# wamuumu/query-recommendation-system

Hardware: AMD Instinct MI355X
Metric: MinHash signatures/sec through the whole hot path (signatures -> LSH candidates -> pair scoring -> top-K) (higher is better)
Workload: dtype u16/int32 MinHash values, uint64 keys and pairs (integer); float64 cosine

## Files before the change

### include/qrlsh.h

```cpp
#ifndef QRLSH_H
#define QRLSH_H

#include <stddef.h>
#include <stdint.h>

#ifdef __cplusplus
extern "C" {
#endif

#define QRLSH_OK 0
#define QRLSH_EINVAL (-1)
#define QRLSH_EHIP (-2)
#define QRLSH_EUNSUPPORTED (-3)
#define QRLSH_EWORKSPACE (-4)

#define QRLSH_PERM_U16 0
#define QRLSH_PERM_I32 1

#define QRLSH_SIG_I32 0
#define QRLSH_SIG_U16 1

#define QRLSH_SORT_MIX 1u
#define QRLSH_SORT_IOTA 2u
#define QRLSH_SORT_FOLD 4u
#define QRLSH_SORT_OWNER 8u

#define QRLSH_SORT_HOST 16u

int qrlsh_version(void);
const char *qrlsh_last_error(void);

uint64_t qrlsh_mix64_host(uint64_t x);

int qrlsh_check_csr(const int64_t *offsets, const int32_t *rows, int64_t nq, int64_t nnz, int32_t D,
                    uint32_t *flags_out, void *stream);
int qrlsh_minhash(const int64_t *offsets, const int32_t *rows, int64_t nq, const void *perm_t,
                  int32_t perm_dtype, int32_t P, int32_t P_stride, int32_t D, int32_t *sig_out,
                  uint16_t *sig16_out, int64_t *norm2_out, uint64_t *keys_out, int32_t b, void *stream);

int qrlsh_band_keys(const int32_t *sig, int64_t nq, int32_t P, int32_t b, uint64_t *keys_out,
                    int64_t *norm2_out, void *stream);

size_t qrlsh_sort_workspace_bytes(int64_t n, int32_t nbatch);
int qrlsh_sort_u64(uint64_t *keys_a, uint64_t *keys_b, uint32_t *vals_a, uint32_t *vals_b, int64_t n,
                   int32_t nbatch, int32_t bit_lo, int32_t bit_hi, uint32_t flags, uint64_t aux,
                   void *workspace, size_t workspace_bytes, void *stream);

int qrlsh_owner_bounds(const uint64_t *words, int64_t n, int32_t bit_lo, uint64_t shard, int32_t world,
                       int64_t *bounds_out, void *stream);

size_t qrlsh_pairs_workspace_bytes(int64_t nq, int32_t b);
int qrlsh_pairs_count(const uint64_t *sorted_keys, int64_t nq, int32_t b, int32_t r, int32_t hash_bits,
                      void *workspace, size_t workspace_bytes, uint64_t *total_out, void *stream);
int qrlsh_pairs_fill(const uint64_t *sorted_keys, const uint32_t *sorted_ids, int64_t nq, int32_t b,
                     int32_t r, int32_t hash_bits, const void *workspace, uint64_t *pairs_out,
                     void *stream);

size_t qrlsh_bucket_workspace_bytes(int64_t nq, int32_t b, int32_t part_bits);
int qrlsh_bucket_pairs_count(const uint64_t *keys, uint64_t *part_keys, uint32_t *part_ids,
                             uint64_t *tmp_keys, uint32_t *tmp_ids, int64_t nq, int32_t b, int32_t r,
                             int32_t part_bits, void *workspace, size_t workspace_bytes,
                             uint64_t *total_overflow_out, void *stream);
int qrlsh_bucket_pairs_fill(const uint64_t *part_keys, const uint32_t *part_ids, int64_t nq, int32_t b,
                            int32_t r, int32_t part_bits, void *workspace, uint64_t *pairs_out,
                            void *stream);
size_t qrlsh_bucket_part_words(int64_t nq, int32_t b, int32_t part_bits);
int64_t qrlsh_set_big_part_limit(int64_t records);
size_t qrlsh_bucket_tmp_words(int64_t nq, int32_t b, int32_t part_bits);
int qrlsh_bucket_pairs_emit(const uint64_t *keys, uint64_t *part_keys, uint32_t *part_ids,
                            uint64_t *tmp_keys, uint32_t *tmp_ids, int64_t nq, int32_t b, int32_t r,
                            int32_t part_bits, void *workspace, size_t workspace_bytes,
                            uint64_t *pairs_out, uint64_t capacity, uint64_t *total_overflow_out,
                            void *stream);

int qrlsh_bucket_pairs_emit_chunked(const uint64_t *keys, int64_t key_chunk, int64_t key_chunk_stride,
                                    int64_t key_band_stride, uint64_t *part_keys, uint32_t *part_ids,
                                    uint64_t *tmp_keys, uint32_t *tmp_ids, int64_t nq, int32_t b, int32_t r,
                                    int32_t part_bits, void *workspace, size_t workspace_bytes,
                                    uint64_t *pairs_out, uint64_t capacity, uint64_t *total_overflow_out,
                                    void *stream);

size_t qrlsh_compact_workspace_bytes(int64_t n);
int qrlsh_unique_count(const uint64_t *sorted, int64_t n, void *workspace, size_t workspace_bytes,
                       uint64_t *total_out, void *stream);
int qrlsh_unique_fill(const uint64_t *sorted, int64_t n, const void *workspace, uint64_t *out,
                      void *stream);

size_t qrlsh_row_unique_workspace_bytes(int64_t n);
int qrlsh_row_unique_count(const uint64_t *grouped, int64_t n, int32_t group_bits, int32_t id_bits,
                           uint64_t *tmp, void *workspace, size_t workspace_bytes, uint64_t *total_overflow_out,
                           void *stream);
int qrlsh_row_unique_fill(const uint64_t *tmp, int64_t n, const void *workspace, uint64_t *out, void *stream);

size_t qrlsh_region_unique_workspace_bytes(int64_t nids, int32_t group_bits);
int qrlsh_region_unique_count(const uint64_t *grouped, int64_t n, int32_t group_bits, int32_t id_bits, int64_t nids,
                              uint64_t *tmp, void *workspace, size_t workspace_bytes, uint64_t *total_overflow_out,
                              void *stream);
int qrlsh_region_unique_fill(const uint64_t *tmp, int64_t n, int32_t group_bits, int64_t nids, const void *workspace,
                             uint64_t *out, void *stream);

size_t qrlsh_pair_regions_words(int64_t n, int64_t nids, int32_t group_bits, double words_per_query);
size_t qrlsh_pair_regions_tmp_words(int64_t n, int64_t nids, int32_t group_bits, double words_per_query);
int64_t qrlsh_pair_regions_cap(int64_t n, int64_t nids, int32_t group_bits, double words_per_query);
int64_t qrlsh_pair_regions_count(int64_t n, int64_t nids, int32_t group_bits, double words_per_query);
int qrlsh_pair_regions_scatter(const uint64_t *words, int64_t n, int32_t group_bits, int64_t nids, double words_per_query,
                               uint64_t *tmp_regions, uint64_t *regions, uint32_t *counts, uint32_t *overflow_out,
                               void *stream);
int qrlsh_region_unique_count_regions(const uint64_t *regions, const uint32_t *counts, int64_t cap, int64_t n,
                                      int32_t group_bits, int32_t id_bits, int64_t nids, uint64_t *tmp, void *workspace,
                                      size_t workspace_bytes, uint64_t *total_overflow_out, void *stream);

int qrlsh_row_norms(const int32_t *sig, int64_t nq, int32_t P, int64_t *norm2_out, void *stream);
int qrlsh_verify_pairs(const void *sig, int32_t sig_dtype, int32_t P, int32_t b, const uint64_t *pairs,
                       int64_t n, uint8_t *flags_out, void *stream);
int qrlsh_score_pairs(const void *sig, int32_t sig_dtype, const int64_t *norm2, int32_t P,
                      const uint64_t *pairs, int64_t n, int32_t *milli_out, double *cos_out,
                      uint64_t *edge_out, int32_t id_bits, uint32_t *edge_dst_out, void *stream);

int qrlsh_topk_count(const uint64_t *sorted_edges, int64_t n_edges, int32_t K, int32_t id_bits,
                     void *workspace, size_t workspace_bytes, uint64_t *total_out, void *stream);
int qrlsh_topk_fill(const uint64_t *sorted_edges, const uint32_t *sorted_dst, int64_t n_edges, int32_t K,
                    int32_t id_bits, const void *workspace, int32_t *src_out, int32_t *dst_out,
                    int32_t *milli_out, void *stream);
int qrlsh_topk_fill_based(const uint64_t *sorted_edges, const uint32_t *sorted_dst, int64_t n_edges, int32_t K,
                          int32_t id_bits, int64_t src_base, const void *workspace, int32_t *src_out,
                          int32_t *dst_out, int32_t *milli_out, void *stream);

int qrlsh_score_pairs_rev(const void *sig, int32_t sig_dtype, const int64_t *norm2, int32_t P,
                          const uint64_t *pairs, int64_t n, int32_t *milli_out, uint64_t *rev_out, int32_t id_bits,
                          uint32_t *rev_dst_out, void *stream);
int qrlsh_set_score_runs(int on);
size_t qrlsh_topk_select_workspace_bytes(int64_t nq);
int qrlsh_topk_select_count(const uint64_t *pairs, int64_t n, const uint64_t *rev_sorted, const uint32_t *rev_dst,
                            int64_t nq, int32_t K, int32_t id_bits, void *workspace, size_t workspace_bytes,
                            uint64_t *total_out, void *stream);
int qrlsh_topk_select_fill(const uint64_t *pairs, const int32_t *milli, int64_t n, const uint64_t *rev_sorted,
                           const uint32_t *rev_dst, int64_t nq, int32_t K, int32_t id_bits, const void *workspace,
                           int32_t *src_out, int32_t *dst_out, int32_t *milli_out, void *stream);

int qrlsh_remap_pairs(const uint64_t *pairs, int64_t n, int64_t q0, int64_t nql, const uint64_t *need,
                      int64_t n_need, uint64_t *out, void *stream);
int qrlsh_pair_edges(const uint64_t *pairs, const int32_t *milli, int64_t n, int32_t id_bits,
                     uint64_t *fwd_out, uint64_t *rev_out, uint32_t *fwd_dst_out, uint32_t *rev_dst_out,
                     void *stream);
size_t qrlsh_idset_workspace_bytes(int64_t nids);
int qrlsh_idset_build(const uint64_t *pairs, int64_t n, int64_t q0, int64_t nql, int64_t nids, int64_t shard,
                      int32_t world, void *workspace, size_t workspace_bytes, int64_t *bounds_out, void *stream);
int qrlsh_idset_list(const void *workspace, int64_t nids, uint64_t *ids_out, void *stream);
int qrlsh_idset_remap(const uint64_t *pairs, int64_t n, int64_t q0, int64_t nql, const void *workspace,
                      int64_t nids, uint64_t *out, void *stream);
int qrlsh_gather_rows(const void *sig, int64_t row_bytes, const int64_t *norm2, const uint64_t *ids, int64_t n,
                      int64_t q0, void *rows_out, int64_t *norms_out, void *stream);
int qrlsh_score_pairs_split(const void *sig, const int64_t *norm2, int64_t split_rows, const void *sig_b,
                            const int64_t *norm2_b, int32_t sig_dtype, int32_t P, const uint64_t *pairs,
                            int64_t n, int32_t *milli_out, void *stream);
int qrlsh_edges_localize(const uint64_t *edges, const uint32_t *edge_dst, int64_t n, int32_t id_bits, int64_t q0,
                         int64_t nql, uint64_t *out, void *stream);

int qrlsh_answer_sets_count(const uint32_t *bitmaps, int64_t words_per_row, int64_t D,
                            const int32_t *qrows, int64_t nq, int32_t nfeat, int32_t *sizes_out,
                            void *stream);
int qrlsh_answer_sets_fill(const uint32_t *bitmaps, int64_t words_per_row, int64_t D,
                           const int32_t *qrows, int64_t nq, int32_t nfeat, const int64_t *offsets,
                           int32_t *rows_out, void *stream);

int qrlsh_answer_sets_sweep(const uint32_t *bitmaps, int64_t words_per_row, int64_t D,
                            const int32_t *qrows, int64_t nq, int32_t nfeat, int32_t *sizes_out,
                            int32_t *slots_out, void *stream);
int qrlsh_answer_sets_compact(const int32_t *slots, const int64_t *offsets, int64_t nq,
                              int32_t *rows_out, void *stream);

#define QRLSH_SUM_PAIRWISE 0
#define QRLSH_SUM_SEQUENTIAL 1
size_t qrlsh_predict_workspace_bytes(int64_t nu, int64_t nq, int32_t kq);
int qrlsh_predict(const int32_t *ratings, int64_t nu, int64_t nq, const int64_t *q_off,
                  const int32_t *q_idx, const double *q_val, const int32_t *u_idx, const double *u_val,
                  int32_t ku, double query_weight, double user_weight, double default_mean,
                  int32_t sum_order, int32_t *out, uint32_t *too_long_out, int32_t kq, void *workspace,
                  size_t workspace_bytes, void *stream);

#define QRLSH_RECOMMEND_MAX_K 1024
size_t qrlsh_recommend_workspace_bytes(int64_t m, int64_t nq, int32_t k, int32_t slices);
int qrlsh_recommend_topk(const int32_t *ratings, const int32_t *pred, int64_t nu, int64_t nq, const int32_t *users,
                         int64_t m, int32_t k, int32_t lo, int32_t slices, int32_t *idx_out, int32_t *val_out,
                         int32_t *avail_out, void *workspace, size_t workspace_bytes, void *stream);

int qrlsh_center_rows(const int32_t *ratings, int64_t nu, int64_t nq, int64_t nq_stride, int32_t *out,
                      void *stream);

size_t qrlsh_user_gram_workspace_bytes(int64_t nu, int64_t nq);
int qrlsh_user_gram(const int32_t *ratings, int64_t nu, int64_t nq, double *mean_out, double *inv_scale_out,
                    double *gram_out, void *workspace, size_t workspace_bytes, void *stream);

size_t qrlsh_gather_sets_workspace_bytes(int64_t n);
int qrlsh_gather_sets_count(const uint64_t *ids, int64_t n, const void *offs, int32_t off_bytes, int64_t nql,
                            int64_t world, uint64_t *offsets_out, void *workspace, size_t workspace_bytes,
                            void *stream);
int qrlsh_gather_sets_fill(const uint64_t *ids, int64_t n, const void *offs, int32_t off_bytes, const void *rows,
                           int32_t row_bytes, int64_t nql, int64_t max_nnz, const uint64_t *offsets,
                           int32_t *rows_out, void *stream);

int qrlsh_synth_sizes(uint64_t seed, int64_t q0, int64_t nq_local, int64_t nq_total, int32_t cluster,
                      uint32_t D, const uint32_t *cdf, int32_t ncdf, uint32_t rep_thresh24,
                      int32_t *sizes_out, void *stream);
int qrlsh_synth_fill(uint64_t seed, int64_t q0, int64_t nq_local, int64_t nq_total, int32_t cluster,
                     uint32_t D, const uint32_t *cdf, int32_t ncdf, uint32_t rep_thresh24,
                     const int64_t *offsets, int32_t *rows_out, void *stream);

int qrlsh_prof_enable(int on);
int qrlsh_set_overlap(int on);
int qrlsh_prof_pause(int paused);
int qrlsh_prof_report(char *buf_host, size_t buflen);

#ifdef __cplusplus
}
#endif
#endif
```

### query-recommendation-system_amd/csrc/score.hip

```cpp
#include <stdlib.h>

#include "common.h"

typedef int i32x4 __attribute__((ext_vector_type(4)));
typedef unsigned short u16x8 __attribute__((ext_vector_type(8)));
typedef unsigned int u32x4 __attribute__((ext_vector_type(4)));

constexpr int SCORE_LPP = 16;

__device__ static inline int64_t c16(unsigned short v) { return v == 0xFFFFu ? -1 : (int64_t)v; }

template <typename SigT, bool VECLOAD>
__global__ __launch_bounds__(256) void score_pairs_kernel(const SigT *__restrict__ sig,
                                                          const int64_t *__restrict__ norm2, int P,
                                                          const uint64_t *__restrict__ pairs, int64_t n,
                                                          int32_t *__restrict__ milli, double *__restrict__ cosv,
                                                          uint64_t *__restrict__ edges, int id_bits,
                                                          uint32_t *__restrict__ edge_dst,
                                                          const SigT *__restrict__ sig_b,
                                                          const int64_t *__restrict__ norm2_b, uint32_t split,
                                                          int rev_only) {
  constexpr bool IS16 = sizeof(SigT) == 2;
  constexpr int VEC = IS16 ? 8 : 4;
  const int lane = threadIdx.x & (WAVE - 1);
  const int lig = lane & (SCORE_LPP - 1);
  const int64_t group = (((int64_t)blockIdx.x * blockDim.x + threadIdx.x) / SCORE_LPP);
  const int64_t ngroups = ((int64_t)gridDim.x * blockDim.x) / SCORE_LPP;
  const int64_t iters = (n + ngroups - 1) / ngroups;
  uint64_t pr_next = (group < n) ? pairs[group] : 0;
  for (int64_t it = 0; it < iters; ++it) {
    const int64_t t = it * ngroups + group;
    const bool live = t < n;
    const uint64_t pr = pr_next;
    const int64_t tn = t + ngroups;
    pr_next = (tn < n) ? pairs[tn] : 0;
    const uint32_t i = (uint32_t)(pr >> 32), j = (uint32_t)pr;
    const SigT *a = i < split ? sig + (size_t)i * P : sig_b + (size_t)(i - split) * P;
    const SigT *c = j < split ? sig + (size_t)j * P : sig_b + (size_t)(j - split) * P;
    const bool own_norms = norm2 == nullptr;
    int64_t na = 0, nb = 0;
    if (!own_norms && live && lig == 0) {
      na = i < split ? norm2[i] : norm2_b[i - split];
      nb = j < split ? norm2[j] : norm2_b[j - split];
    }
    int64_t dot = 0;
    if (live) {
      if (VECLOAD) {
        for (int col = lig * VEC; col < P; col += SCORE_LPP * VEC) {
          if (IS16) {
            const u16x8 x = *reinterpret_cast<const u16x8 *>(a + col);
            const u16x8 y = *reinterpret_cast<const u16x8 *>(c + col);
            const u32x4 xw = __builtin_bit_cast(u32x4, x), yw = __builtin_bit_cast(u32x4, y);
            const uint32_t hi = (xw[0] | xw[1] | xw[2] | xw[3] | yw[0] | yw[1] | yw[2] | yw[3]) & 0x80008000u;
            if (hi == 0) {
              uint32_t s0 = __builtin_amdgcn_udot2(__builtin_shufflevector(x, x, 0, 1),
                                                   __builtin_shufflevector(y, y, 0, 1), 0u, false);
              uint32_t s1 = __builtin_amdgcn_udot2(__builtin_shufflevector(x, x, 2, 3),
                                                   __builtin_shufflevector(y, y, 2, 3), 0u, false);
              s0 = __builtin_amdgcn_udot2(__builtin_shufflevector(x, x, 4, 5), __builtin_shufflevector(y, y, 4, 5),
                                          s0, false);
              s1 = __builtin_amdgcn_udot2(__builtin_shufflevector(x, x, 6, 7), __builtin_shufflevector(y, y, 6, 7),
                                          s1, false);
              dot += (int64_t)((uint64_t)s0 + (uint64_t)s1);
              if (own_norms) {
                uint32_t a0 = 0, a1 = 0, b0 = 0, b1 = 0;
                a0 = __builtin_amdgcn_udot2(__builtin_shufflevector(x, x, 0, 1), __builtin_shufflevector(x, x, 0, 1), a0, false);
                a1 = __builtin_amdgcn_udot2(__builtin_shufflevector(x, x, 2, 3), __builtin_shufflevector(x, x, 2, 3), a1, false);
                a0 = __builtin_amdgcn_udot2(__builtin_shufflevector(x, x, 4, 5), __builtin_shufflevector(x, x, 4, 5), a0, false);
                a1 = __builtin_amdgcn_udot2(__builtin_shufflevector(x, x, 6, 7), __builtin_shufflevector(x, x, 6, 7), a1, false);
                b0 = __builtin_amdgcn_udot2(__builtin_shufflevector(y, y, 0, 1), __builtin_shufflevector(y, y, 0, 1), b0, false);
                b1 = __builtin_amdgcn_udot2(__builtin_shufflevector(y, y, 2, 3), __builtin_shufflevector(y, y, 2, 3), b1, false);
                b0 = __builtin_amdgcn_udot2(__builtin_shufflevector(y, y, 4, 5), __builtin_shufflevector(y, y, 4, 5), b0, false);
                b1 = __builtin_amdgcn_udot2(__builtin_shufflevector(y, y, 6, 7), __builtin_shufflevector(y, y, 6, 7), b1, false);
                na += (int64_t)((uint64_t)a0 + (uint64_t)a1);
                nb += (int64_t)((uint64_t)b0 + (uint64_t)b1);
              }
            } else {
#pragma unroll
              for (int e = 0; e < 8; ++e) {
                const int64_t xe = c16(x[e]), ye = c16(y[e]);
                dot += xe * ye;
                if (own_norms) {
                  na += xe * xe;
                  nb += ye * ye;
                }
              }
            }
          } else {
            const i32x4 x = *reinterpret_cast<const i32x4 *>(a + col);
            const i32x4 y = *reinterpret_cast<const i32x4 *>(c + col);
            dot += (int64_t)x.x * y.x + (int64_t)x.y * y.y + (int64_t)x.z * y.z + (int64_t)x.w * y.w;
            if (own_norms) {
              na += (int64_t)x.x * x.x + (int64_t)x.y * x.y + (int64_t)x.z * x.z + (int64_t)x.w * x.w;
              nb += (int64_t)y.x * y.x + (int64_t)y.y * y.y + (int64_t)y.z * y.z + (int64_t)y.w * y.w;
            }
          }
        }
      } else {
        for (int col = lig; col < P; col += SCORE_LPP) {
          const int64_t xe = IS16 ? c16((unsigned short)a[col]) : (int64_t)a[col];
          const int64_t ye = IS16 ? c16((unsigned short)c[col]) : (int64_t)c[col];
          dot += xe * ye;
          if (own_norms) {
            na += xe * xe;
            nb += ye * ye;
          }
        }
      }
    }
#pragma unroll
    for (int m = 1; m < SCORE_LPP; m <<= 1) dot += __shfl_xor(dot, m, WAVE);
    if (own_norms) {
#pragma unroll
      for (int m = 1; m < SCORE_LPP; m <<= 1) {
        na += __shfl_xor(na, m, WAVE);
        nb += __shfl_xor(nb, m, WAVE);
      }
    }
    if (live && lig == 0) {
      double cs = 0.0;
      if (na != 0 && nb != 0) cs = (double)dot / (sqrt((double)na) * sqrt((double)nb));
      const int32_t mi = (int32_t)rint(cs * 1000.0);
      milli[t] = mi;
      if (cosv) cosv[t] = cs;
      if (edges) {
        const uint64_t inv = (uint64_t)(1000 - mi);
        if (rev_only) {
          if (edge_dst) {
            edges[t] = ((uint64_t)j << 11) | inv;
            edge_dst[t] = i;
          } else {
            edges[t] = ((uint64_t)j << (id_bits + 11)) | (inv << id_bits) | i;
          }
        } else if (edge_dst) {
          edges[2 * t] = ((uint64_t)i << 11) | inv;
          edges[2 * t + 1] = ((uint64_t)j << 11) | inv;
          edge_dst[2 * t] = j;
          edge_dst[2 * t + 1] = i;
        } else {
          edges[2 * t] = ((uint64_t)i << (id_bits + 11)) | (inv << id_bits) | j;
          edges[2 * t + 1] = ((uint64_t)j << (id_bits + 11)) | (inv << id_bits) | i;
        }
      }
    }
  }
}

template <int U> __device__ static inline uint32_t row_bcast_u32(uint32_t v) {
  return (uint32_t)__builtin_amdgcn_update_dpp((int)v, (int)v, 0x150 + U, 0xF, 0xF, false);
}
template <int CTRL> __device__ static inline uint64_t dpp_add_u64(uint64_t v) {
  const uint32_t lo = (uint32_t)__builtin_amdgcn_update_dpp(0, (int)(uint32_t)v, CTRL, 0xF, 0xF, false);
  const uint32_t hi = (uint32_t)__builtin_amdgcn_update_dpp(0, (int)(uint32_t)(v >> 32), CTRL, 0xF, 0xF, false);
  return v + (((uint64_t)hi << 32) | lo);
}
__device__ static inline uint64_t row_sum_u64(uint64_t v) {
  v = dpp_add_u64<0xB1>(v);
  v = dpp_add_u64<0x4E>(v);
  v = dpp_add_u64<0x141>(v);
  v = dpp_add_u64<0x140>(v);
  return v;
}

__device__ static __attribute__((noinline)) uint64_t chunk_dot_wide(u16x8 x, u16x8 y) {
  int64_t d = 0;
#pragma unroll
  for (int e = 0; e < 8; ++e) d += c16(x[e]) * c16(y[e]);
  return (uint64_t)d;
}

__device__ static inline uint64_t chunk_dot(u16x8 x, u16x8 y) {
  const u32x4 xw = __builtin_bit_cast(u32x4, x), yw = __builtin_bit_cast(u32x4, y);
  const uint32_t hi = (xw[0] | xw[1] | xw[2] | xw[3] | yw[0] | yw[1] | yw[2] | yw[3]) & 0x80008000u;
  if (hi == 0) {
    uint32_t s0 = __builtin_amdgcn_udot2(__builtin_shufflevector(x, x, 0, 1), __builtin_shufflevector(y, y, 0, 1), 0u, false);
    uint32_t s1 = __builtin_amdgcn_udot2(__builtin_shufflevector(x, x, 2, 3), __builtin_shufflevector(y, y, 2, 3), 0u, false);
    s0 = __builtin_amdgcn_udot2(__builtin_shufflevector(x, x, 4, 5), __builtin_shufflevector(y, y, 4, 5), s0, false);
    s1 = __builtin_amdgcn_udot2(__builtin_shufflevector(x, x, 6, 7), __builtin_shufflevector(y, y, 6, 7), s1, false);
    return (uint64_t)s0 + (uint64_t)s1;
  }
  return chunk_dot_wide(x, y);
}

#ifndef QR_SCORE_PF
#define QR_SCORE_PF 1
#endif
constexpr int SCORE_PF = QR_SCORE_PF;

#ifndef QR_SCORE_OCC
#define QR_SCORE_OCC 8
#endif
#ifndef QR_SCORE_OCC2
#define QR_SCORE_OCC2 5
#endif
template <int CH>
__global__ __launch_bounds__(256, CH == 1 ? QR_SCORE_OCC : QR_SCORE_OCC2) void score_runs_kernel(const uint16_t *__restrict__ sig, const int64_t *__restrict__ norm2,
                                                         const uint64_t *__restrict__ pairs, int64_t n,
                                                         int32_t *__restrict__ milli, double *__restrict__ cosv,
                                                         uint64_t *__restrict__ edges, int id_bits,
                                                         uint32_t *__restrict__ edge_dst,
                                                         const uint16_t *__restrict__ sig_b,
                                                         const int64_t *__restrict__ norm2_b, uint32_t split, int rev_only) {
  constexpr int P = CH * 128;
  constexpr int NB = SCORE_PF + 1;
  const int lig = threadIdx.x & (SCORE_LPP - 1);
  const int64_t group = ((int64_t)blockIdx.x * blockDim.x + threadIdx.x) / SCORE_LPP;
  const int64_t nchunks = (n + SCORE_LPP - 1) / SCORE_LPP;
  auto row_of = [&](uint32_t id) -> const uint16_t * {
    return (id < split ? sig + (size_t)id * P : sig_b + (size_t)(id - split) * P) + lig * 8;
  };
  auto load_row = [&](u16x8 (&dst)[CH], const uint16_t *p) {
#pragma unroll
    for (int k = 0; k < CH; ++k) dst[k] = *reinterpret_cast<const u16x8 *>(p + k * 128);
  };
  {
    const int64_t c = group;
    if (c >= nchunks) return;
    const int64_t t = c * SCORE_LPP + lig;
    const bool live = t < n;
    const uint64_t pw = live ? pairs[t] : 0ull;
    const uint32_t my_i = (uint32_t)(pw >> 32), my_j = (uint32_t)pw;
    int64_t na = 0, nb = 0;
    if (live) {
      na = my_i < split ? norm2[my_i] : norm2_b[my_i - split];
      nb = my_j < split ? norm2[my_j] : norm2_b[my_j - split];
    }
    uint64_t my_dot = 0;
    u16x8 ab[NB][CH], cb[NB][CH];
#define QR_ROW_I(U) row_bcast_u32<(U)>(my_i)
#define QR_ROW_J(U) row_bcast_u32<(U)>(my_j)
#ifndef QR_SCORE_AREUSE
#define QR_SCORE_AREUSE 0
#endif
#if QR_SCORE_AREUSE
#define QR_REQ(V)                                                                           \
    if ((V) < SCORE_LPP) {                                                                  \
      if ((V) == 0) {                                                                       \
        load_row(ab[0], row_of(QR_ROW_I(0)));                                               \
      } else {                                                                              \
        const uint32_t vi = QR_ROW_I((V) % SCORE_LPP), pi = QR_ROW_I(((V) + SCORE_LPP - 1) % SCORE_LPP); \
        _Pragma("unroll") for (int k = 0; k < CH; ++k) ab[(V) % NB][k] = ab[((V) + NB - 1) % NB][k]; \
        if (vi != pi) load_row(ab[(V) % NB], row_of(vi));                                   \
      }                                                                                     \
      load_row(cb[(V) % NB], row_of(QR_ROW_J((V) % SCORE_LPP)));                            \
    }
#else
#define QR_REQ(V)                                                                           \
    if ((V) < SCORE_LPP) {                                                                  \
      load_row(ab[(V) % NB], row_of(QR_ROW_I((V) % SCORE_LPP)));                            \
      load_row(cb[(V) % NB], row_of(QR_ROW_J((V) % SCORE_LPP)));                            \
    }
#endif
    static_assert(SCORE_PF >= 1 && SCORE_PF <= 4, "prefetch depth");
    QR_REQ(0)
    if (SCORE_PF > 1) { QR_REQ(1) }
    if (SCORE_PF > 2) { QR_REQ(2) }
    if (SCORE_PF > 3) { QR_REQ(3) }
#define QR_STEP(U)                                                                          \
    {                                                                                       \
      QR_REQ((U) + SCORE_PF)                                                                \
      uint64_t part = 0;                                                                    \
      _Pragma("unroll") for (int k = 0; k < CH; ++k) part += chunk_dot(ab[(U) % NB][k], cb[(U) % NB][k]); \
      const uint64_t tot = row_sum_u64(part);                                               \
      if (lig == (U)) my_dot = tot;                                                         \
      asm volatile("" : "+v"(my_dot));     \
      __builtin_amdgcn_sched_barrier(0);  \
    }
    QR_STEP(0) QR_STEP(1) QR_STEP(2) QR_STEP(3) QR_STEP(4) QR_STEP(5) QR_STEP(6) QR_STEP(7)
    QR_STEP(8) QR_STEP(9) QR_STEP(10) QR_STEP(11) QR_STEP(12) QR_STEP(13) QR_STEP(14) QR_STEP(15)
#undef QR_STEP
#undef QR_REQ
#undef QR_ROW_I
#undef QR_ROW_J
    if (live) {
      const int64_t dot = (int64_t)my_dot;
      double cs = 0.0;
      if (na != 0 && nb != 0) cs = (double)dot / (sqrt((double)na) * sqrt((double)nb));
      const int32_t mi = (int32_t)rint(cs * 1000.0);
      milli[t] = mi;
      if (cosv) cosv[t] = cs;
      if (edges) {
        const uint64_t inv = (uint64_t)(1000 - mi), i = my_i, j = my_j;
        if (rev_only) {
          if (edge_dst) {
            edges[t] = (j << 11) | inv;
            edge_dst[t] = (uint32_t)i;
          } else {
            edges[t] = (j << (id_bits + 11)) | (inv << id_bits) | i;
          }
        } else if (edge_dst) {
          edges[2 * t] = (i << 11) | inv;
          edges[2 * t + 1] = (j << 11) | inv;
          edge_dst[2 * t] = (uint32_t)j;
          edge_dst[2 * t + 1] = (uint32_t)i;
        } else {
          edges[2 * t] = (i << (id_bits + 11)) | (inv << id_bits) | j;
          edges[2 * t + 1] = (j << (id_bits + 11)) | (inv << id_bits) | i;
        }
      }
    }
  }
}

static int g_score_runs = -1;
QRLSH_EXPORT int qrlsh_set_score_runs(int on) {
  const int old = g_score_runs;
  g_score_runs = on != 0;
  return old;
}

static int score_launch(const void *sig, const void *sig_b, int64_t split, int32_t sig_dtype, const int64_t *norm2,
                        const int64_t *norm2_b, int32_t P, const uint64_t *pairs, int64_t n, int32_t *milli_out,
                        double *cos_out, uint64_t *edge_out, int32_t id_bits, uint32_t *edge_dst_out, void *stream,
                        int rev_only = 0) {
  const int64_t groups_per_block = 256 / SCORE_LPP;
  int64_t blocks = ceil_div64(n, groups_per_block);
  if (blocks > 256 * 32) blocks = 256 * 32;
  hipStream_t st = static_cast<hipStream_t>(stream);
  const dim3 grid((unsigned)blocks), block(256);
  const bool aligned = ((((uintptr_t)sig | (uintptr_t)sig_b) & 15) == 0);
  const uint32_t sp = split >= (1ll << 32) ? 0xFFFFFFFFu : (uint32_t)split;
  if (sig_dtype == QRLSH_SIG_U16) {
    const uint16_t *s16 = static_cast<const uint16_t *>(sig), *s16b = static_cast<const uint16_t *>(sig_b);
    if (g_score_runs < 0) {
      const char *e = getenv("QRLSH_SCORE_RUNS");
      g_score_runs = !(e && e[0] == '0');
    }
    if (g_score_runs && aligned && norm2 && (P == 128 || P == 256) && (sig_b == nullptr || norm2_b)) {
      const int64_t rb = ceil_div64(ceil_div64(n, SCORE_LPP), groups_per_block);
      QR_CHECK_ARG(rb <= 2147483647ll, "qrlsh_score_pairs: too many pairs for one launch");
      const dim3 rgrid((unsigned)rb);
      if (P == 128)
        QR_LAUNCH("score_pairs", (score_runs_kernel<1>), rgrid, block, 0, st, s16, norm2, pairs, n, milli_out, cos_out,
                  edge_out, id_bits, edge_dst_out, s16b, norm2_b, sp, rev_only);
      else
        QR_LAUNCH("score_pairs", (score_runs_kernel<2>), rgrid, block, 0, st, s16, norm2, pairs, n, milli_out, cos_out,
                  edge_out, id_bits, edge_dst_out, s16b, norm2_b, sp, rev_only);
      QR_LAUNCH_CHECK("qrlsh_score_pairs");
      return QRLSH_OK;
    }
    if (aligned && P % 8 == 0)
      QR_LAUNCH("score_pairs", (score_pairs_kernel<uint16_t, true>), grid, block, 0, st, s16, norm2, P, pairs, n, milli_out,
                cos_out, edge_out, id_bits, edge_dst_out, s16b, norm2_b, sp, rev_only);
    else
      QR_LAUNCH("score_pairs", (score_pairs_kernel<uint16_t, false>), grid, block, 0, st, s16, norm2, P, pairs, n, milli_out,
                cos_out, edge_out, id_bits, edge_dst_out, s16b, norm2_b, sp, rev_only);
  } else {
    const int32_t *s32 = static_cast<const int32_t *>(sig), *s32b = static_cast<const int32_t *>(sig_b);
    if (aligned && P % 4 == 0)
      QR_LAUNCH("score_pairs", (score_pairs_kernel<int32_t, true>), grid, block, 0, st, s32, norm2, P, pairs, n, milli_out,
                cos_out, edge_out, id_bits, edge_dst_out, s32b, norm2_b, sp, rev_only);
    else
      QR_LAUNCH("score_pairs", (score_pairs_kernel<int32_t, false>), grid, block, 0, st, s32, norm2, P, pairs, n, milli_out,
                cos_out, edge_out, id_bits, edge_dst_out, s32b, norm2_b, sp, rev_only);
  }
  QR_LAUNCH_CHECK("qrlsh_score_pairs");
  return QRLSH_OK;
}

QRLSH_EXPORT int qrlsh_score_pairs(const void *sig, int32_t sig_dtype, const int64_t *norm2, int32_t P,
                                   const uint64_t *pairs, int64_t n, int32_t *milli_out, double *cos_out,
                                   uint64_t *edge_out, int32_t id_bits, uint32_t *edge_dst_out, void *stream) {
  QR_CHECK_ARG(n >= 0 && P > 0, "qrlsh_score_pairs: bad sizes n=%lld P=%d", (long long)n, P);
  QR_CHECK_ARG(sig_dtype == QRLSH_SIG_I32 || sig_dtype == QRLSH_SIG_U16, "qrlsh_score_pairs: bad sig_dtype %d", sig_dtype);
  if (n == 0) return QRLSH_OK;
  QR_CHECK_ARG(sig && pairs && milli_out, "qrlsh_score_pairs: null pointer");
  if (edge_out && !edge_dst_out)
    QR_CHECK_ARG(id_bits > 0 && id_bits <= 26, "qrlsh_score_pairs: id_bits=%d must be in [1,26] without edge_dst_out", id_bits);
  QR_CHECK_ARG(!edge_dst_out || edge_out, "qrlsh_score_pairs: edge_dst_out needs edge_out");
  return score_launch(sig, nullptr, 1ll << 32, sig_dtype, norm2, nullptr, P, pairs, n, milli_out, cos_out, edge_out,
                      id_bits, edge_dst_out, stream);
}

QRLSH_EXPORT int qrlsh_score_pairs_rev(const void *sig, int32_t sig_dtype, const int64_t *norm2, int32_t P,
                                       const uint64_t *pairs, int64_t n, int32_t *milli_out, uint64_t *rev_out,
                                       int32_t id_bits, uint32_t *rev_dst_out, void *stream) {
  QR_CHECK_ARG(n >= 0 && P > 0, "qrlsh_score_pairs_rev: bad sizes n=%lld P=%d", (long long)n, P);
  QR_CHECK_ARG(sig_dtype == QRLSH_SIG_I32 || sig_dtype == QRLSH_SIG_U16, "qrlsh_score_pairs_rev: bad sig_dtype %d",
               sig_dtype);
  if (n == 0) return QRLSH_OK;
  QR_CHECK_ARG(sig && pairs && milli_out && rev_out, "qrlsh_score_pairs_rev: null pointer");
  QR_CHECK_ARG(rev_dst_out || (id_bits > 0 && id_bits <= 26),
               "qrlsh_score_pairs_rev: id_bits=%d must be in [1,26] without rev_dst_out", id_bits);
  return score_launch(sig, nullptr, 1ll << 32, sig_dtype, norm2, nullptr, P, pairs, n, milli_out, nullptr, rev_out, id_bits,
                      rev_dst_out, stream, 1);
}

QRLSH_EXPORT int qrlsh_score_pairs_split(const void *sig, const int64_t *norm2, int64_t split_rows, const void *sig_b,
                                         const int64_t *norm2_b, int32_t sig_dtype, int32_t P, const uint64_t *pairs,
                                         int64_t n, int32_t *milli_out, void *stream) {
  QR_CHECK_ARG(n >= 0 && P > 0 && split_rows >= 0 && split_rows < (1ll << 32), "qrlsh_score_pairs_split: bad sizes");
  QR_CHECK_ARG(sig_dtype == QRLSH_SIG_I32 || sig_dtype == QRLSH_SIG_U16, "qrlsh_score_pairs_split: bad sig_dtype %d",
               sig_dtype);
  if (n == 0) return QRLSH_OK;
  QR_CHECK_ARG(pairs && milli_out && (split_rows == 0 || sig) && ((norm2 == nullptr) == (norm2_b == nullptr) || !sig_b),
               "qrlsh_score_pairs_split: null pointer (norm2 and norm2_b: both or neither)");
  return score_launch(sig, sig_b, split_rows, sig_dtype, norm2, norm2_b, P, pairs, n, milli_out, nullptr, nullptr, 0,
                      nullptr, stream, 0);
}

template <typename SigT>
__global__ __launch_bounds__(256) void verify_pairs_kernel(const SigT *__restrict__ sig, int P, int b,
                                                           const uint64_t *__restrict__ pairs, int64_t n,
                                                           uint8_t *__restrict__ flags) {
  const int64_t t = (int64_t)blockIdx.x * blockDim.x + threadIdx.x;
  if (t >= n) return;
  const uint64_t pr = pairs[t];
  const SigT *a = sig + (size_t)(uint32_t)(pr >> 32) * P;
  const SigT *c = sig + (size_t)(uint32_t)pr * P;
  const int r = P / b;
  uint8_t hit = 0;
  for (int band = 0; band < b && !hit; ++band) {
    bool eq = true, empty = true;
    for (int k = 0; k < r; ++k) {
      const uint32_t x = (uint32_t)a[band * r + k] & 0xFFFFu, y = (uint32_t)c[band * r + k] & 0xFFFFu;
      eq &= x == y;
      empty &= x == 0xFFFFu;
    }
    hit = eq && !empty;
  }
  flags[t] = hit;
}

QRLSH_EXPORT int qrlsh_verify_pairs(const void *sig, int32_t sig_dtype, int32_t P, int32_t b, const uint64_t *pairs,
                                    int64_t n, uint8_t *flags_out, void *stream) {
  QR_CHECK_ARG(n >= 0 && P > 0 && b > 0 && P % b == 0, "qrlsh_verify_pairs: bad sizes n=%lld P=%d b=%d", (long long)n, P, b);
  QR_CHECK_ARG(sig_dtype == QRLSH_SIG_I32 || sig_dtype == QRLSH_SIG_U16, "qrlsh_verify_pairs: bad sig_dtype %d", sig_dtype);
  if (n == 0) return QRLSH_OK;
  QR_CHECK_ARG(sig && pairs && flags_out, "qrlsh_verify_pairs: null pointer");
  hipStream_t st = static_cast<hipStream_t>(stream);
  const dim3 grid((unsigned)ceil_div64(n, 256)), block(256);
  if (sig_dtype == QRLSH_SIG_U16)
    QR_LAUNCH("verify_pairs", (verify_pairs_kernel<uint16_t>), grid, block, 0, st, static_cast<const uint16_t *>(sig), P, b,
              pairs, n, flags_out);
  else
    QR_LAUNCH("verify_pairs", (verify_pairs_kernel<int32_t>), grid, block, 0, st, static_cast<const int32_t *>(sig), P, b,
              pairs, n, flags_out);
  QR_LAUNCH_CHECK("qrlsh_verify_pairs");
  return QRLSH_OK;
}

__global__ __launch_bounds__(256) void remap_pairs_kernel(const uint64_t *__restrict__ pairs, int64_t n, uint64_t q0,
                                                          uint64_t nql, const uint64_t *__restrict__ need,
                                                          int64_t n_need, uint64_t *__restrict__ out) {
  const int64_t t = (int64_t)blockIdx.x * blockDim.x + threadIdx.x;
  if (t >= n) return;
  const uint64_t pr = pairs[t], i = pr >> 32, j = pr & 0xFFFFFFFFull;
  uint64_t slot;
  if (j >= q0 && j < q0 + nql) {
    slot = j - q0;
  } else {
    int64_t lo = 0, hi = n_need;
    while (lo < hi) {
      const int64_t mid = (lo + hi) >> 1;
      if (need[mid] < j) lo = mid + 1;
      else hi = mid;
    }
    slot = nql + (uint64_t)lo;
  }
  out[t] = (i - q0) << 32 | slot;
}

__global__ __launch_bounds__(256) void pair_edges_kernel(const uint64_t *__restrict__ pairs,
                                                         const int32_t *__restrict__ milli, int64_t n, int id_bits,
                                                         uint64_t *__restrict__ fwd, uint64_t *__restrict__ rev,
                                                         uint32_t *__restrict__ fwd_dst,
                                                         uint32_t *__restrict__ rev_dst) {
  const int64_t t = (int64_t)blockIdx.x * blockDim.x + threadIdx.x;
  if (t >= n) return;
  const uint64_t pr = pairs[t], i = pr >> 32, j = pr & 0xFFFFFFFFull, inv = (uint64_t)(1000 - milli[t]);
  uint64_t *f = rev ? fwd + t : fwd + 2 * t, *r = rev ? rev + t : fwd + 2 * t + 1;
  if (id_bits > 0) {
    *f = i << (id_bits + 11) | inv << id_bits | j;
    *r = j << (id_bits + 11) | inv << id_bits | i;
  } else {
    *f = i << 11 | inv;
    *r = j << 11 | inv;
    if (rev) {
      fwd_dst[t] = (uint32_t)j;
      rev_dst[t] = (uint32_t)i;
    } else {
      fwd_dst[2 * t] = (uint32_t)j;
      fwd_dst[2 * t + 1] = (uint32_t)i;
    }
  }
}

QRLSH_EXPORT int qrlsh_remap_pairs(const uint64_t *pairs, int64_t n, int64_t q0, int64_t nql, const uint64_t *need,
                                   int64_t n_need, uint64_t *out, void *stream) {
  QR_CHECK_ARG(n >= 0 && q0 >= 0 && nql >= 0 && n_need >= 0, "qrlsh_remap_pairs: bad sizes");
  if (n == 0) return QRLSH_OK;
  QR_CHECK_ARG(pairs && out && (n_need == 0 || need), "qrlsh_remap_pairs: null pointer");
  QR_LAUNCH("remap_pairs", remap_pairs_kernel, dim3((unsigned)ceil_div64(n, 256)), dim3(256), 0,
            static_cast<hipStream_t>(stream), pairs, n, (uint64_t)q0, (uint64_t)nql, need, n_need, out);
  QR_LAUNCH_CHECK("qrlsh_remap_pairs");
  return QRLSH_OK;
}

QRLSH_EXPORT int qrlsh_pair_edges(const uint64_t *pairs, const int32_t *milli, int64_t n, int32_t id_bits,
                                  uint64_t *fwd_out, uint64_t *rev_out, uint32_t *fwd_dst_out, uint32_t *rev_dst_out,
                                  void *stream) {
  QR_CHECK_ARG(n >= 0 && id_bits >= 0 && id_bits <= 26, "qrlsh_pair_edges: bad arguments (id_bits=%d)", id_bits);
  if (n == 0) return QRLSH_OK;
  QR_CHECK_ARG(pairs && milli && fwd_out, "qrlsh_pair_edges: null pointer");
  QR_CHECK_ARG(id_bits > 0 || (fwd_dst_out && (rev_dst_out || !rev_out)), "qrlsh_pair_edges: id_bits == 0 needs the dst outputs");
  QR_LAUNCH("pair_edges", pair_edges_kernel, dim3((unsigned)ceil_div64(n, 256)), dim3(256), 0,
            static_cast<hipStream_t>(stream), pairs, milli, n, id_bits, fwd_out, rev_out, fwd_dst_out, rev_dst_out);
  QR_LAUNCH_CHECK("qrlsh_pair_edges");
  return QRLSH_OK;
}
```

### query-recommendation-system_amd/csrc/sort.hip

```cpp
#include "common.h"

constexpr int SORT_THREADS = 256;
constexpr int SORT_IPT = 16;
constexpr int SORT_TILE = SORT_THREADS * SORT_IPT;
constexpr int RADIX = 256;

__device__ static inline int xcd_tile(int bid, int ntiles) {
  const int q = ntiles >> 3, r = ntiles & 7, x = bid & 7, y = bid >> 3;
  return (x < r ? x * (q + 1) : r * (q + 1) + (x - r) * q) + y;
}

enum { SM_PLAIN = 0, SM_MIX = 1, SM_FOLD = 2, SM_OWNER = 3, SM_HOST = 4 };
template <int MODE> __device__ static inline uint32_t digit_of(uint64_t key, int shift, uint32_t fold = 0) {
  if (MODE == SM_OWNER || MODE == SM_HOST) {
    const uint64_t o = MODE == SM_HOST ? qr_pair_host(key, fold) : (key >> shift) / fold;
    return o < RADIX ? (uint32_t)o : RADIX - 1;
  }
  uint64_t x = key;
  if (MODE == SM_MIX) x = qr_mix64(key);
  if (MODE == SM_FOLD) x = ((key >> 32) << fold) | (key & ((1ull << fold) - 1ull));
  return (uint32_t)(x >> shift) & (RADIX - 1);
}

template <bool SPREAD>
// ... 307 lines not shown
    for (int i = 0; i < SORT_THREADS / WAVE; ++i) {
      const uint32_t c = cnt[i][d];
      cnt[i][d] = run;
      run += c;
    }
  }
  __syncthreads();
#pragma unroll
  for (int k = 0; k < SORT_IPT; ++k) {
    const int64_t idx = wbase + (int64_t)k * WAVE + lane;
    if (idx < n) skey[cnt[w][dr[k] >> 16] + (dr[k] & 0xFFFFu)] = key[k];
  }
  __syncthreads();
  const int ntile = (int)min((int64_t)SORT_TILE, n - tbase);
#pragma unroll
  for (int k = 0; k < SORT_IPT; ++k) {
    const int p = k * SORT_THREADS + threadIdx.x;
    if (p < ntile) {
      const uint64_t kk = skey[p];
      keys_out[boff + gdelta[digit_of<MODE>(kk, shift, fold)] + (uint32_t)p] = kk;
    }
  }
}

template <bool IOTA>
__global__ __launch_bounds__(SORT_THREADS, 3) void part_scatter_staged_kernel(
    const uint64_t *__restrict__ keys_in, const uint32_t *__restrict__ vals_in, uint64_t *__restrict__ keys_out,
    uint32_t *__restrict__ vals_out, int64_t n, int ntiles, int shift, const uint32_t *__restrict__ goff,
    const uint32_t *__restrict__ rtot, uint64_t ek, uint32_t dmask) {
  __shared__ uint32_t cnt[SORT_THREADS / WAVE][RADIX];
  __shared__ uint32_t dsum[SORT_THREADS / WAVE];
  __shared__ uint32_t lsum[SORT_THREADS / WAVE];
  __shared__ uint32_t gdelta[RADIX];
  __shared__ uint64_t skey[SORT_TILE];
  __shared__ uint32_t sval[SORT_TILE];
  const int tile = xcd_tile(blockIdx.x, ntiles), batch = blockIdx.y;
  const int lane = threadIdx.x & (WAVE - 1), w = threadIdx.x >> 6;
#pragma unroll
  for (int i = 0; i < SORT_THREADS / WAVE; ++i) cnt[i][threadIdx.x] = 0;
  __syncthreads();
  const size_t boff = (size_t)batch * n;
  const int64_t tbase = (int64_t)tile * SORT_TILE;
  const int64_t wbase = tbase + (int64_t)w * (WAVE * SORT_IPT);
  uint64_t key[SORT_IPT];
  uint32_t val[SORT_IPT];
  uint32_t dr[SORT_IPT];
  const uint64_t lt_mask = (1ull << lane) - 1ull;
#pragma unroll
  for (int k = 0; k < SORT_IPT; ++k) {
    const int64_t idx = wbase + (int64_t)k * WAVE + lane;
    const bool valid = idx < n;
    key[k] = valid ? keys_in[boff + idx] : 0;
    val[k] = IOTA ? (uint32_t)idx : (valid ? vals_in[boff + idx] : 0);
  }
#pragma unroll
  for (int k = 0; k < SORT_IPT; ++k) {
    const int64_t idx = wbase + (int64_t)k * WAVE + lane;
    const bool valid = idx < n;
    const uint32_t d = part_digit<true>(key[k], (int64_t)val[k], shift, ek, dmask);
    uint64_t m = __ballot(valid);
#pragma unroll
    for (int bit = 0; bit < 8; ++bit) {
      const bool one = (d >> bit) & 1u;
      const uint64_t bal = __ballot(one);
      m &= one ? bal : ~bal;
    }
    const uint32_t below = (uint32_t)__popcll(m & lt_mask);
    uint32_t prev = 0;
    if (valid) {
      prev = cnt[w][d];
      if (below == 0) cnt[w][d] = prev + (uint32_t)__popcll(m);
    }
    dr[k] = (d << 16) | (prev + below);
  }
  __syncthreads();
  {
    const int d = threadIdx.x;
    const uint32_t tot = rtot[(size_t)batch * RADIX + d];
    uint32_t tc = 0;
#pragma unroll
    for (int i = 0; i < SORT_THREADS / WAVE; ++i) tc += cnt[i][d];
    uint32_t inc = tot, linc = tc;
#pragma unroll
    for (int k = 1; k < WAVE; k <<= 1) {
      const uint32_t o = __shfl_up(inc, k, WAVE), lo = __shfl_up(linc, k, WAVE);
      if (lane >= k) {
        inc += o;
        linc += lo;
      }
    }
    if (lane == WAVE - 1) {
      dsum[w] = inc;
      lsum[w] = linc;
    }
    __syncthreads();
    uint32_t dbase = inc - tot, lstart = linc - tc;
#pragma unroll
    for (int k = 0; k < SORT_THREADS / WAVE; ++k)
      if (k < w) {
        dbase += dsum[k];
        lstart += lsum[k];
      }
    gdelta[d] = dbase + goff[((size_t)batch * RADIX + d) * ntiles + tile] - lstart;
    uint32_t run = lstart;
#pragma unroll
    for (int i = 0; i < SORT_THREADS / WAVE; ++i) {
      const uint32_t c = cnt[i][d];
      cnt[i][d] = run;
      run += c;
    }
  }
  __syncthreads();
#pragma unroll
  for (int k = 0; k < SORT_IPT; ++k) {
    const int64_t idx = wbase + (int64_t)k * WAVE + lane;
    if (idx < n) {
      const uint32_t d = dr[k] >> 16, lp = cnt[w][d] + (dr[k] & 0xFFFFu);
      skey[lp] = key[k];
      sval[lp] = val[k] | d << 24;
    }
  }
  __syncthreads();
  const int ntile = (int)min((int64_t)SORT_TILE, n - tbase);
#pragma unroll
  for (int k = 0; k < SORT_IPT; ++k) {
    const int p = k * SORT_THREADS + threadIdx.x;
    if (p < ntile) {
      const uint32_t vv = sval[p];
      const size_t dst = boff + gdelta[vv >> 24] + (uint32_t)p;
      keys_out[dst] = skey[p];
      vals_out[dst] = vv & 0xFFFFFFu;
    }
  }
}

struct PartPool {
  uint64_t *keys;
  uint32_t *vals;
  unsigned long long *cursor;
  uint32_t cap;
  uint4 *runs;
  unsigned long long *nruns;
  uint32_t runs_max;
  uint32_t *fill;
  uint32_t slot_base;
};

#ifndef QR_PS_IPT
#define QR_PS_IPT 16
#endif
constexpr int PS_IPT = QR_PS_IPT;
constexpr int PS_TILE = SORT_THREADS * PS_IPT;
constexpr int PS_WGS = PS_IPT <= 16 ? 3 : 2;
template <bool LEVEL2>
__global__ __launch_bounds__(SORT_THREADS, PS_WGS) void part_scatter_atomic_kernel(
    const uint64_t *__restrict__ keys_in, const uint32_t *__restrict__ vals_in, uint64_t *__restrict__ keys_out,
    uint32_t *__restrict__ vals_out, int64_t n_in, int ntiles, int shift, uint32_t dmask,
    uint32_t *__restrict__ cursors, uint32_t cap, uint32_t *__restrict__ overflow, uint64_t ek,
    const uint32_t *__restrict__ in_counts, uint32_t in_cap, int64_t chunk_len, int64_t chunk_stride,
    int64_t band_stride, PartPool pool) {
  __shared__ uint32_t cnt[RADIX];
  __shared__ uint32_t lsum[SORT_THREADS / WAVE];
  __shared__ uint32_t gdelta[RADIX];
  __shared__ uint8_t gok[RADIX];
  __shared__ uint64_t skey[PS_TILE];
  __shared__ uint32_t sval[PS_TILE];
  const int tile = LEVEL2 ? (int)blockIdx.x : xcd_tile(blockIdx.x, ntiles), batch = blockIdx.y;
  const int lane = threadIdx.x & (WAVE - 1), w = threadIdx.x >> 6;
  const int64_t n = LEVEL2 ? (int64_t)min(in_counts[batch], in_cap) : n_in;
  const int64_t tbase = (int64_t)tile * PS_TILE;
  if (tbase >= n) return;
  cnt[threadIdx.x] = 0;
  __syncthreads();
  const size_t boff = LEVEL2 ? (size_t)batch * in_cap : (size_t)batch * (size_t)(band_stride ? band_stride : n);
  const bool chunked = !LEVEL2 && chunk_len > 0 && chunk_len < n;
  const int64_t wbase = tbase + (int64_t)w * (WAVE * PS_IPT);
  const uint32_t nd = dmask + 1u;
  uint64_t key[PS_IPT];
  uint32_t val[PS_IPT];
  uint32_t dr[PS_IPT];
#pragma unroll
  for (int k = 0; k < PS_IPT; ++k) {
    const int64_t idx = wbase + (int64_t)k * WAVE + lane;
    const size_t at = chunked ? boff + (size_t)(idx / chunk_len) * chunk_stride + (size_t)(idx % chunk_len) : boff + idx;
    key[k] = idx < n ? keys_in[at] : ek;
    val[k] = LEVEL2 ? (idx < n ? vals_in[boff + idx] : 0u) : (uint32_t)idx;
  }
#pragma unroll
  for (int k = 0; k < PS_IPT; ++k) {
    const int64_t idx = wbase + (int64_t)k * WAVE + lane;
    const bool valid = idx < n && (LEVEL2 || key[k] != ek);
    if (!LEVEL2) key[k] = qr_mix64(key[k]);
    const uint32_t d = (uint32_t)(key[k] >> shift) & dmask;
    dr[k] = valid ? (d << 16) | atomicAdd(&cnt[d], 1u) : 0xFFFFFFFFu;
  }
  __syncthreads();
  const uint32_t tc = cnt[threadIdx.x];
  const uint32_t gb = tc ? atomicAdd(&cursors[(size_t)batch * nd + threadIdx.x], tc) : 0u;
  uint32_t lstart;
  {
    uint32_t linc = tc;
#pragma unroll
    for (int k = 1; k < WAVE; k <<= 1) {
      const uint32_t lo = __shfl_up(linc, k, WAVE);
      if (lane >= k) linc += lo;
    }
    if (lane == WAVE - 1) lsum[w] = linc;
    __syncthreads();
    lstart = linc - tc;
#pragma unroll
    for (int k = 0; k < SORT_THREADS / WAVE; ++k)
      if (k < w) lstart += lsum[k];
    cnt[threadIdx.x] = lstart;
  }
  __syncthreads();
#pragma unroll
  for (int k = 0; k < PS_IPT; ++k) {
    if (dr[k] != 0xFFFFFFFFu) {
      const uint32_t lp = cnt[dr[k] >> 16] + (dr[k] & 0xFFFFu);
      skey[lp] = key[k];
      sval[lp] = val[k];
    }
  }
  {
    const int d = threadIdx.x;
    uint32_t where = gb + tc <= cap ? 1u : 0u;
    uint32_t delta = (uint32_t)d * cap + gb - lstart;
    if (!where) {
      if (pool.keys) {
        const unsigned long long pb =
            __hip_atomic_fetch_add(pool.cursor, (unsigned long long)tc, __ATOMIC_RELAXED, __HIP_MEMORY_SCOPE_AGENT);
        if (pb + tc <= (unsigned long long)pool.cap) {
          const unsigned long long ri = __hip_atomic_fetch_add(pool.nruns, 1ull, __ATOMIC_RELAXED, __HIP_MEMORY_SCOPE_AGENT);
          if (ri < (unsigned long long)pool.runs_max) {
            const uint32_t slot = pool.slot_base + (uint32_t)batch * nd + (uint32_t)d;
            pool.runs[ri] = make_uint4(slot, tc, (uint32_t)pb, 0u);
            atomicMin(&pool.fill[slot], gb);
            where = 2u;
            delta = (uint32_t)pb - lstart;
          }
        }
      }
      if (!where) atomicOr(overflow, 1u);
    }
    gok[d] = (uint8_t)where;
    gdelta[d] = delta;
  }
  __syncthreads();
  uint32_t nstaged = 0;
#pragma unroll
  for (int k = 0; k < SORT_THREADS / WAVE; ++k) nstaged += lsum[k];
  const size_t obase = (size_t)batch * nd * cap;
#pragma unroll
  for (int k = 0; k < PS_IPT; ++k) {
    const uint32_t p = k * SORT_THREADS + threadIdx.x;
    if (p < nstaged) {
      const uint64_t x = skey[p];
      const uint32_t d = (uint32_t)(x >> shift) & dmask;
      const uint32_t where = gok[d];
      if (where == 1u) {
        const size_t dst = obase + (uint32_t)(gdelta[d] + p);
        keys_out[dst] = x;
        vals_out[dst] = sval[p];
      } else if (where == 2u) {
        const uint32_t dst = gdelta[d] + p;
        pool.keys[dst] = x;
        pool.vals[dst] = sval[p];
      }
    }
  }
}

#ifndef QR_PG_IPT
#define QR_PG_IPT 32
#endif
constexpr int PG_IPT = QR_PG_IPT;
constexpr int PG_TILE = SORT_THREADS * PG_IPT;
constexpr int PG_WGS = PG_IPT <= 16 ? 4 : PG_IPT <= 40 ? 2 : 1;
template <bool LEVEL2>
__global__ __launch_bounds__(SORT_THREADS, PG_WGS) void pair_group_scatter_kernel(
    const uint64_t *__restrict__ in, uint64_t *__restrict__ out, int64_t n_in, int ntiles, int shift, uint32_t dmask,
    uint32_t *__restrict__ cursors, uint32_t cap, uint32_t *__restrict__ overflow, const uint32_t *__restrict__ in_counts,
    uint32_t in_cap) {
  __shared__ uint32_t cnt[RADIX];
  __shared__ uint32_t lsum[SORT_THREADS / WAVE];
  __shared__ uint32_t gdelta[RADIX];
  __shared__ uint8_t gok[RADIX];
  __shared__ uint64_t skey[PG_TILE];
  const int tile = LEVEL2 ? (int)blockIdx.x : xcd_tile(blockIdx.x, ntiles), batch = blockIdx.y;
  const int lane = threadIdx.x & (WAVE - 1), w = threadIdx.x >> 6;
  const int64_t n = LEVEL2 ? (int64_t)min(in_counts[batch], in_cap) : n_in;
  const int64_t tbase = (int64_t)tile * PG_TILE;
  if (tbase >= n) return;
  cnt[threadIdx.x] = 0;
  __syncthreads();
  const size_t boff = LEVEL2 ? (size_t)batch * in_cap : 0;
  const int64_t wbase = tbase + (int64_t)w * (WAVE * PG_IPT);
  const uint32_t nd = dmask + 1u;
  uint64_t key[PG_IPT];
  uint32_t dr[PG_IPT];
#pragma unroll
  for (int k = 0; k < PG_IPT; ++k) {
    const int64_t idx = wbase + (int64_t)k * WAVE + lane;
    key[k] = idx < n ? in[boff + idx] : 0ull;
  }
#pragma unroll
  for (int k = 0; k < PG_IPT; ++k) {
    const int64_t idx = wbase + (int64_t)k * WAVE + lane;
    const uint32_t d = (uint32_t)(key[k] >> shift) & dmask;
    dr[k] = idx < n ? (d << 16) | atomicAdd(&cnt[d], 1u) : 0xFFFFFFFFu;
  }
  __syncthreads();
  const uint32_t tc = cnt[threadIdx.x];
  const uint32_t gb = tc ? atomicAdd(&cursors[(size_t)batch * nd + threadIdx.x], tc) : 0u;
  uint32_t lstart;
  {
    uint32_t linc = tc;
#pragma unroll
    for (int k = 1; k < WAVE; k <<= 1) {
      const uint32_t lo = __shfl_up(linc, k, WAVE);
      if (lane >= k) linc += lo;
    }
    if (lane == WAVE - 1) lsum[w] = linc;
    __syncthreads();
    lstart = linc - tc;
#pragma unroll
    for (int k = 0; k < SORT_THREADS / WAVE; ++k)
      if (k < w) lstart += lsum[k];
    cnt[threadIdx.x] = lstart;
  }
  __syncthreads();
#pragma unroll
  for (int k = 0; k < PG_IPT; ++k)
    if (dr[k] != 0xFFFFFFFFu) skey[cnt[dr[k] >> 16] + (dr[k] & 0xFFFFu)] = key[k];
  {
    const int d = threadIdx.x;
    const bool ok = (uint64_t)gb + tc <= cap;
    if (!ok) atomicOr(overflow, 1u);
    gok[d] = ok;
    gdelta[d] = (uint32_t)d * cap + gb - lstart;
  }
  __syncthreads();
  uint32_t nstaged = 0;
#pragma unroll
  for (int k = 0; k < SORT_THREADS / WAVE; ++k) nstaged += lsum[k];
  const size_t obase = (size_t)batch * nd * cap;
#pragma unroll
  for (int k = 0; k < PG_IPT; ++k) {
    const uint32_t p = k * SORT_THREADS + threadIdx.x;
    if (p < nstaged) {
      const uint64_t x = skey[p];
      const uint32_t d = (uint32_t)(x >> shift) & dmask;
      if (gok[d]) out[obase + (uint32_t)(gdelta[d] + p)] = x;
    }
  }
}

struct PairRegions {
  int rbits, ra, rb;
  int64_t nregions;
  int64_t na;
  uint32_t cap_a, cap_b;
};
static PairRegions pair_regions(int64_t n, int64_t nids, int group_bits, double words_per_query) {
  PairRegions r;
  const int64_t nr = (nids + (1ll << group_bits) - 1) >> group_bits;
  r.rbits = 1;
  while ((1ll << r.rbits) < nr) ++r.rbits;
  r.rb = r.rbits <= 8 ? r.rbits : (r.rbits + 1) / 2;
  r.ra = r.rbits - r.rb;
  r.na = (nr + (1ll << r.rb) - 1) >> r.rb;
  r.nregions = r.na << r.rb;
  double per = (double)n / (double)(nr > 0 ? nr : 1);
  const double hint = words_per_query * (double)(1ll << group_bits);
  if (hint > per) per = hint;
  const double cb = 3.0 * per + 4096.0;
  const double ca = r.ra ? 2.5 * per * (double)(1ll << r.rb) + 65536.0 : 0.0;
  r.cap_b = (uint32_t)(cb > 4.0e9 ? 4.0e9 : cb);
  r.cap_b = (r.cap_b + 63u) / 64u * 64u;
  r.cap_a = (uint32_t)(ca > 4.0e9 ? 4.0e9 : ca);
  r.cap_a = (r.cap_a + 63u) / 64u * 64u;
  return r;
}

static bool pair_regions_fit_u32(const PairRegions &r) {
  return (uint64_t)r.na * r.cap_a < (1ull << 32) && ((uint64_t)r.cap_b << r.rb) < (1ull << 32);
}

QRLSH_EXPORT size_t qrlsh_pair_regions_words(int64_t n, int64_t nids, int32_t group_bits, double words_per_query) {
  if (n <= 0 || nids <= 0 || group_bits < 0 || group_bits > 8) return 0;
  const PairRegions r = pair_regions(n, nids, group_bits, words_per_query);
  if (r.rbits > 16) return 0;
  if (!pair_regions_fit_u32(r)) return 0;
  return (size_t)r.nregions * r.cap_b;
}
QRLSH_EXPORT size_t qrlsh_pair_regions_tmp_words(int64_t n, int64_t nids, int32_t group_bits, double words_per_query) {
  if (n <= 0 || nids <= 0 || group_bits < 0 || group_bits > 8) return 0;
  const PairRegions r = pair_regions(n, nids, group_bits, words_per_query);
  return r.ra ? (size_t)r.na * r.cap_a : 0;
}
QRLSH_EXPORT int64_t qrlsh_pair_regions_cap(int64_t n, int64_t nids, int32_t group_bits, double words_per_query) {
  if (n <= 0 || nids <= 0 || group_bits < 0 || group_bits > 8) return 0;
  return (int64_t)pair_regions(n, nids, group_bits, words_per_query).cap_b;
}
QRLSH_EXPORT int64_t qrlsh_pair_regions_count(int64_t n, int64_t nids, int32_t group_bits, double words_per_query) {
  if (n <= 0 || nids <= 0 || group_bits < 0 || group_bits > 8) return 0;
  return pair_regions(n, nids, group_bits, words_per_query).nregions;
}

QRLSH_EXPORT int qrlsh_pair_regions_scatter(const uint64_t *words, int64_t n, int32_t group_bits, int64_t nids,
                                            double words_per_query, uint64_t *tmp_regions, uint64_t *regions,
                                            uint32_t *counts, uint32_t *overflow_out, void *stream) {
  QR_CHECK_ARG(n >= 0 && n < (1ll << 32) && nids > 0 && group_bits >= 0 && group_bits <= 8 && counts && overflow_out,
               "qrlsh_pair_regions_scatter: bad arguments");
  hipStream_t st = static_cast<hipStream_t>(stream);
  const PairRegions r = pair_regions(n > 0 ? n : 1, nids, group_bits, words_per_query);
  QR_CHECK_ARG(r.rbits <= 16 && r.na <= RADIX, "qrlsh_pair_regions_scatter: %d region bits", r.rbits);
  QR_CHECK_ARG(pair_regions_fit_u32(r),
               "qrlsh_pair_regions_scatter: regions reach 2^32 words (na * cap_a = %llu, 2^rb * cap_b = %llu; need both < 2^32)",
               (unsigned long long)r.na * r.cap_a, (unsigned long long)r.cap_b << r.rb);
// ... 213 lines not shown
  static_assert(CAP % THREADS == 0 && CAP <= 65535, "image = whole records per thread, slots fit 16 bits");
  __shared__ unsigned long long gbase;
  __shared__ __attribute__((aligned(16))) unsigned long long tab[CAP];
  __shared__ uint32_t cnt[CAP];
  __shared__ uint32_t wsum[THREADS / WAVE];
  const int part = blockIdx.x, band = blockIdx.y;
  const int tid = threadIdx.x, lane = tid & (WAVE - 1), w = tid >> 6;
  const size_t bslot = (size_t)band * nparts + part;
  const uint32_t start = counts ? 0u : starts[(size_t)band * (nparts + 1) + part];
  const uint32_t m = counts ? counts[bslot] : starts[(size_t)band * (nparts + 1) + part + 1] - start;
  const size_t first = counts ? bslot * cap : (size_t)band * nq + start;
  if (m > (uint32_t)CAP || (counts && m > cap)) {
    if (tid == 0) {
      bool listed = false;
      if (MODE == FIN_EMIT && biglist && counts) {
        const unsigned long long at =
            __hip_atomic_fetch_add(nbig, 1ull, __ATOMIC_RELAXED, __HIP_MEMORY_SCOPE_AGENT);
        if (at < (unsigned long long)big_max) {
          biglist[at] = (uint64_t)(big_base + bslot);
          listed = true;
        }
      }
      if (!listed) atomicOr(overflow, 1u);
      if (MODE == FIN_COUNT) blk[bslot] = 0;
    }
    return;
  }
  if (m == 0) {
    if (MODE == FIN_COUNT && tid == 0) blk[bslot] = 0;
    return;
  }
  const uint64_t *k = keys + first;
  const uint32_t *id = ids + first;
  uint64_t kreg[IPT];
  uint32_t ireg[IPT];
#pragma unroll
  for (int j = 0; j < IPT; ++j) {
    const uint32_t i = tid + j * THREADS;
    kreg[j] = i < m ? k[i] : ek;
    if (FILL) ireg[j] = i < m ? id[i] : 0u;
  }
#pragma unroll
  for (int j = 0; j < IPT; ++j) {
    const uint32_t i = tid + j * THREADS;
    tab[i] = ek;
    cnt[i] = 0;
  }
  __syncthreads();
  uint32_t so[IPT];
  uint32_t mine = 0;
  uint32_t slot[IPT];
  unsigned long long seen[IPT];
#pragma unroll
  for (int j = 0; j < IPT; ++j) {
    slot[j] = fin_home<CAP>(kreg[j]);
    seen[j] = kreg[j] != ek
                  ? atomicCAS(&tab[slot[j]], (unsigned long long)ek, (unsigned long long)kreg[j])
                  : (unsigned long long)ek;
  }
#pragma unroll
  for (int j = 0; j < IPT; ++j) {
    if (kreg[j] != ek) {
      unsigned long long old = seen[j];
      while (old != ek && old != kreg[j]) {
        slot[j] = slot[j] + 1 == (uint32_t)CAP ? 0u : slot[j] + 1;
        old = atomicCAS(&tab[slot[j]], (unsigned long long)ek, (unsigned long long)kreg[j]);
      }
    }
  }
#pragma unroll
  for (int j = 0; j < IPT; ++j) {
    so[j] = 0xFFFFFFFFu;
    if (kreg[j] != ek) {
      const uint32_t o = atomicAdd(&cnt[slot[j]], 1u);
      so[j] = o << 16 | slot[j];
      mine += o;
    }
  }
  uint32_t inc = mine;
#pragma unroll
  for (int d = 1; d < WAVE; d <<= 1) {
    const uint32_t o = __shfl_up(inc, d, WAVE);
    if (lane >= d) inc += o;
  }
  if (lane == WAVE - 1) wsum[w] = inc;
  __syncthreads();
  uint32_t base = 0, tot = 0;
#pragma unroll
  for (int i = 0; i < THREADS / WAVE; ++i) {
    const uint32_t x = wsum[i];
    if (i < w) base += x;
    tot += x;
  }
  if (MODE == FIN_COUNT) {
    if (tid == 0) blk[bslot] = (uint64_t)tot;
    return;
  }
  if (MODE == FIN_EMIT) {
    if (tot == 0) return;
    if (tid == 0)
      gbase = __hip_atomic_fetch_add(reinterpret_cast<unsigned long long *>(blk), (unsigned long long)tot,
                                     __ATOMIC_RELAXED, __HIP_MEMORY_SCOPE_AGENT);
  }
  const uint32_t pos0 = base + inc - mine;
  {
    const uint32_t b0 = tid * IPT;
    uint32_t v[IPT], sum = 0;
#pragma unroll
    for (int q = 0; q < IPT; ++q) {
      v[q] = cnt[b0 + q];
      sum += v[q];
    }
    uint32_t sinc = sum;
#pragma unroll
    for (int d = 1; d < WAVE; d <<= 1) {
      const uint32_t o = __shfl_up(sinc, d, WAVE);
      if (lane >= d) sinc += o;
    }
    __syncthreads();
    if (lane == WAVE - 1) wsum[w] = sinc;
    __syncthreads();
    uint32_t run = sinc - sum;
#pragma unroll
    for (int i = 0; i < THREADS / WAVE; ++i)
      if (i < w) run += wsum[i];
#pragma unroll
    for (int q = 0; q < IPT; ++q) {
      cnt[b0 + q] = run;
      run += v[q];
    }
  }
  __syncthreads();
  uint32_t *grp = reinterpret_cast<uint32_t *>(tab);
#pragma unroll
  for (int j = 0; j < IPT; ++j)
    if (so[j] != 0xFFFFFFFFu) grp[cnt[so[j] & 0xFFFFu] + (so[j] >> 16)] = ireg[j];
  __syncthreads();
  {
    const uint64_t obase = MODE == FIN_EMIT ? (uint64_t)gbase : blk[bslot];
    if (MODE == FIN_EMIT && obase + tot > capacity) return;
    uint64_t *dst = out + obase;
    uint32_t pos = pos0;
#pragma unroll
    for (int j = 0; j < IPT; ++j) {
      const bool rec = so[j] != 0xFFFFFFFFu;
      const uint32_t o = rec ? so[j] >> 16 : 0u;
      emit_run(dst, pos, ireg[j], grp, rec ? cnt[so[j] & 0xFFFFu] : 0u, o);
      pos += o;
    }
  }
}

constexpr int FIN_PK_THREADS = 512, FIN_PK_CAP = 4096, FIN_PK_MAX = 4095;
__global__ __launch_bounds__(FIN_PK_THREADS, 8) void bucket_finish_packed_kernel(
    const uint64_t *__restrict__ keys, const uint32_t *__restrict__ ids, int nparts, uint64_t *__restrict__ blk,
    uint32_t *__restrict__ overflow, uint64_t *__restrict__ out, uint64_t capacity, const uint32_t *__restrict__ counts,
    uint32_t cap, uint64_t *__restrict__ biglist, unsigned long long *__restrict__ nbig, uint32_t big_max,
    uint32_t big_base) {
  constexpr int THREADS = FIN_PK_THREADS, CAP = FIN_PK_CAP, IPT = CAP / THREADS;
  constexpr unsigned long long KMASK = (1ull << 52) - 1ull, ONE = 1ull << 52;
  __shared__ unsigned long long gbase;
  __shared__ __attribute__((aligned(16))) unsigned long long tab[CAP];
  __shared__ uint32_t wsum[THREADS / WAVE];
  const int part = blockIdx.x, band = blockIdx.y;
  const int tid = threadIdx.x, lane = tid & (WAVE - 1), w = tid >> 6;
  const size_t bslot = (size_t)band * nparts + part;
  const uint32_t m = counts[bslot];
  if (m > (uint32_t)FIN_PK_MAX) {
    if (tid == 0) {
      bool listed = false;
      const unsigned long long at = __hip_atomic_fetch_add(nbig, 1ull, __ATOMIC_RELAXED, __HIP_MEMORY_SCOPE_AGENT);
      if (at < (unsigned long long)big_max) {
        biglist[at] = (uint64_t)(big_base + bslot);
        listed = true;
      }
      if (!listed) atomicOr(overflow, 1u);
    }
    return;
  }
  if (m == 0) return;
  const size_t first = bslot * cap;
  const uint64_t *k = keys + first;
  const uint32_t *id = ids + first;
  uint64_t kreg[IPT];
  uint32_t ireg[IPT];
#pragma unroll
  for (int j = 0; j < IPT; ++j) {
    const uint32_t i = tid + j * THREADS;
    kreg[j] = i < m ? k[i] : 0ull;
    ireg[j] = i < m ? id[i] : 0u;
  }
#pragma unroll
  for (int j = 0; j < IPT; ++j) tab[tid + j * THREADS] = 0ull;
  __syncthreads();
  uint32_t so[IPT];
  uint32_t mine = 0;
#pragma unroll
  for (int j = 0; j < IPT; ++j) {
    so[j] = 0xFFFFFFFFu;
    if (tid + j * THREADS < (int)m) {
      const unsigned long long k52 = kreg[j] & KMASK;
      uint32_t slot = fin_home<CAP>(kreg[j]);
      uint32_t o;
      for (;;) {
        const unsigned long long old = atomicCAS(&tab[slot], 0ull, k52 | ONE);
        if (old == 0ull) {
          o = 0;
          break;
        }
        if ((old & KMASK) == k52) {
          o = (uint32_t)(atomicAdd(&tab[slot], ONE) >> 52);
          break;
        }
        slot = slot + 1 == (uint32_t)CAP ? 0u : slot + 1;
      }
      so[j] = o << 16 | slot;
      mine += o;
    }
  }
  uint32_t inc = mine;
#pragma unroll
  for (int d = 1; d < WAVE; d <<= 1) {
    const uint32_t o = __shfl_up(inc, d, WAVE);
    if (lane >= d) inc += o;
  }
  if (lane == WAVE - 1) wsum[w] = inc;
  __syncthreads();
  uint32_t base = 0, tot = 0;
#pragma unroll
  for (int i = 0; i < THREADS / WAVE; ++i) {
    const uint32_t x = wsum[i];
    if (i < w) base += x;
    tot += x;
  }
  if (tot == 0) return;
  if (tid == 0)
    gbase = __hip_atomic_fetch_add(reinterpret_cast<unsigned long long *>(blk), (unsigned long long)tot, __ATOMIC_RELAXED,
                                   __HIP_MEMORY_SCOPE_AGENT);
  const uint32_t pos0 = base + inc - mine;
  uint32_t *rs = reinterpret_cast<uint32_t *>(tab);
  uint32_t *grp = rs + CAP;
  {
    const uint32_t b0 = tid * IPT;
    uint32_t v[IPT], sum = 0;
#pragma unroll
    for (int q = 0; q < IPT; ++q) {
      v[q] = (uint32_t)(tab[b0 + q] >> 52);
      sum += v[q];
    }
    uint32_t sinc = sum;
#pragma unroll
    for (int d = 1; d < WAVE; d <<= 1) {
      const uint32_t o = __shfl_up(sinc, d, WAVE);
      if (lane >= d) sinc += o;
    }
    __syncthreads();
    if (lane == WAVE - 1) wsum[w] = sinc;
    __syncthreads();
    uint32_t run = sinc - sum;
#pragma unroll
    for (int i = 0; i < THREADS / WAVE; ++i)
      if (i < w) run += wsum[i];
#pragma unroll
    for (int q = 0; q < IPT; ++q) {
      rs[b0 + q] = run;
      run += v[q];
    }
  }
  __syncthreads();
#pragma unroll
  for (int j = 0; j < IPT; ++j)
    if (so[j] != 0xFFFFFFFFu) grp[rs[so[j] & 0xFFFFu] + (so[j] >> 16)] = ireg[j];
  __syncthreads();
  {
    const uint64_t obase = (uint64_t)gbase;
    if (obase + tot > capacity) return;
    uint64_t *dst = out + obase;
    uint32_t pos = pos0;
#pragma unroll
    for (int j = 0; j < IPT; ++j) {
      const bool rec = so[j] != 0xFFFFFFFFu;
      const uint32_t o = rec ? so[j] >> 16 : 0u;
      emit_run(dst, pos, ireg[j], grp, rec ? rs[so[j] & 0xFFFFu] : 0u, o);
      pos += o;
    }
  }
}

constexpr int FIN_BIG_GRID = 256;
constexpr int FIN_BIG_BLOCKS = 16;
constexpr uint32_t FIN_BIG_LIST = 4096;
constexpr int FIN_BIG_SLICES = 8;
constexpr uint32_t POOL_RUNS = 1u << 20;

struct BigDesc {
  uint64_t where;
  uint32_t m, pool;
};

__global__ __launch_bounds__(256) void bucket_big_gather_kernel(const uint64_t *__restrict__ biglist,
                                                                const unsigned long long *__restrict__ nbig, uint32_t big_max,
                                                                BigDesc *__restrict__ desc, const uint64_t *__restrict__ part_keys,
                                                                const uint32_t *__restrict__ part_ids,
                                                                const uint32_t *__restrict__ counts, uint32_t cap, PartPool pool,
                                                                uint32_t max_records, uint32_t *__restrict__ overflow) {
  __shared__ unsigned long long base_s;
  __shared__ uint32_t match[256];
  __shared__ uint32_t nmatch;
  const int tid = threadIdx.x;
  unsigned long long nb = *nbig;
  if (nb > big_max) nb = big_max;
  for (unsigned long long e = blockIdx.x; e < nb; e += gridDim.x) {
    const uint32_t slot = (uint32_t)biglist[e];
    const uint32_t m = counts[slot];
    const uint32_t f = pool.fill ? pool.fill[slot] : 0xFFFFFFFFu;
    if (m > max_records || (f == 0xFFFFFFFFu && m > cap)) {
      if (tid == 0) {
        atomicOr(overflow, 1u);
        desc[e] = BigDesc{0ull, 0u, 0u};
      }
      continue;
    }
    if (f == 0xFFFFFFFFu) {
      if (tid == 0) desc[e] = BigDesc{(uint64_t)slot * cap, m, 0u};
      continue;
    }
    __syncthreads();
    if (tid == 0)
      base_s = __hip_atomic_fetch_add(pool.cursor, (unsigned long long)m, __ATOMIC_RELAXED, __HIP_MEMORY_SCOPE_AGENT);
    __syncthreads();
    const unsigned long long base = base_s;
    if (base + m > (unsigned long long)pool.cap) {
      if (tid == 0) {
        atomicOr(overflow, 1u);
        desc[e] = BigDesc{0ull, 0u, 0u};
      }
      continue;
    }
    for (uint32_t i = tid; i < f; i += blockDim.x) {
      pool.keys[base + i] = part_keys[(size_t)slot * cap + i];
      pool.vals[base + i] = part_ids[(size_t)slot * cap + i];
    }
    uint32_t at = f;
    unsigned long long nr = *pool.nruns;
    if (nr > pool.runs_max) nr = pool.runs_max;
    for (unsigned long long r0 = 0; r0 < nr; r0 += blockDim.x) {
      __syncthreads();
      if (tid == 0) nmatch = 0;
      __syncthreads();
      const unsigned long long r = r0 + tid;
      if (r < nr && pool.runs[r].x == slot) match[atomicAdd(&nmatch, 1u)] = (uint32_t)r;
      __syncthreads();
      const uint32_t nm = nmatch;
      for (uint32_t q = 0; q < nm; ++q) {
        const uint4 run = pool.runs[match[q]];
        if (at + run.y <= m)
          for (uint32_t i = tid; i < run.y; i += blockDim.x) {
            pool.keys[base + at + i] = pool.keys[(size_t)run.z + i];
            pool.vals[base + at + i] = pool.vals[(size_t)run.z + i];
          }
        at += run.y;
      }
    }
    if (tid == 0) {
      if (at != m) atomicOr(overflow, 1u);
      desc[e] = BigDesc{(uint64_t)base, at == m ? m : 0u, 1u};
    }
  }
}

__global__ __launch_bounds__(FIN_THREADS) void bucket_finish_big_kernel(
    const uint64_t *__restrict__ keys, const uint32_t *__restrict__ ids, const uint64_t *pool_keys, const uint32_t *pool_ids,
    uint64_t ek, const BigDesc *__restrict__ desc, const unsigned long long *__restrict__ nbig, uint32_t big_max,
    uint64_t *__restrict__ blk, uint64_t *__restrict__ out, uint64_t capacity) {
  __shared__ unsigned long long gbase;
  __shared__ __attribute__((aligned(16))) unsigned long long tab[FIN_CAP];
  __shared__ uint32_t cnt[FIN_CAP + 1];
  __shared__ uint32_t grp[FIN_CAP];
  __shared__ uint32_t srt[FIN_CAP];
  __shared__ uint32_t wsum[FIN_THREADS / WAVE];
  const int tid = threadIdx.x, lane = tid & (WAVE - 1), w = tid >> 6;
  unsigned long long nb = *nbig;
  if (nb > big_max) nb = big_max;
  auto scan = [&](uint32_t v, uint32_t &total) -> uint32_t {
    uint32_t inc = v;
#pragma unroll
    for (int d = 1; d < WAVE; d <<= 1) {
      const uint32_t o = __shfl_up(inc, d, WAVE);
      if (lane >= d) inc += o;
    }
    __syncthreads();
    if (lane == WAVE - 1) wsum[w] = inc;
    __syncthreads();
    uint32_t base = 0, tot = 0;
#pragma unroll
    for (int i = 0; i < FIN_THREADS / WAVE; ++i) {
      const uint32_t x = wsum[i];
      if (i < w) base += x;
      tot += x;
    }
    total = tot;
    return base + inc - v;
  };
  constexpr int COMBOS = FIN_BIG_BLOCKS * (FIN_BIG_BLOCKS + 1) / 2;
  static_assert(FIN_THREADS % FIN_BIG_SLICES == 0, "a thread's records share their position mod the slice count");
  for (unsigned long long item = blockIdx.x; item < nb * COMBOS * FIN_BIG_SLICES; item += gridDim.x) {
    const uint32_t sl = (uint32_t)(item % FIN_BIG_SLICES);
    const unsigned long long e = item / ((unsigned long long)COMBOS * FIN_BIG_SLICES);
    int combo = (int)((item / FIN_BIG_SLICES) % COMBOS);
    uint32_t bi = 0;
    while (combo > (int)bi) {
      combo -= (int)bi + 1;
      ++bi;
    }
    const uint32_t bj_only = (uint32_t)combo;
    const BigDesc de = desc[e];
    const uint32_t m = de.m;
    const uint64_t *k = (de.pool ? pool_keys : keys) + de.where;
    const uint32_t *id = (de.pool ? pool_ids : ids) + de.where;
    const uint32_t nblk = (m + FIN_CAP - 1) / FIN_CAP;
    if (bi >= nblk) continue;
    {
      const uint32_t lo = bi * FIN_CAP, mb = min((uint32_t)FIN_CAP, m - lo);
      uint64_t kreg[FIN_IPT];
      uint32_t ireg[FIN_IPT], so[FIN_IPT];
      __syncthreads();
#pragma unroll
      for (int j = 0; j < FIN_IPT; ++j) {
        const uint32_t i = tid + j * FIN_THREADS;
        kreg[j] = i < mb ? k[lo + i] : ek;
        ireg[j] = i < mb ? id[lo + i] : 0u;
        tab[i] = ek;
        cnt[i] = 0;
      }
      __syncthreads();
#pragma unroll
      for (int j = 0; j < FIN_IPT; ++j) {
        so[j] = 0xFFFFFFFFu;
        if (kreg[j] != ek) {
          uint32_t slot = fin_home(kreg[j]);
          for (;;) {
            const unsigned long long old = atomicCAS(&tab[slot], (unsigned long long)ek, (unsigned long long)kreg[j]);
            if (old == ek || old == kreg[j]) break;
            slot = slot + 1 == (uint32_t)FIN_CAP ? 0u : slot + 1;
          }
          const uint32_t o = atomicAdd(&cnt[slot], 1u);
          so[j] = o << 16 | slot;
        }
      }
      __syncthreads();
      {
        const uint32_t b0 = tid * FIN_IPT;
        uint32_t v[FIN_IPT], sum = 0;
#pragma unroll
        for (int q = 0; q < FIN_IPT; ++q) {
          v[q] = cnt[b0 + q];
          sum += v[q];
        }
        uint32_t all;
        uint32_t run = scan(sum, all);
#pragma unroll
        for (int q = 0; q < FIN_IPT; ++q) {
          cnt[b0 + q] = run;
          run += v[q];
        }
        if (tid == 0) cnt[FIN_CAP] = all;
      }
      __syncthreads();
#pragma unroll
      for (int j = 0; j < FIN_IPT; ++j)
        if (so[j] != 0xFFFFFFFFu) grp[cnt[so[j] & 0xFFFFu] + (so[j] >> 16)] = ireg[j];
      __syncthreads();
      if (bj_only == bi) {
        uint32_t rk[FIN_IPT];
#pragma unroll
        for (int j = 0; j < FIN_IPT; ++j) {
          rk[j] = 0;
          if (so[j] != 0xFFFFFFFFu) {
            const uint32_t sl0 = so[j] & 0xFFFFu, s0 = cnt[sl0], c = cnt[sl0 + 1] - s0, me = ireg[j];
            uint32_t r = 0;
            for (uint32_t u = 0; u < c; ++u) r += grp[s0 + u] < me;
            rk[j] = r;
          }
        }
        __syncthreads();
#pragma unroll
        for (int j = 0; j < FIN_IPT; ++j)
          if (so[j] != 0xFFFFFFFFu) srt[cnt[so[j] & 0xFFFFu] + rk[j]] = ireg[j];
        uint32_t mine = 0;
#pragma unroll
        for (int j = 0; j < FIN_IPT; ++j) {
          if (so[j] == 0xFFFFFFFFu || (rk[j] & (FIN_BIG_SLICES - 1)) != sl) rk[j] = 0;
          mine += rk[j];
        }
        uint32_t tot;
        const uint32_t pos0 = scan(mine, tot);
        if (tid == 0 && tot)
          gbase = __hip_atomic_fetch_add(reinterpret_cast<unsigned long long *>(blk), (unsigned long long)tot,
                                         __ATOMIC_RELAXED, __HIP_MEMORY_SCOPE_AGENT);
        __syncthreads();
        if (tot && gbase + tot <= capacity) {
          uint64_t *dst = out + gbase;
          uint32_t pos = pos0;
#pragma unroll
          for (int j = 0; j < FIN_IPT; ++j) {
            emit_run(dst, pos, ireg[j], srt, so[j] != 0xFFFFFFFFu ? cnt[so[j] & 0xFFFFu] : 0u, rk[j]);
            pos += rk[j];
          }
        }
      }
      if (bj_only < bi) {
        const uint32_t bj = bj_only;
        const uint32_t lo2 = bj * FIN_CAP;
        uint32_t hit[FIN_IPT];
        uint32_t mine2 = 0;
#pragma unroll
        for (int j = 0; j < FIN_IPT; ++j) {
          const uint32_t i = tid + j * FIN_THREADS;
          const uint64_t x = k[lo2 + i];
          ireg[j] = id[lo2 + i];
          uint32_t slot = fin_home(x), found = 0xFFFFFFFFu;
          const bool my_slice = (uint32_t)(tid & (FIN_BIG_SLICES - 1)) == sl;
          for (int step = 0; my_slice && step < FIN_CAP; ++step) {
            const unsigned long long tv = tab[slot];
            if (tv == x) {
              found = slot;
              break;
            }
            if (tv == ek) break;
            slot = slot + 1 == (uint32_t)FIN_CAP ? 0u : slot + 1;
          }
          if ((uint32_t)(tid & (FIN_BIG_SLICES - 1)) != sl) found = 0xFFFFFFFFu;
          hit[j] = found;
          if (found != 0xFFFFFFFFu) mine2 += cnt[found + 1] - cnt[found];
        }
        uint32_t tot2;
        const uint32_t p0 = scan(mine2, tot2);
        if (tid == 0 && tot2)
          gbase = __hip_atomic_fetch_add(reinterpret_cast<unsigned long long *>(blk), (unsigned long long)tot2,
                                         __ATOMIC_RELAXED, __HIP_MEMORY_SCOPE_AGENT);
        __syncthreads();
        if (tot2 && gbase + tot2 <= capacity) {
          uint64_t *dst = out + gbase;
          uint32_t pos = p0;
#pragma unroll
          for (int j = 0; j < FIN_IPT; ++j) {
            const bool h = hit[j] != 0xFFFFFFFFu;
            const uint32_t s0 = h ? cnt[hit[j]] : 0u, c = h ? cnt[hit[j] + 1] - s0 : 0u;
            emit_run(dst, pos, ireg[j], grp, s0, c);
            pos += c;
          }
        }
        __syncthreads();
      }
    }
  }
}

static int g_fin_packed = [] {
  const char *e = getenv("QRLSH_FIN_PACKED");
  return !(e && e[0] == '0') ? 1 : 0;
}();

static uint32_t g_big_limit = (uint32_t)FIN_BIG_BLOCKS * FIN_CAP;
QRLSH_EXPORT int64_t qrlsh_set_big_part_limit(int64_t records) {
  const int64_t max = (int64_t)FIN_BIG_BLOCKS * FIN_CAP, old = g_big_limit;
  g_big_limit = (uint32_t)(records <= 0 || records > max ? max : records);
  return old;
}

static size_t align16(size_t x) { return (x + 15) & ~(size_t)15; }
constexpr int EMIT_MAX_GROUPS = 16;
struct BucketWs {
  uint32_t *ghist, *rtot, *starts;
  uint64_t *blk;
  uint32_t *tail;
  uint32_t *fill;
  unsigned long long *poolctl;
  uint4 *runs;
  BigDesc *desc;
  size_t bytes;
};
static BucketWs bucket_ws(void *workspace, int64_t nq, int32_t b, int32_t T) {
  BucketWs w;
  const size_t nparts = (size_t)1 << T;
  const int64_t ntiles = ceil_div64(nq, SORT_TILE);
  char *p = static_cast<char *>(workspace);
  size_t off = 0;
  w.ghist = reinterpret_cast<uint32_t *>(p + off);
  w.rtot = w.ghist + (size_t)b * RADIX * ntiles;
  off += align16(qrlsh_sort_workspace_bytes(nq, b));
  w.starts = reinterpret_cast<uint32_t *>(p + off);
  off += align16((size_t)b * (nparts + 1) * sizeof(uint32_t));
  w.blk = reinterpret_cast<uint64_t *>(p + off);
  off += (size_t)b * nparts * sizeof(uint64_t);
  w.tail = reinterpret_cast<uint32_t *>(p + off);
  off += 16;
  w.fill = reinterpret_cast<uint32_t *>(p + off);
  off += align16((size_t)b * nparts * sizeof(uint32_t));
  w.poolctl = reinterpret_cast<unsigned long long *>(p + off);
  off += 16;
  w.runs = reinterpret_cast<uint4 *>(p + off);
  off += (size_t)POOL_RUNS * sizeof(uint4);
  w.desc = reinterpret_cast<BigDesc *>(p + off);
  off += (size_t)EMIT_MAX_GROUPS * FIN_BIG_LIST * sizeof(BigDesc);
  w.bytes = off;
  return w;
}

QRLSH_EXPORT size_t qrlsh_bucket_workspace_bytes(int64_t nq, int32_t b, int32_t part_bits) {
  if (nq <= 0 || b <= 0 || part_bits < 8 || part_bits > 16) return 64;
  return bucket_ws(nullptr, nq, b, part_bits).bytes;
}

static void bucket_partition(const uint64_t *keys, uint64_t *part_keys, uint32_t *part_ids, uint64_t *tmp_keys,
                             uint32_t *tmp_ids, int64_t nq, int32_t b, int32_t r, int32_t part_bits, const BucketWs &w,
                             hipStream_t st) {
  const int T = part_bits, nparts = 1 << T;
  const int ntiles = (int)ceil_div64(nq, SORT_TILE);
  const dim3 grid(ntiles, b), block(SORT_THREADS);
  const uint64_t ek = qr_empty_key(r);
  const uint32_t *no_vals = nullptr;
  const bool staged = nq <= (1ll << 24);
  if (T == 8) {
    QR_LAUNCH("sort_hist", (sort_hist_kernel<SM_MIX, true>), grid, block, 0, st, keys, nq, ntiles, 56, w.ghist, ek, 0,
              (uint32_t)RADIX - 1u, no_vals);
    launch_rowscan(w.ghist, ntiles, w.rtot, b, st);
    if (staged)
      QR_LAUNCH("sort_scatter_kv", (part_scatter_staged_kernel<true>), grid, block, 0, st, keys, no_vals, part_keys,
                part_ids, nq, ntiles, 56, w.ghist, w.rtot, ek, (uint32_t)RADIX - 1u);
    else
      QR_LAUNCH("sort_scatter_kv", (sort_scatter_kernel<SM_MIX, true, true, true>), grid, block, 0, st, keys, no_vals,
                part_keys, part_ids, nq, ntiles, 56, w.ghist, w.rtot, ek, 0, (uint32_t)RADIX - 1u);
  } else {
    const uint32_t lowmask = (1u << (T - 8)) - 1u;
    QR_LAUNCH("sort_hist", (sort_hist_kernel<SM_MIX, true>), grid, block, 0, st, keys, nq, ntiles, 64 - T, w.ghist, ek, 0,
              lowmask, no_vals);
    launch_rowscan(w.ghist, ntiles, w.rtot, b, st);
    if (staged)
      QR_LAUNCH("sort_scatter_kv", (part_scatter_staged_kernel<true>), grid, block, 0, st, keys, no_vals, tmp_keys,
                tmp_ids, nq, ntiles, 64 - T, w.ghist, w.rtot, ek, lowmask);
    else
      QR_LAUNCH("sort_scatter_kv", (sort_scatter_kernel<SM_MIX, true, true, true>), grid, block, 0, st, keys, no_vals,
                tmp_keys, tmp_ids, nq, ntiles, 64 - T, w.ghist, w.rtot, ek, 0, lowmask);
    QR_LAUNCH("sort_hist", (sort_hist_kernel<SM_MIX, true>), grid, block, 0, st, (const uint64_t *)tmp_keys, nq, ntiles,
              56, w.ghist, ek, 0, (uint32_t)RADIX - 1u, (const uint32_t *)tmp_ids);
    launch_rowscan(w.ghist, ntiles, w.rtot, b, st);
    if (staged)
      QR_LAUNCH("sort_scatter_kv", (part_scatter_staged_kernel<false>), grid, block, 0, st, (const uint64_t *)tmp_keys,
                (const uint32_t *)tmp_ids, part_keys, part_ids, nq, ntiles, 56, w.ghist, w.rtot, ek,
                (uint32_t)RADIX - 1u);
    else
      QR_LAUNCH("sort_scatter_kv", (sort_scatter_kernel<SM_MIX, true, false, true>), grid, block, 0, st,
                (const uint64_t *)tmp_keys, (const uint32_t *)tmp_ids, part_keys, part_ids, nq, ntiles, 56, w.ghist,
                w.rtot, ek, 0, (uint32_t)RADIX - 1u);
  }
  QR_LAUNCH("bucket_bounds", bucket_bounds_kernel, dim3((nparts + 1 + 255) / 256, b), dim3(256), 0, st,
            (const uint64_t *)part_keys, (const uint32_t *)part_ids, nq, T, ek, w.starts);
}

static int bucket_check(const char *name, const uint64_t *keys, uint64_t *part_keys, uint32_t *part_ids,
                        uint64_t *tmp_keys, uint32_t *tmp_ids, int64_t nq, int32_t b, int32_t r, int32_t part_bits,
                        void *workspace, size_t workspace_bytes, uint64_t *total_overflow_out, hipStream_t st) {
  QR_CHECK_ARG(nq >= 0 && b > 0 && b <= 65535 && r > 0, "%s: bad sizes nq=%lld b=%d r=%d", name, (long long)nq, b, r);
  QR_CHECK_ARG(part_bits >= 8 && part_bits <= 16, "%s: part_bits=%d not in [8,16]", name, part_bits);
  QR_CHECK_ARG(nq < (1ll << 32), "%s: nq too large", name);
  QR_CHECK_ARG(total_overflow_out && workspace, "%s: null pointer", name);
  if (hipMemsetAsync(total_overflow_out, 0, 2 * sizeof(uint64_t), st) != hipSuccess) {
    qrlsh_set_error("%s: hipMemsetAsync failed", name);
    return QRLSH_EHIP;
  }
  if (nq == 0) return QRLSH_OK;
  QR_CHECK_ARG(keys && part_keys && part_ids, "%s: null pointer", name);
  QR_CHECK_ARG(part_bits == 8 || (tmp_keys && tmp_ids), "%s: part_bits > 8 needs tmp buffers", name);
  if (workspace_bytes < qrlsh_bucket_workspace_bytes(nq, b, part_bits)) {
    qrlsh_set_error("%s: workspace %zu < %zu bytes", name, workspace_bytes,
                    qrlsh_bucket_workspace_bytes(nq, b, part_bits));
    return QRLSH_EWORKSPACE;
  }
  return QRLSH_OK;
}

QRLSH_EXPORT int qrlsh_bucket_pairs_count(const uint64_t *keys, uint64_t *part_keys, uint32_t *part_ids,
                                          uint64_t *tmp_keys, uint32_t *tmp_ids, int64_t nq, int32_t b, int32_t r,
                                          int32_t part_bits, void *workspace, size_t workspace_bytes,
                                          uint64_t *total_overflow_out, void *stream) {
  hipStream_t st = static_cast<hipStream_t>(stream);
  const int rc = bucket_check("qrlsh_bucket_pairs_count", keys, part_keys, part_ids, tmp_keys, tmp_ids, nq, b, r,
                              part_bits, workspace, workspace_bytes, total_overflow_out, st);
  if (rc != QRLSH_OK || nq == 0) return rc;
  const int nparts = 1 << part_bits;
  const uint64_t ek = qr_empty_key(r);
  const BucketWs w = bucket_ws(workspace, nq, b, part_bits);
  bucket_partition(keys, part_keys, part_ids, tmp_keys, tmp_ids, nq, b, r, part_bits, w, st);
  QR_LAUNCH("bucket_count", (bucket_finish_kernel<FIN_COUNT>), dim3(nparts, b), dim3(FIN_THREADS), 0, st,
            (const uint64_t *)part_keys, (const uint32_t *)part_ids, nq, (const uint32_t *)w.starts, nparts, ek, w.blk,
            reinterpret_cast<uint32_t *>(total_overflow_out + 1), (uint64_t *)nullptr, (uint64_t)0);
  QR_LAUNCH("scan_blocks", scan_u64_kernel, dim3(1), dim3(1024), 0, st, w.blk, (int64_t)b * nparts, total_overflow_out);
  QR_LAUNCH_CHECK("qrlsh_bucket_pairs_count");
  return QRLSH_OK;
}

static uint32_t part_region(int64_t nq) {
  const int64_t c = ((nq / RADIX) * 3 / 2 + 512 + 63) / 64 * 64;
  return (uint32_t)(c < FIN_CAP ? c : FIN_CAP);
}

static int coarse_bits(int T) { return (T + 1) / 2; }
static uint32_t coarse_region(int64_t nq, int c1) {
  const double a = (double)nq / (double)(1 << c1);
  const double slack = a >= 4096.0 ? 0.25 * a + 8192.0 : 6.0 * sqrt(a) + 2.0 * a + 64.0;
  return (uint32_t)(((int64_t)(a + slack) + 63) / 64 * 64);
}
static bool small_form(int64_t nq, int T) { return (nq >> T) >= 1024 && (nq >> T) <= FIN_SMALL_MEAN; }
static uint32_t fine_region(int64_t nq, int T) {
  if ((nq >> T) >= 1024) return small_form(nq, T) ? FIN_SMALL_CAP : FIN_CAP;
  const int64_t c = ((nq >> T) * 2 + 128 + 63) / 64 * 64;
  return (uint32_t)(c < FIN_CAP ? c : FIN_CAP);
}
static bool one_kernel_partition(int64_t nq, int part_bits) { return nq < (1ll << 32) && part_bits >= 8; }
static size_t pool_records(int64_t nq, int32_t b) {
  size_t n = (size_t)b * (size_t)nq / 16;
  if (n < ((size_t)1 << 20)) n = (size_t)1 << 20;
  if (n > 0xFFFFFF00ull) n = 0xFFFFFF00ull;
  return n;
}
static size_t region_words(int64_t nq, int32_t b, int32_t part_bits) {
  return part_bits == 8 ? (size_t)b * RADIX * part_region(nq) : ((size_t)b << part_bits) * fine_region(nq, part_bits);
}

QRLSH_EXPORT size_t qrlsh_bucket_part_words(int64_t nq, int32_t b, int32_t part_bits) {
  if (nq <= 0 || b <= 0) return 0;
  const size_t plain = (size_t)b * nq;
  if (!one_kernel_partition(nq, part_bits)) return plain;
  const size_t regions = region_words(nq, b, part_bits) + pool_records(nq, b);
  return regions > plain ? regions : plain;
}
QRLSH_EXPORT size_t qrlsh_bucket_tmp_words(int64_t nq, int32_t b, int32_t part_bits) {
  if (nq <= 0 || b <= 0 || part_bits <= 8) return 0;
  const size_t plain = (size_t)b * nq;
  if (!one_kernel_partition(nq, part_bits)) return plain;
  const int c1 = coarse_bits(part_bits);
  const size_t regions = ((size_t)b << c1) * coarse_region(nq, c1);
  return regions > plain ? regions : plain;
}

QRLSH_EXPORT int qrlsh_bucket_pairs_emit(const uint64_t *keys, uint64_t *part_keys, uint32_t *part_ids,
                                         uint64_t *tmp_keys, uint32_t *tmp_ids, int64_t nq, int32_t b, int32_t r,
                                         int32_t part_bits, void *workspace, size_t workspace_bytes,
                                         uint64_t *pairs_out, uint64_t capacity, uint64_t *total_overflow_out,
                                         void *stream) {
  return qrlsh_bucket_pairs_emit_chunked(keys, 0, 0, 0, part_keys, part_ids, tmp_keys, tmp_ids, nq, b, r, part_bits,
                                         workspace, workspace_bytes, pairs_out, capacity, total_overflow_out, stream);
}

QRLSH_EXPORT int qrlsh_bucket_pairs_emit_chunked(const uint64_t *keys, int64_t key_chunk, int64_t key_chunk_stride,
                                                 int64_t key_band_stride, uint64_t *part_keys, uint32_t *part_ids,
                                                 uint64_t *tmp_keys, uint32_t *tmp_ids, int64_t nq, int32_t b,
                                                 int32_t r, int32_t part_bits, void *workspace,
                                                 size_t workspace_bytes, uint64_t *pairs_out, uint64_t capacity,
                                                 uint64_t *total_overflow_out, void *stream) {
  QR_CHECK_ARG(key_chunk >= 0 && key_chunk_stride >= 0 && key_band_stride >= 0,
               "qrlsh_bucket_pairs_emit_chunked: bad key layout");
  hipStream_t st = static_cast<hipStream_t>(stream);
  const int rc = bucket_check("qrlsh_bucket_pairs_emit", keys, part_keys, part_ids, tmp_keys, tmp_ids, nq, b, r,
                              part_bits, workspace, workspace_bytes, total_overflow_out, st);
  if (rc != QRLSH_OK || nq == 0) return rc;
  QR_CHECK_ARG(pairs_out || capacity == 0, "qrlsh_bucket_pairs_emit: null output with capacity %llu",
               (unsigned long long)capacity);
  const int nparts = 1 << part_bits;
  const BucketWs w = bucket_ws(workspace, nq, b, part_bits);
  const uint64_t ekx = qr_mix64(qr_empty_key(r));
#define QR_PART_SCATTER(LEVEL2_, ...) QR_LAUNCH("part_scatter", (part_scatter_atomic_kernel<LEVEL2_>), __VA_ARGS__)
  if (one_kernel_partition(nq, part_bits)) {
    const int T = part_bits;
    const bool two = T > 8;
    const int c1 = two ? coarse_bits(T) : 8;
    const uint32_t cap1 = two ? coarse_region(nq, c1) : part_region(nq), cap2 = two ? fine_region(nq, T) : cap1;
    const uint32_t lowmask = (1u << (T - c1)) - 1u;
    uint32_t *cur1 = two ? w.ghist : w.starts, *cur2 = w.starts;
    if (hipMemsetAsync(cur1, 0, ((size_t)b << c1) * sizeof(uint32_t), st) != hipSuccess ||
        (two && hipMemsetAsync(cur2, 0, ((size_t)b << T) * sizeof(uint32_t), st) != hipSuccess)) {
      qrlsh_set_error("qrlsh_bucket_pairs_emit: hipMemsetAsync failed");
      return QRLSH_EHIP;
    }
    uint32_t *ovf = reinterpret_cast<uint32_t *>(total_overflow_out + 1);
    const size_t reg_words = region_words(nq, b, T);
    PartPool pool;
    pool.keys = part_keys + reg_words;
    pool.vals = part_ids + reg_words;
    pool.cursor = w.poolctl;
    pool.nruns = w.poolctl + 1;
    pool.cap = (uint32_t)pool_records(nq, b);
    pool.runs = w.runs;
    pool.runs_max = POOL_RUNS;
    pool.fill = w.fill;
    pool.slot_base = 0;
    PartPool no_pool = pool;
    no_pool.keys = nullptr;
    no_pool.vals = nullptr;
    if (hipMemsetAsync(w.fill, 0xFF, ((size_t)b << T) * sizeof(uint32_t), st) != hipSuccess ||
        hipMemsetAsync(w.poolctl, 0, 16, st) != hipSuccess) {
      qrlsh_set_error("qrlsh_bucket_pairs_emit: hipMemsetAsync failed");
      return QRLSH_EHIP;
    }
    constexpr int MAX_GROUPS = EMIT_MAX_GROUPS;
    unsigned long long *nbig0 = reinterpret_cast<unsigned long long *>(w.blk);
    uint64_t *biglist0 = w.blk + MAX_GROUPS;
    const uint64_t slots = (uint64_t)b << T;
    if (hipMemsetAsync(nbig0, 0, MAX_GROUPS * sizeof(unsigned long long), st) != hipSuccess) {
      qrlsh_set_error("qrlsh_bucket_pairs_emit: hipMemsetAsync failed");
      return QRLSH_EHIP;
    }
    const bool small_parts = two && small_form(nq, T);
    const int ntiles = (int)ceil_div64(nq, PS_TILE);
    const int64_t band_words = key_band_stride ? key_band_stride : nq;
    static int groups_env = -1;
    if (groups_env < 0) {
      const char *e = getenv("QRLSH_EMIT_GROUPS");
      groups_env = e ? atoi(e) : 2;
      if (groups_env < 1) groups_env = 1;
    }
    int GROUPS = (int64_t)b * nq >= (64ll << 20) ? groups_env : 1;
    if (GROUPS > MAX_GROUPS) GROUPS = MAX_GROUPS;
    const int per = (b + GROUPS - 1) / GROUPS;
    const int ngroups = (b + per - 1) / per;
    const uint64_t list_room = (slots - MAX_GROUPS) / (uint64_t)ngroups;
    const uint32_t big_max = (uint32_t)(list_room < FIN_BIG_LIST ? list_room : FIN_BIG_LIST);
    if (ngroups > 1 && hipMemsetAsync(w.runs, 0, (size_t)POOL_RUNS * sizeof(uint4), st) != hipSuccess) {
      qrlsh_set_error("qrlsh_bucket_pairs_emit: hipMemsetAsync failed");
      return QRLSH_EHIP;
    }
    hipStream_t aux = nullptr;
    int gi = 0;
    for (int g0 = 0; g0 < b; g0 += per, ++gi) {
      const int nb = (b - g0 < per) ? b - g0 : per;
      hipStream_t s = (aux && (gi & 1)) ? aux : st;
      uint64_t *biglist = biglist0 + (size_t)gi * big_max;
      unsigned long long *nbig = nbig0 + gi;
      uint64_t *k1 = two ? tmp_keys : part_keys;
      uint32_t *v1 = two ? tmp_ids : part_ids;
      pool.slot_base = (uint32_t)((size_t)g0 << T);
      BigDesc *desc = w.desc + (size_t)gi * FIN_BIG_LIST;
      QR_PART_SCATTER(false, dim3(ntiles, nb), dim3(SORT_THREADS), 0, s, keys + (size_t)g0 * band_words,
                      (const uint32_t *)nullptr, k1 + ((size_t)g0 << c1) * cap1, v1 + ((size_t)g0 << c1) * cap1, nq,
                      ntiles, 64 - c1, (1u << c1) - 1u, cur1 + ((size_t)g0 << c1), cap1, ovf, qr_empty_key(r),
                      (const uint32_t *)nullptr, 0u, key_chunk, key_chunk_stride, key_band_stride, two ? no_pool : pool);
      if (two)
        QR_PART_SCATTER(true, dim3((unsigned)ceil_div64(cap1, PS_TILE), nb << c1), dim3(SORT_THREADS), 0, s,
                        (const uint64_t *)tmp_keys + ((size_t)g0 << c1) * cap1,
                        (const uint32_t *)tmp_ids + ((size_t)g0 << c1) * cap1, part_keys + ((size_t)g0 << T) * cap2,
                        part_ids + ((size_t)g0 << T) * cap2, (int64_t)0, 0, 64 - T, lowmask, cur2 + ((size_t)g0 << T),
                        cap2, ovf, qr_empty_key(r), (const uint32_t *)cur1 + ((size_t)g0 << c1), cap1, (int64_t)0,
                        (int64_t)0, (int64_t)0, pool);
      if (gi == 0 && b > per) aux = qr_aux_fork(st);
      if (small_parts && T >= 12 && g_fin_packed)
        QR_LAUNCH("bucket_emit", bucket_finish_packed_kernel, dim3(nparts, nb), dim3(FIN_PK_THREADS), 0, s,
                  (const uint64_t *)part_keys + ((size_t)g0 << T) * cap2, (const uint32_t *)part_ids + ((size_t)g0 << T) * cap2,
                  nparts, total_overflow_out, ovf, pairs_out, capacity, (const uint32_t *)cur2 + ((size_t)g0 << T), cap2, biglist,
                  nbig, big_max, (uint32_t)((size_t)g0 << T));
      else if (small_parts)
        QR_LAUNCH("bucket_emit", (bucket_finish_kernel<FIN_EMIT, FIN_SMALL_THREADS, FIN_SMALL_CAP>), dim3(nparts, nb),
                  dim3(FIN_SMALL_THREADS), 0, s, (const uint64_t *)part_keys + ((size_t)g0 << T) * cap2,
                  (const uint32_t *)part_ids + ((size_t)g0 << T) * cap2, nq, (const uint32_t *)nullptr, nparts, ekx,
                  total_overflow_out, ovf, pairs_out, capacity, (const uint32_t *)cur2 + ((size_t)g0 << T), cap2, biglist, nbig,
                  big_max, (uint32_t)((size_t)g0 << T));
      else
        QR_LAUNCH("bucket_emit", (bucket_finish_kernel<FIN_EMIT>), dim3(nparts, nb), dim3(FIN_THREADS), 0, s,
                  (const uint64_t *)part_keys + ((size_t)g0 << T) * cap2, (const uint32_t *)part_ids + ((size_t)g0 << T) * cap2,
                  nq, (const uint32_t *)nullptr, nparts, ekx, total_overflow_out, ovf, pairs_out, capacity,
                  (const uint32_t *)cur2 + ((size_t)g0 << T), cap2, biglist, nbig, big_max, (uint32_t)((size_t)g0 << T));
      QR_LAUNCH("bucket_emit_big", bucket_big_gather_kernel, dim3(64), dim3(256), 0, s, (const uint64_t *)biglist,
                (const unsigned long long *)nbig, big_max, desc, (const uint64_t *)part_keys, (const uint32_t *)part_ids,
                (const uint32_t *)cur2, cap2, pool, g_big_limit, ovf);
      QR_LAUNCH("bucket_emit_big", bucket_finish_big_kernel, dim3(FIN_BIG_GRID), dim3(FIN_THREADS), 0, s,
                (const uint64_t *)part_keys, (const uint32_t *)part_ids, (const uint64_t *)pool.keys,
                (const uint32_t *)pool.vals, ekx, (const BigDesc *)desc, (const unsigned long long *)nbig, big_max,
                total_overflow_out, pairs_out, capacity);
    }
    if (aux && qr_aux_join(st) != QRLSH_OK) return QRLSH_EHIP;
    QR_LAUNCH_CHECK("qrlsh_bucket_pairs_emit");
    return QRLSH_OK;
  }
#undef QR_PART_SCATTER
  QR_CHECK_ARG(key_chunk == 0, "qrlsh_bucket_pairs_emit_chunked: chunked keys need nq < 2^32");
  bucket_partition(keys, part_keys, part_ids, tmp_keys, tmp_ids, nq, b, r, part_bits, w, st);
  QR_LAUNCH("bucket_emit", (bucket_finish_kernel<FIN_EMIT>), dim3(nparts, b), dim3(FIN_THREADS), 0, st,
            (const uint64_t *)part_keys, (const uint32_t *)part_ids, nq, (const uint32_t *)w.starts, nparts,
            qr_empty_key(r), total_overflow_out, reinterpret_cast<uint32_t *>(total_overflow_out + 1), pairs_out,
            capacity);
  QR_LAUNCH_CHECK("qrlsh_bucket_pairs_emit");
  return QRLSH_OK;
}

QRLSH_EXPORT int qrlsh_bucket_pairs_fill(const uint64_t *part_keys, const uint32_t *part_ids, int64_t nq, int32_t b,
                                         int32_t r, int32_t part_bits, void *workspace, uint64_t *pairs_out,
                                         void *stream) {
  QR_CHECK_ARG(nq >= 0 && b > 0 && r > 0 && part_bits >= 8 && part_bits <= 16,
               "qrlsh_bucket_pairs_fill: bad sizes");
  if (nq == 0) return QRLSH_OK;
  QR_CHECK_ARG(part_keys && part_ids && workspace && pairs_out, "qrlsh_bucket_pairs_fill: null pointer");
  const int nparts = 1 << part_bits;
  const BucketWs w = bucket_ws(workspace, nq, b, part_bits);
  QR_LAUNCH("bucket_fill", (bucket_finish_kernel<FIN_FILL>), dim3(nparts, b), dim3(FIN_THREADS), 0,
            static_cast<hipStream_t>(stream), part_keys, part_ids, nq, (const uint32_t *)w.starts, nparts,
            qr_empty_key(r), w.blk, w.tail, pairs_out, (uint64_t)0);
  QR_LAUNCH_CHECK("qrlsh_bucket_pairs_fill");
  return QRLSH_OK;
}
```

### query-recommendation-system_amd/qrlsh/_lib.py

```python
import ctypes
import os

_HERE = os.path.dirname(os.path.abspath(__file__))
LIB_PATH = os.environ.get("QRLSH_LIB", os.path.join(_HERE, "libqrlsh.so"))

QRLSH_OK = 0
QRLSH_EINVAL = -1
QRLSH_EHIP = -2
QRLSH_EUNSUPPORTED = -3
QRLSH_EWORKSPACE = -4

PERM_U16 = 0
PERM_I32 = 1
SIG_I32 = 0
SIG_U16 = 1
SORT_MIX = 1
SORT_IOTA = 2
SORT_FOLD = 4
SORT_OWNER = 8
SORT_HOST = 16
SUM_PAIRWISE = 0
SUM_SEQUENTIAL = 1
RECOMMEND_MAX_K = 1024

_vp = ctypes.c_void_p
_i32 = ctypes.c_int32
_i64 = ctypes.c_int64
_u32 = ctypes.c_uint32
_u64 = ctypes.c_uint64
_sz = ctypes.c_size_t

SIGNATURES = {
    "qrlsh_version": (ctypes.c_int, []),
    "qrlsh_last_error": (ctypes.c_char_p, []),
    "qrlsh_mix64_host": (_u64, [_u64]),
    "qrlsh_minhash": (ctypes.c_int, [_vp, _vp, _i64, _vp, _i32, _i32, _i32, _i32, _vp, _vp, _vp, _vp, _i32, _vp]),
    "qrlsh_check_csr": (ctypes.c_int, [_vp, _vp, _i64, _i64, _i32, _vp, _vp]),
    "qrlsh_band_keys": (ctypes.c_int, [_vp, _i64, _i32, _i32, _vp, _vp, _vp]),
    "qrlsh_sort_workspace_bytes": (_sz, [_i64, _i32]),
    "qrlsh_sort_u64": (ctypes.c_int, [_vp, _vp, _vp, _vp, _i64, _i32, _i32, _i32, _u32, _u64, _vp, _sz, _vp]),
    "qrlsh_owner_bounds": (ctypes.c_int, [_vp, _i64, _i32, _u64, _i32, _vp, _vp]),
    "qrlsh_pairs_workspace_bytes": (_sz, [_i64, _i32]),
    "qrlsh_pairs_count": (ctypes.c_int, [_vp, _i64, _i32, _i32, _i32, _vp, _sz, _vp, _vp]),
    "qrlsh_pairs_fill": (ctypes.c_int, [_vp, _vp, _i64, _i32, _i32, _i32, _vp, _vp, _vp]),
    "qrlsh_bucket_workspace_bytes": (_sz, [_i64, _i32, _i32]),
    "qrlsh_bucket_pairs_count": (ctypes.c_int, [_vp, _vp, _vp, _vp, _vp, _i64, _i32, _i32, _i32, _vp, _sz, _vp, _vp]),
    "qrlsh_bucket_pairs_fill": (ctypes.c_int, [_vp, _vp, _i64, _i32, _i32, _i32, _vp, _vp, _vp]),
    "qrlsh_bucket_pairs_emit_chunked": (ctypes.c_int, [_vp, _i64, _i64, _i64, _vp, _vp, _vp, _vp, _i64, _i32, _i32, _i32, _vp, _sz, _vp, _u64, _vp, _vp]),
    "qrlsh_bucket_part_words": (_sz, [_i64, _i32, _i32]),
    "qrlsh_set_big_part_limit": (_i64, [_i64]),
    "qrlsh_set_score_runs": (_i32, [_i32]),
    "qrlsh_bucket_tmp_words": (_sz, [_i64, _i32, _i32]),
    "qrlsh_bucket_pairs_emit": (ctypes.c_int, [_vp, _vp, _vp, _vp, _vp, _i64, _i32, _i32, _i32, _vp, _sz, _vp, _u64, _vp, _vp]),
    "qrlsh_compact_workspace_bytes": (_sz, [_i64]),
    "qrlsh_row_unique_workspace_bytes": (_sz, [_i64]),
    "qrlsh_row_unique_count": (ctypes.c_int, [_vp, _i64, _i32, _i32, _vp, _vp, _sz, _vp, _vp]),
    "qrlsh_row_unique_fill": (ctypes.c_int, [_vp, _i64, _vp, _vp, _vp]),
    "qrlsh_region_unique_workspace_bytes": (_sz, [_i64, _i32]),
    "qrlsh_region_unique_count": (ctypes.c_int, [_vp, _i64, _i32, _i32, _i64, _vp, _vp, _sz, _vp, _vp]),
    "qrlsh_region_unique_fill": (ctypes.c_int, [_vp, _i64, _i32, _i64, _vp, _vp, _vp]),
    "qrlsh_region_unique_count_regions": (ctypes.c_int, [_vp, _vp, _i64, _i64, _i32, _i32, _i64, _vp, _vp, _sz, _vp, _vp]),
    "qrlsh_pair_regions_words": (_sz, [_i64, _i64, _i32, ctypes.c_double]),
    "qrlsh_pair_regions_tmp_words": (_sz, [_i64, _i64, _i32, ctypes.c_double]),
    "qrlsh_pair_regions_cap": (_i64, [_i64, _i64, _i32, ctypes.c_double]),
    "qrlsh_pair_regions_count": (_i64, [_i64, _i64, _i32, ctypes.c_double]),
    "qrlsh_pair_regions_scatter": (ctypes.c_int, [_vp, _i64, _i32, _i64, ctypes.c_double, _vp, _vp, _vp, _vp, _vp]),
    "qrlsh_unique_count": (ctypes.c_int, [_vp, _i64, _vp, _sz, _vp, _vp]),
    "qrlsh_unique_fill": (ctypes.c_int, [_vp, _i64, _vp, _vp, _vp]),
    "qrlsh_row_norms": (ctypes.c_int, [_vp, _i64, _i32, _vp, _vp]),
    "qrlsh_verify_pairs": (ctypes.c_int, [_vp, _i32, _i32, _i32, _vp, _i64, _vp, _vp]),
    "qrlsh_score_pairs": (ctypes.c_int, [_vp, _i32, _vp, _i32, _vp, _i64, _vp, _vp, _vp, _i32, _vp, _vp]),
    "qrlsh_remap_pairs": (ctypes.c_int, [_vp, _i64, _i64, _i64, _vp, _i64, _vp, _vp]),
    "qrlsh_pair_edges": (ctypes.c_int, [_vp, _vp, _i64, _i32, _vp, _vp, _vp, _vp, _vp]),
    "qrlsh_topk_count": (ctypes.c_int, [_vp, _i64, _i32, _i32, _vp, _sz, _vp, _vp]),
    "qrlsh_topk_fill": (ctypes.c_int, [_vp, _vp, _i64, _i32, _i32, _vp, _vp, _vp, _vp, _vp]),
    "qrlsh_topk_fill_based": (ctypes.c_int, [_vp, _vp, _i64, _i32, _i32, _i64, _vp, _vp, _vp, _vp, _vp]),
    "qrlsh_score_pairs_rev": (ctypes.c_int, [_vp, _i32, _vp, _i32, _vp, _i64, _vp, _vp, _i32, _vp, _vp]),
    "qrlsh_topk_select_workspace_bytes": (_sz, [_i64]),
    "qrlsh_topk_select_count": (ctypes.c_int, [_vp, _i64, _vp, _vp, _i64, _i32, _i32, _vp, _sz, _vp, _vp]),
    "qrlsh_topk_select_fill": (ctypes.c_int, [_vp, _vp, _i64, _vp, _vp, _i64, _i32, _i32, _vp, _vp, _vp, _vp, _vp]),
    "qrlsh_idset_workspace_bytes": (_sz, [_i64]),
    "qrlsh_idset_build": (ctypes.c_int, [_vp, _i64, _i64, _i64, _i64, _i64, _i32, _vp, _sz, _vp, _vp]),
    "qrlsh_idset_list": (ctypes.c_int, [_vp, _i64, _vp, _vp]),
    "qrlsh_idset_remap": (ctypes.c_int, [_vp, _i64, _i64, _i64, _vp, _i64, _vp, _vp]),
    "qrlsh_gather_rows": (ctypes.c_int, [_vp, _i64, _vp, _vp, _i64, _i64, _vp, _vp, _vp]),
    "qrlsh_score_pairs_split": (ctypes.c_int, [_vp, _vp, _i64, _vp, _vp, _i32, _i32, _vp, _i64, _vp, _vp]),
    "qrlsh_edges_localize": (ctypes.c_int, [_vp, _vp, _i64, _i32, _i64, _i64, _vp, _vp]),
    "qrlsh_answer_sets_count": (ctypes.c_int, [_vp, _i64, _i64, _vp, _i64, _i32, _vp, _vp]),
    "qrlsh_answer_sets_fill": (ctypes.c_int, [_vp, _i64, _i64, _vp, _i64, _i32, _vp, _vp, _vp]),
    "qrlsh_answer_sets_sweep": (ctypes.c_int, [_vp, _i64, _i64, _vp, _i64, _i32, _vp, _vp, _vp]),
    "qrlsh_answer_sets_compact": (ctypes.c_int, [_vp, _vp, _i64, _vp, _vp]),
    "qrlsh_predict_workspace_bytes": (_sz, [_i64, _i64, _i32]),
    "qrlsh_predict": (ctypes.c_int, [_vp, _i64, _i64, _vp, _vp, _vp, _vp, _vp, _i32, ctypes.c_double, ctypes.c_double,
                                     ctypes.c_double, _i32, _vp, _vp, _i32, _vp, _sz, _vp]),
    "qrlsh_recommend_workspace_bytes": (_sz, [_i64, _i64, _i32, _i32]),
    "qrlsh_recommend_topk": (ctypes.c_int, [_vp, _vp, _i64, _i64, _vp, _i64, _i32, _i32, _i32, _vp, _vp, _vp, _vp, _sz,
                                            _vp]),
    "qrlsh_center_rows": (ctypes.c_int, [_vp, _i64, _i64, _i64, _vp, _vp]),
    "qrlsh_user_gram_workspace_bytes": (_sz, [_i64, _i64]),
    "qrlsh_user_gram": (ctypes.c_int, [_vp, _i64, _i64, _vp, _vp, _vp, _vp, _sz, _vp]),
    "qrlsh_gather_sets_workspace_bytes": (_sz, [_i64]),
    "qrlsh_gather_sets_count": (ctypes.c_int, [_vp, _i64, _vp, _i32, _i64, _i64, _vp, _vp, _sz, _vp]),
    "qrlsh_gather_sets_fill": (ctypes.c_int, [_vp, _i64, _vp, _i32, _vp, _i32, _i64, _i64, _vp, _vp, _vp]),
    "qrlsh_prof_enable": (ctypes.c_int, [ctypes.c_int]),
    "qrlsh_set_overlap": (ctypes.c_int, [ctypes.c_int]),
    "qrlsh_prof_pause": (ctypes.c_int, [ctypes.c_int]),
    "qrlsh_prof_report": (ctypes.c_int, [ctypes.c_char_p, _sz]),
    "qrlsh_synth_sizes": (ctypes.c_int, [_u64, _i64, _i64, _i64, _i32, _u32, _vp, _i32, _u32, _vp, _vp]),
    "qrlsh_synth_fill": (ctypes.c_int, [_u64, _i64, _i64, _i64, _i32, _u32, _vp, _i32, _u32, _vp, _vp, _vp]),
}


class QrlshError(RuntimeError):
    def __init__(self, code, msg):
        super().__init__("libqrlsh error %d: %s" % (code, msg))
        self.code = code


_lib = None


def load():
    global _lib
    if _lib is not None:
        return _lib
    if not os.path.exists(LIB_PATH):
        raise ImportError(
            "libqrlsh.so not found at %s -- the HIP extension is required (there is no CPU fallback). "
            "Build it with: make -C query-recommendation-system_amd/csrc" % LIB_PATH)
    lib = ctypes.CDLL(LIB_PATH)
    for name, (res, args) in SIGNATURES.items():
        fn = getattr(lib, name)
        fn.restype = res
        fn.argtypes = args
    _lib = lib
    return lib


def check(rc):
    if rc < 0:
        msg = load().qrlsh_last_error().decode("utf-8", "replace")
        if rc == QRLSH_EUNSUPPORTED:
            raise NotImplementedError("libqrlsh: " + msg)
        raise QrlshError(rc, msg)
    return rc


def prof_enable(on=True):
    check(load().qrlsh_prof_enable(1 if on else 0))


def prof_pause(paused=True):
    check(load().qrlsh_prof_pause(1 if paused else 0))


def prof_report():
    buf = ctypes.create_string_buffer(1 << 16)
    check(load().qrlsh_prof_report(buf, len(buf)))
    out = {}
    for line in buf.value.decode().splitlines():
        name, cnt, ms = line.split()
        out[name] = (int(cnt), float(ms))
    return out
```

### query-recommendation-system_amd/qrlsh/ops.py

```python
import ctypes

import numpy as np
import torch

from . import _lib

_vp = ctypes.c_void_p


def _stream():
    return _vp(torch.cuda.current_stream().cuda_stream)


def _ptr(t):
    if t is None:
        return None
    return _vp(t.data_ptr())


def _need(t, dtype, name, ndim=None):
    if not isinstance(t, torch.Tensor) or not t.is_cuda:
        raise TypeError("%s must be a CUDA/HIP tensor" % name)
    if t.dtype != dtype:
        raise TypeError("%s must have dtype %s, got %s" % (name, dtype, t.dtype))
# ... 239 lines not shown
    ib = id_bits_for(nq)
    p, _ = sort_u64(pairs, None, 0, 2 * ib, fold=ib)
    return p


def row_group_bits(id_bits, words_per_row=0.0):
    g = id_bits % 8
    if not (id_bits > 8 and 0 < g <= 4):
        return 0
    return g if words_per_row * (1 << g) <= 1024 else 0


def group_pairs_by_i(pairs, nq, group_bits=0):
    p, _ = sort_u64(pairs, None, 32 + group_bits, 32 + id_bits_for(nq))
    return p


def row_unique(grouped, group_bits=0, id_bits=32):
    lib = _lib.load()
    _need(grouped, torch.int64, "grouped", 1)
    n = grouped.numel()
    if n == 0:
        return grouped
    dev = grouped.device
    tmp = torch.empty_like(grouped)
    ws = _ws(lib.qrlsh_row_unique_workspace_bytes(n), dev)
    tot = torch.empty(2, dtype=torch.int64, device=dev)
    _lib.check(lib.qrlsh_row_unique_count(_ptr(grouped), n, int(group_bits), int(id_bits), _ptr(tmp), _ptr(ws),
                                          ws.numel(), _ptr(tot), _stream()))
    total, overflow = tot.tolist()
    if overflow:
        return None
    out = torch.empty((total,), dtype=torch.int64, device=dev)
    _lib.check(lib.qrlsh_row_unique_fill(_ptr(tmp), n, _ptr(ws), _ptr(out), _stream()))
    return out


def region_group_bits(id_bits, nids, words_per_query=0.0):
    g = min(8, 32 - id_bits, id_bits)
    if g + id_bits == 32 and nids >= (1 << id_bits):
        g -= 1
    while g > 0 and words_per_query * (1 << g) > 16384:
        g -= 1
    return g if g >= 3 else None


def region_unique(grouped, group_bits, id_bits, nids):
    lib = _lib.load()
    _need(grouped, torch.int64, "grouped", 1)
    n = grouped.numel()
    if n == 0:
        return grouped
    dev = grouped.device
    tmp = torch.empty_like(grouped)
    ws = _ws(lib.qrlsh_region_unique_workspace_bytes(nids, group_bits), dev)
    tot = torch.empty(2, dtype=torch.int64, device=dev)
    _lib.check(lib.qrlsh_region_unique_count(_ptr(grouped), n, int(group_bits), int(id_bits), int(nids), _ptr(tmp), _ptr(ws),
                                             ws.numel(), _ptr(tot), _stream()))
    total, overflow = tot.tolist()
    if overflow:
        return None
    out = torch.empty((total,), dtype=torch.int64, device=dev)
    _lib.check(lib.qrlsh_region_unique_fill(_ptr(tmp), n, int(group_bits), int(nids), _ptr(ws), _ptr(out), _stream()))
    return out


REGION_MIN_GROUP_BITS = 6
REGION_SCATTER_MAX_BYTES = 48 << 30


def region_unique_scattered(emitted, group_bits, id_bits, nids, words_per_query=0.0):
    lib = _lib.load()
    _need(emitted, torch.int64, "emitted", 1)
    n = emitted.numel()
    if n == 0:
        return emitted, ""
    dev = emitted.device
    wpq = float(words_per_query)
    words = lib.qrlsh_pair_regions_words(n, nids, group_bits, wpq)
    twords = lib.qrlsh_pair_regions_tmp_words(n, nids, group_bits, wpq)
    if words == 0 or n >= (1 << 32) or (2 * words + twords) * 8 > REGION_SCATTER_MAX_BYTES:
        return None, "cap"
    cap = lib.qrlsh_pair_regions_cap(n, nids, group_bits, wpq)
    nreg = lib.qrlsh_pair_regions_count(n, nids, group_bits, wpq)
    try:
        regions = torch.empty((words,), dtype=torch.int64, device=dev)
        tmpr = torch.empty((twords,), dtype=torch.int64, device=dev) if twords else None
        tmp = torch.empty_like(regions)
    except torch.cuda.OutOfMemoryError:
        regions = tmpr = tmp = None
        torch.cuda.empty_cache()
        return None, "cap"
    counts = torch.empty((nreg + 256,), dtype=torch.int32, device=dev)
    ovf = torch.empty((1,), dtype=torch.int32, device=dev)
    _lib.check(lib.qrlsh_pair_regions_scatter(_ptr(emitted), n, int(group_bits), int(nids), wpq, _ptr(tmpr), _ptr(regions),
                                              _ptr(counts), _ptr(ovf), _stream()))
    del tmpr
    ws = _ws(lib.qrlsh_region_unique_workspace_bytes(nids, group_bits), dev)
    tot = torch.empty(2, dtype=torch.int64, device=dev)
    _lib.check(lib.qrlsh_region_unique_count_regions(_ptr(regions), _ptr(counts), cap, n, int(group_bits), int(id_bits),
                                                     int(nids), _ptr(tmp), _ptr(ws), ws.numel(), _ptr(tot), _stream()))
    total, overflow = tot.tolist()
    if int(ovf.item()):
        return None, "cap"
    if overflow:
        return None, "distinct"
    del regions
    out = torch.empty((total,), dtype=torch.int64, device=dev)
    _lib.check(lib.qrlsh_region_unique_fill(_ptr(tmp), n, int(group_bits), int(nids), _ptr(ws), _ptr(out), _stream()))
    return out, ""


def unique_pairs(emitted, nq, stats=None, words_per_query=None, scatter=True):
    ib = id_bits_for(nq)
    wpq = emitted.numel() / max(nq, 1) if words_per_query is None else words_per_query
    g = region_group_bits(ib, nq, wpq)
    pairs = None
    if g is not None and g < REGION_MIN_GROUP_BITS:
        grouped, g = emitted, 0
    elif g is not None:
        path, why = "regions-in-lds", "cap"
        if scatter:
            pairs, why = region_unique_scattered(emitted, g, ib, nq, wpq)
            path = "regions-in-lds (scattered)"
        if pairs is None and why == "distinct":
            grouped = emitted
        elif pairs is None:
            grouped = group_pairs_by_i(emitted, nq, g)
            pairs = region_unique(grouped, g, ib, nq)
            path = "regions-in-lds"
    else:
        g = row_group_bits(ib, wpq)
        grouped = group_pairs_by_i(emitted, nq, g)
        pairs = row_unique(grouped, g, ib)
        path = "rows-in-lds"
    if stats is not None:
        stats["dedup_path"] = path if pairs is not None else "full-sort"
        stats["group_bits"] = g
    if pairs is None:
        pairs = unique_sorted(sort_pairs(grouped, nq))
    return pairs


def part_bits_for(n):
    t = 8
    while t < 16 and n > 4400 * (1 << t):
        t += 1
    return t


_EMIT_HINT = {}


def emit_pairs_fast(keys, r, part_bits=None, one_pass=True, capacity=None, chunks=None):
    lib = _lib.load()
    if chunks is not None:
        world, b, nql = chunks[:3]
        stride = chunks[3] if len(chunks) > 3 else b * nql
        nq = world * nql
        _need(keys, torch.int64, "keys")
        if stride < b * nql or keys.numel() < (world - 1) * stride + b * nql or not one_pass:
            raise ValueError("chunked keys: need (world - 1) * stride + nb * nql words and the one-pass form")
        layout = (nql, stride, nql)
    else:
        _need(keys, torch.int64, "keys", 2)
        b, nq = keys.shape
        layout = (0, 0, 0)
    dev = keys.device
    T = part_bits if part_bits is not None else part_bits_for(nq)
    if nq > 6144 * (1 << T):
        return None
    words = lib.qrlsh_bucket_part_words(nq, b, T) if one_pass else b * nq
    pk = torch.empty((words,), dtype=torch.int64, device=dev)
    pid = torch.empty((words,), dtype=torch.int32, device=dev)
    twords = (lib.qrlsh_bucket_tmp_words(nq, b, T) if one_pass else b * nq) if T > 8 else 0
    tk = torch.empty((twords,), dtype=torch.int64, device=dev) if T > 8 else None
    tid = torch.empty((twords,), dtype=torch.int32, device=dev) if T > 8 else None
    ws = _ws(lib.qrlsh_bucket_workspace_bytes(nq, b, T), dev)
    tot = torch.zeros(2, dtype=torch.int64, device=dev)
    if one_pass:
        shape = (nq, b, r)
        if capacity is None:
            capacity = _EMIT_HINT[shape] * 5 // 4 + 1024 if shape in _EMIT_HINT else 24 * nq + 1024
        while True:
            pairs = torch.empty((capacity,), dtype=torch.int64, device=dev)
            _lib.check(lib.qrlsh_bucket_pairs_emit_chunked(_ptr(keys), layout[0], layout[1], layout[2], _ptr(pk),
                                                           _ptr(pid), _ptr(tk), _ptr(tid), nq, b, r, T, _ptr(ws),
                                                           ws.numel(), _ptr(pairs), capacity, _ptr(tot), _stream()))
            n, overflow = tot.tolist()
            if overflow:
                return None
            _EMIT_HINT[shape] = n
            if n <= capacity:
                return pairs[:n]
            del pairs
            capacity = n
    _lib.check(lib.qrlsh_bucket_pairs_count(_ptr(keys), _ptr(pk), _ptr(pid), _ptr(tk), _ptr(tid), nq, b, r, T,
                                            _ptr(ws), ws.numel(), _ptr(tot), _stream()))
    n, overflow = tot.tolist()
    if overflow:
        return None
    del tk, tid
    pairs = torch.empty((n,), dtype=torch.int64, device=dev)
    if n:
        _lib.check(lib.qrlsh_bucket_pairs_fill(_ptr(pk), _ptr(pid), nq, b, r, T, _ptr(ws), _ptr(pairs), _stream()))
    return pairs


def emit_pairs_any(keys, r, stats=None):
    emitted = emit_pairs_fast(keys, r)
    if stats is not None:
        stats["bucket_path"] = "partition+lds" if emitted is not None else "general-sort"
        stats["part_bits"] = part_bits_for(keys.shape[1])
    if emitted is None:
        sk, sid = bucket_sort(keys)
        emitted = emit_pairs(sk, sid, r)
    return emitted


def verify_pairs(sig, b, pairs):
    lib = _lib.load()
    if not isinstance(sig, torch.Tensor) or sig.dtype not in (torch.int32, torch.int16):
        raise TypeError("sig must be an int32 or int16 (compact) tensor")
    _need(sig, sig.dtype, "sig", 2)
    _need(pairs, torch.int64, "pairs", 1)
    n = pairs.numel()
    flags = torch.empty((n,), dtype=torch.uint8, device=sig.device)
    code = _lib.SIG_U16 if sig.dtype == torch.int16 else _lib.SIG_I32
    _lib.check(lib.qrlsh_verify_pairs(_ptr(sig), code, sig.shape[1], b, _ptr(pairs), n, _ptr(flags), _stream()))
    return flags


def drop_unverified(sig, b, pairs, stats=None):
    if pairs.numel() == 0:
        return pairs
    flags = verify_pairs(sig, b, pairs)
    bad = int((flags == 0).sum().item())
    if stats is not None:
        stats["hash_collision_pairs_dropped"] = bad
    return pairs if bad == 0 else pairs[flags.bool()]


def candidate_pairs(keys, r, stats=None, sig=None):
    b, nq = keys.shape
    if r > 4 and sig is None:
        raise ValueError("band width r=%d > 4 needs the signatures for exact verification" % r)
    emitted = emit_pairs_any(keys, r, stats)
    if stats is not None:
        stats["emitted_pairs"] = int(emitted.numel())
    if emitted.numel() == 0:
        return emitted
    pairs = unique_pairs(emitted, nq, stats)
    if r > 4:
        pairs = drop_unverified(sig, b, pairs, stats)
    return pairs


def wide_ids(id_bits):
    return 2 * id_bits + 11 > 64


def score_pairs(sig, norm2, pairs, want_cos=False, edge_id_bits=None, wide=None):
    lib = _lib.load()
    if not isinstance(sig, torch.Tensor) or sig.dtype not in (torch.int32, torch.int16):
        raise TypeError("sig must be an int32 or int16 (compact) tensor")
    _need(sig, sig.dtype, "sig", 2)
    if norm2 is not None:
        _need(norm2, torch.int64, "norm2", 1)
    _need(pairs, torch.int64, "pairs", 1)
    n = pairs.numel()
    dev = sig.device
    milli = torch.empty((n,), dtype=torch.int32, device=dev)
    cosv = torch.empty((n,), dtype=torch.float64, device=dev) if want_cos else None
    edges = torch.empty((2 * n,), dtype=torch.int64, device=dev) if edge_id_bits is not None else None
    if wide is None:
        wide = edge_id_bits is not None and wide_ids(edge_id_bits)
    edst = torch.empty((2 * n,), dtype=torch.int32, device=dev) if (wide and edges is not None) else None
    code = _lib.SIG_U16 if sig.dtype == torch.int16 else _lib.SIG_I32
    _lib.check(lib.qrlsh_score_pairs(_ptr(sig), code, _ptr(norm2), sig.shape[1], _ptr(pairs), n, _ptr(milli),
                                     _ptr(cosv), _ptr(edges), edge_id_bits if edge_id_bits is not None else 0,
                                     _ptr(edst), _stream()))
    return milli, cosv, ((edges, edst) if edst is not None else edges)


class RemoteIds:

    def __init__(self, ws, nids, q0, nql, bounds):
        self.ws, self.nids, self.q0, self.nql, self.bounds = ws, nids, q0, nql, bounds


def remote_ids(pairs, q0, nql, nids, world):
    lib = _lib.load()
    _need(pairs, torch.int64, "pairs", 1)
    dev = pairs.device
    ws = _ws(lib.qrlsh_idset_workspace_bytes(nids), dev)
    bounds = torch.empty((world + 1,), dtype=torch.int64, device=dev)
    _lib.check(lib.qrlsh_idset_build(_ptr(pairs), pairs.numel(), int(q0), int(nql), int(nids), int(nql), world,
                                     _ptr(ws), ws.numel(), _ptr(bounds), _stream()))
    return RemoteIds(ws, nids, q0, nql, bounds)


def remote_id_list(rid, total):
    lib = _lib.load()
    out = torch.empty((total,), dtype=torch.int64, device=rid.ws.device)
    if total:
        _lib.check(lib.qrlsh_idset_list(_ptr(rid.ws), rid.nids, _ptr(out), _stream()))
    return out


def remap_pairs_ids(pairs, rid):
    lib = _lib.load()
    _need(pairs, torch.int64, "pairs", 1)
    out = torch.empty_like(pairs)
    _lib.check(lib.qrlsh_idset_remap(_ptr(pairs), pairs.numel(), int(rid.q0), int(rid.nql), _ptr(rid.ws), rid.nids,
                                     _ptr(out), _stream()))
    return out


def gather_rows(sig, norm2, ids, q0):
    lib = _lib.load()
    _need(ids, torch.int64, "ids", 1)
    n = ids.numel()
    rows = torch.empty((n, sig.shape[1]), dtype=sig.dtype, device=sig.device)
    norms = torch.empty((n,), dtype=torch.int64, device=sig.device)
    _lib.check(lib.qrlsh_gather_rows(_ptr(sig), sig.shape[1] * sig.element_size(), _ptr(norm2), _ptr(ids), n, int(q0),
                                     _ptr(rows), _ptr(norms), _stream()))
    return rows, norms


def gather_sets(ids, offs_all, rows_all, nql):
    lib = _lib.load()
    _need(ids, torch.int64, "ids", 1)
    if offs_all.dtype not in (torch.int32, torch.int64) or rows_all.dtype not in (torch.int16, torch.int32):
        raise TypeError("offs_all must be int32 / int64, rows_all int16 / int32")
    _need(offs_all, offs_all.dtype, "offs_all", 2)
    _need(rows_all, rows_all.dtype, "rows_all", 2)
    world, max_nnz = rows_all.shape
    if tuple(offs_all.shape) != (world, nql + 1):
        raise ValueError("offs_all must be [world, nql + 1]")
    n, dev = ids.numel(), ids.device
    off = torch.empty((n + 1,), dtype=torch.int64, device=dev)
    ws = _ws(lib.qrlsh_gather_sets_workspace_bytes(n), dev)
    _lib.check(lib.qrlsh_gather_sets_count(_ptr(ids), n, _ptr(offs_all), offs_all.element_size(), int(nql), world, _ptr(off),
                                           _ptr(ws), ws.numel(), _stream()))
    total = int(off[-1].item())
    rows = torch.empty((total,), dtype=torch.int32, device=dev)
    if total:
        _lib.check(lib.qrlsh_gather_sets_fill(_ptr(ids), n, _ptr(offs_all), offs_all.element_size(), _ptr(rows_all),
                                              rows_all.element_size(), int(nql), max_nnz, _ptr(off), _ptr(rows), _stream()))
    return off, rows


def score_pairs_split(sig, norm2, sig_b, norm2_b, pairs):
    lib = _lib.load()
    _need(pairs, torch.int64, "pairs", 1)
    n = pairs.numel()
    milli = torch.empty((n,), dtype=torch.int32, device=pairs.device)
    code = _lib.SIG_U16 if sig.dtype == torch.int16 else _lib.SIG_I32
    _lib.check(lib.qrlsh_score_pairs_split(_ptr(sig), _ptr(norm2), sig.shape[0], _ptr(sig_b), _ptr(norm2_b), code,
                                           sig.shape[1], _ptr(pairs), n, _ptr(milli), _stream()))
    return milli


def pair_edges_interleaved(pairs, milli, id_bits, wide=False):
    lib = _lib.load()
    n, dev = pairs.numel(), pairs.device
    e = torch.empty((2 * n,), dtype=torch.int64, device=dev)
    d = torch.empty((2 * n,), dtype=torch.int32, device=dev) if wide else None
    _lib.check(lib.qrlsh_pair_edges(_ptr(pairs), _ptr(milli), n, 0 if wide else int(id_bits), _ptr(e), None, _ptr(d),
                                    None, _stream()))
    return (e, d) if wide else e


def local_bits_for(nql):
    return max(1, int(nql - 1).bit_length()) if nql > 1 else 1


def topk_edges_local(edges, edst, K, id_bits, q0, nql, select=True):
    lib = _lib.load()
    dev = edges.device
    n = edges.numel()
    if n == 0:
        z = torch.empty((0,), dtype=torch.int32, device=dev)
        return z, z.clone(), z.clone()
    lb = local_bits_for(nql)
    if lb + 11 + id_bits > 64:
        raise NotImplementedError("%d local + %d global id bits do not fit the 64-bit top-K key" % (lb, id_bits))
    loc = torch.empty_like(edges)
    _lib.check(lib.qrlsh_edges_localize(_ptr(edges), _ptr(edst), n, id_bits, int(q0), int(nql), _ptr(loc), _stream()))
    if select and K <= SELECT_MAX_K and n < (1 << 31):
        src, dst, val = topk_select(None, None, loc, K, id_bits, int(nql))
        src += int(q0)
        return src, dst, val
    se, _ = sort_u64(loc, None, 0, lb + 11 + id_bits)
    ws = _ws(lib.qrlsh_compact_workspace_bytes(n), dev)
    total = torch.zeros(1, dtype=torch.int64, device=dev)
    _lib.check(lib.qrlsh_topk_count(_ptr(se), n, K, id_bits, _ptr(ws), ws.numel(), _ptr(total), _stream()))
    m = int(total.item())
    src = torch.empty((m,), dtype=torch.int32, device=dev)
    dst = torch.empty((m,), dtype=torch.int32, device=dev)
    val = torch.empty((m,), dtype=torch.int32, device=dev)
    _lib.check(lib.qrlsh_topk_fill_based(_ptr(se), None, n, K, id_bits, int(q0), _ptr(ws), _ptr(src), _ptr(dst),
                                         _ptr(val), _stream()))
    return src, dst, val


def score_pairs_rev(sig, norm2, pairs, id_bits, wide=None):
    lib = _lib.load()
    _need(sig, sig.dtype, "sig", 2)
    if norm2 is not None:
        _need(norm2, torch.int64, "norm2", 1)
    _need(pairs, torch.int64, "pairs", 1)
    n, dev = pairs.numel(), sig.device
    if wide is None:
        wide = wide_ids(id_bits)
    milli = torch.empty((n,), dtype=torch.int32, device=dev)
    rev = torch.empty((n,), dtype=torch.int64, device=dev)
    rdst = torch.empty((n,), dtype=torch.int32, device=dev) if wide else None
    code = _lib.SIG_U16 if sig.dtype == torch.int16 else _lib.SIG_I32
    _lib.check(lib.qrlsh_score_pairs_rev(_ptr(sig), code, _ptr(norm2), sig.shape[1], _ptr(pairs), n, _ptr(milli), _ptr(rev),
                                         0 if wide else int(id_bits), _ptr(rdst), _stream()))
    return milli, ((rev, rdst) if wide else rev)


SELECT_MAX_K = 256


def topk_select(pairs, milli, rev, K, id_bits, nq):
    lib = _lib.load()
    rdst = None
    if isinstance(rev, tuple):
        rev, rdst = rev
    dev = rev.device
    n = rev.numel()
    if n == 0:
        z = torch.empty((0,), dtype=torch.int32, device=dev)
        return z, z.clone(), z.clone()
    if K > SELECT_MAX_K:
        raise ValueError("topk_select handles K <= %d; use topk_edges (the sort form) beyond" % SELECT_MAX_K)
    if rdst is None:
        src_bits = id_bits if pairs is not None else local_bits_for(nq)
        rs, rd = sort_u64(rev, None, id_bits + 11, id_bits + 11 + src_bits)
    else:
        rs, rd = sort_u64(rev, rdst, 11, 11 + id_bits)
    ws = _ws(lib.qrlsh_topk_select_workspace_bytes(nq), dev)
    total = torch.zeros(1, dtype=torch.int64, device=dev)
    _lib.check(lib.qrlsh_topk_select_count(_ptr(pairs), n, _ptr(rs), _ptr(rd), int(nq), K, int(id_bits), _ptr(ws), ws.numel(),
                                           _ptr(total), _stream()))
    m = int(total.item())
    src = torch.empty((m,), dtype=torch.int32, device=dev)
    dst = torch.empty((m,), dtype=torch.int32, device=dev)
    val = torch.empty((m,), dtype=torch.int32, device=dev)
    _lib.check(lib.qrlsh_topk_select_fill(_ptr(pairs), _ptr(milli), n, _ptr(rs), _ptr(rd), int(nq), K, int(id_bits), _ptr(ws),
                                          _ptr(src), _ptr(dst), _ptr(val), _stream()))
    return src, dst, val


def remap_pairs(pairs, q0, nql, need):
    lib = _lib.load()
    _need(pairs, torch.int64, "pairs", 1)
    _need(need, torch.int64, "need", 1)
    out = torch.empty_like(pairs)
    _lib.check(lib.qrlsh_remap_pairs(_ptr(pairs), pairs.numel(), int(q0), int(nql), _ptr(need), need.numel(),
                                     _ptr(out), _stream()))
    return out


def pair_edges(pairs, milli, id_bits, wide=False):
    lib = _lib.load()
    _need(pairs, torch.int64, "pairs", 1)
    _need(milli, torch.int32, "milli", 1)
    n, dev = pairs.numel(), pairs.device
    fwd = torch.empty((n,), dtype=torch.int64, device=dev)
    rev = torch.empty((n,), dtype=torch.int64, device=dev)
    fd = torch.empty((n,), dtype=torch.int32, device=dev) if wide else None
    rd = torch.empty((n,), dtype=torch.int32, device=dev) if wide else None
    _lib.check(lib.qrlsh_pair_edges(_ptr(pairs), _ptr(milli), n, 0 if wide else int(id_bits), _ptr(fwd), _ptr(rev),
                                    _ptr(fd), _ptr(rd), _stream()))
    return ((fwd, fd), (rev, rd)) if wide else (fwd, rev)


def topk_edges(edges, K, id_bits):
    lib = _lib.load()
    edst = None
    if isinstance(edges, tuple):
        edges, edst = edges
    _need(edges, torch.int64, "edges", 1)
    dev = edges.device
    n = edges.numel()
    if n == 0:
        z = torch.empty((0,), dtype=torch.int32, device=dev)
        return z, z.clone(), z.clone()
    if edst is None:
        se, sd = sort_u64(edges, None, id_bits, 2 * id_bits + 11)
        kb = id_bits
    else:
        se, sd = sort_u64(edges, edst, 0, id_bits + 11)
        kb = 0
    ws = _ws(lib.qrlsh_compact_workspace_bytes(n), dev)
    total = torch.zeros(1, dtype=torch.int64, device=dev)
    _lib.check(lib.qrlsh_topk_count(_ptr(se), n, K, kb, _ptr(ws), ws.numel(), _ptr(total), _stream()))
    m = int(total.item())
    src = torch.empty((m,), dtype=torch.int32, device=dev)
    dst = torch.empty((m,), dtype=torch.int32, device=dev)
    val = torch.empty((m,), dtype=torch.int32, device=dev)
    _lib.check(lib.qrlsh_topk_fill(_ptr(se), _ptr(sd), n, K, kb, _ptr(ws), _ptr(src), _ptr(dst), _ptr(val), _stream()))
    return src, dst, val
```

### query-recommendation-system_amd/qrlsh/pipeline.py

```python
import math
import time
from dataclasses import dataclass, field

import numpy as np
import torch

from . import ops


def max_candidates(nq):
    return round(math.log(nq, 1.5))


def select_bands(P, thresh=0.2):
    for b in range(P, 0, -1):
        if P % b == 0 and b % 10 == 0:
            r = P / b
            if round((1 / b) ** (1 / r), 2) >= thresh:
                return b
    raise ValueError("no band count satisfies the reference rule for PERM=%d; pass b explicitly" % P)


@dataclass
class HotPathResult:
    sig: torch.Tensor
    norm2: torch.Tensor
    pairs: torch.Tensor
    milli: torch.Tensor
    src: torch.Tensor
    dst: torch.Tensor
    val: torch.Tensor
    K: int = 0
    b: int = 0
    stats: dict = field(default_factory=dict)

    def sig_int32(self):
        return ops.sig_to_int32(self.sig)


def query_similarities(offsets, rows, table, b, K, timings=None, compact=None, wide_ids=None, topk="select",
                       validate=True):
    nq = offsets.numel() - 1
    P = table.P
    if P % b != 0:
        raise AssertionError("signature length %d not divisible by b=%d" % (P, b))
    r = P // b
    stats = {}

    def tick(name, t0):
        if timings is not None:
            torch.cuda.synchronize()
            timings[name] = timings.get(name, 0.0) + (time.perf_counter() - t0)
            return time.perf_counter()
        return t0

    t0 = time.perf_counter() if timings is not None else 0.0
    if compact is None:
        compact = ops.can_compact(table)
    sig, norm2, keys = ops.minhash(offsets, rows, table, b=b, want_norm=True, compact=compact, validate=validate)
    t0 = tick("signatures", t0)
    pairs = ops.candidate_pairs(keys, r, stats, sig=sig)
    del keys
    t0 = tick("candidates", t0)
    ib = ops.id_bits_for(nq)
    if topk == "select" and (K > ops.SELECT_MAX_K or pairs.numel() >= (1 << 31)):
        topk = "sort"
    if topk == "select":
        milli, rev = ops.score_pairs_rev(sig, norm2, pairs, ib, wide=wide_ids)
        t0 = tick("scoring", t0)
        src, dst, val = ops.topk_select(pairs, milli, rev, K, ib, nq)
    else:
        milli, _, edges = ops.score_pairs(sig, norm2, pairs, edge_id_bits=ib, wide=wide_ids)
        t0 = tick("scoring", t0)
        src, dst, val = ops.topk_edges(edges, K, ib)
    tick("topk", t0)
    stats["topk"] = topk
    stats["unique_pairs"] = int(pairs.numel())
    stats["kept_edges"] = int(src.numel())
    return HotPathResult(sig, norm2, pairs, milli, src, dst, val, K, b, stats)


def sims_to_dict(src, dst, val):
    src, dst, val = ops.to_host(src), ops.to_host(dst), ops.to_host(val)
    out = {}
    if len(src) == 0:
        return out
    cut = np.flatnonzero(np.diff(src)) + 1
    starts = np.concatenate(([0], cut))
    ends = np.concatenate((cut, [len(src)]))
    for s, e in zip(starts, ends):
        out[int(src[s])] = {"indexes": dst[s:e].astype(np.int64), "values": val[s:e].astype(np.float64) / 1000.0}
    return out
```

Baseline: 603.6 million.

## Pack bucket partition records into 8 bytes and verify candidate bands during scoring

Adds a packed bucket-partition path that folds the record id into the low bits of the hashed key, so partition records take 8 bytes instead of 12. This removes the separate value array and its traffic. Because the truncated hash can yield false candidate pairs, the scoring kernel now checks that at least one band matches exactly. It marks pairs that fail, counts them atomically, and a three-kernel compaction then drops them before top-K. This trades cheaper partitioning for extra scoring-time checks, three compaction launches, and atomic contention.

```diff
diff --git a/include/qrlsh.h b/include/qrlsh.h
--- a/include/qrlsh.h
+++ b/include/qrlsh.h
@@ -79,6 +79,13 @@
                                     int32_t part_bits, void *workspace, size_t workspace_bytes,
                                     uint64_t *pairs_out, uint64_t capacity, uint64_t *total_overflow_out,
                                     void *stream);
+
+int qrlsh_bucket_pairs_emit_packed(const uint64_t *keys, uint64_t *part_words, uint64_t *tmp_words, int64_t nq,
+                                   int32_t b, int32_t r, int32_t part_bits, int32_t id_bits, void *workspace,
+                                   size_t workspace_bytes, uint64_t *pairs_out, uint64_t capacity,
+                                   uint64_t *total_overflow_out, void *stream);
+int qrlsh_set_packed_records(int on);
+int qrlsh_set_packed_hash_bits(int bits);
 
 size_t qrlsh_compact_workspace_bytes(int64_t n);
 int qrlsh_unique_count(const uint64_t *sorted, int64_t n, void *workspace, size_t workspace_bytes,
@@ -129,6 +136,12 @@
 int qrlsh_score_pairs_rev(const void *sig, int32_t sig_dtype, const int64_t *norm2, int32_t P,
                           const uint64_t *pairs, int64_t n, int32_t *milli_out, uint64_t *rev_out, int32_t id_bits,
                           uint32_t *rev_dst_out, void *stream);
+int qrlsh_score_pairs_rev_checked(const void *sig, const int64_t *norm2, int32_t P, int32_t b, const uint64_t *pairs,
+                                  int64_t n, int32_t *milli_out, uint64_t *rev_out, int32_t id_bits,
+                                  unsigned long long *false_count, void *stream);
+size_t qrlsh_drop_marked_workspace_bytes(int64_t n);
+int qrlsh_drop_marked_pairs(uint64_t *pairs, int32_t *milli, int64_t n, const unsigned long long *false_count,
+                            void *workspace, size_t workspace_bytes, void *stream);
 int qrlsh_set_score_runs(int on);
 size_t qrlsh_topk_select_workspace_bytes(int64_t nq);
 int qrlsh_topk_select_count(const uint64_t *pairs, int64_t n, const uint64_t *rev_sorted, const uint32_t *rev_dst,
diff --git a/query-recommendation-system_amd/csrc/score.hip b/query-recommendation-system_amd/csrc/score.hip
--- a/query-recommendation-system_amd/csrc/score.hip
+++ b/query-recommendation-system_amd/csrc/score.hip
@@ -154,6 +154,13 @@
   const uint32_t hi = (uint32_t)__builtin_amdgcn_update_dpp(0, (int)(uint32_t)(v >> 32), CTRL, 0xF, 0xF, false);
   return v + (((uint64_t)hi << 32) | lo);
 }
+__device__ static inline uint32_t row_or_u32(uint32_t v) {
+  v |= (uint32_t)__builtin_amdgcn_update_dpp(0, (int)v, 0xB1, 0xF, 0xF, false);
+  v |= (uint32_t)__builtin_amdgcn_update_dpp(0, (int)v, 0x4E, 0xF, 0xF, false);
+  v |= (uint32_t)__builtin_amdgcn_update_dpp(0, (int)v, 0x141, 0xF, 0xF, false);
+  v |= (uint32_t)__builtin_amdgcn_update_dpp(0, (int)v, 0x140, 0xF, 0xF, false);
+  return v;
+}
 __device__ static inline uint64_t row_sum_u64(uint64_t v) {
   v = dpp_add_u64<0xB1>(v);
   v = dpp_add_u64<0x4E>(v);
@@ -193,14 +200,16 @@
 #ifndef QR_SCORE_OCC2
 #define QR_SCORE_OCC2 5
 #endif
-template <int CH>
+template <int CH, bool CHECK = false>
 __global__ __launch_bounds__(256, CH == 1 ? QR_SCORE_OCC : QR_SCORE_OCC2) void score_runs_kernel(const uint16_t *__restrict__ sig, const int64_t *__restrict__ norm2,
                                                          const uint64_t *__restrict__ pairs, int64_t n,
                                                          int32_t *__restrict__ milli, double *__restrict__ cosv,
                                                          uint64_t *__restrict__ edges, int id_bits,
                                                          uint32_t *__restrict__ edge_dst,
                                                          const uint16_t *__restrict__ sig_b,
-                                                         const int64_t *__restrict__ norm2_b, uint32_t split, int rev_only) {
+                                                         const int64_t *__restrict__ norm2_b, uint32_t split, int rev_only,
+                                                         unsigned long long *__restrict__ false_count = nullptr) {
+  static_assert(!CHECK || CH == 1, "the band test is written for rows of 128 values");
   constexpr int P = CH * 128;
   constexpr int NB = SCORE_PF + 1;
   const int lig = threadIdx.x & (SCORE_LPP - 1);
@@ -226,6 +235,7 @@
       nb = my_j < split ? norm2[my_j] : norm2_b[my_j - split];
     }
     uint64_t my_dot = 0;
+    uint32_t hits = 0;
     u16x8 ab[NB][CH], cb[NB][CH];
 #define QR_ROW_I(U) row_bcast_u32<(U)>(my_i)
 #define QR_ROW_J(U) row_bcast_u32<(U)>(my_j)
@@ -263,6 +273,13 @@
       _Pragma("unroll") for (int k = 0; k < CH; ++k) part += chunk_dot(ab[(U) % NB][k], cb[(U) % NB][k]); \
       const uint64_t tot = row_sum_u64(part);                                               \
       if (lig == (U)) my_dot = tot;                                                         \
+      if (CHECK) {                                                                          \
+        const u32x4 aw = __builtin_bit_cast(u32x4, ab[(U) % NB][0]), cw = __builtin_bit_cast(u32x4, cb[(U) % NB][0]); \
+        const bool b0 = aw[0] == cw[0] && aw[1] == cw[1] && (aw[0] & aw[1]) != 0xFFFFFFFFu;  \
+        const bool b1 = aw[2] == cw[2] && aw[3] == cw[3] && (aw[2] & aw[3]) != 0xFFFFFFFFu;  \
+        hits |= (uint32_t)(b0 || b1) << (U);                                                \
+        asm volatile("" : "+v"(hits));   \
+      }                                                                                     \
       asm volatile("" : "+v"(my_dot));     \
       __builtin_amdgcn_sched_barrier(0);  \
     }
@@ -272,7 +289,13 @@
 #undef QR_REQ
 #undef QR_ROW_I
 #undef QR_ROW_J
-    if (live) {
+    bool shares = true;
+    if (CHECK) shares = (row_or_u32(hits) >> lig) & 1u;
+    if (CHECK && live && !shares) {
+      milli[t] = -1;
+      edges[t] = ((((uint64_t)1 << id_bits) - 1u) << (id_bits + 11)) | my_i;
+      atomicAdd(false_count, 1ull);
+    } else if (live) {
       const int64_t dot = (int64_t)my_dot;
       double cs = 0.0;
       if (na != 0 && nb != 0) cs = (double)dot / (sqrt((double)na) * sqrt((double)nb));
@@ -386,6 +409,143 @@
                       rev_dst_out, stream, 1);
 }
 
+QRLSH_EXPORT int qrlsh_score_pairs_rev_checked(const void *sig, const int64_t *norm2, int32_t P, int32_t b,
+                                               const uint64_t *pairs, int64_t n, int32_t *milli_out, uint64_t *rev_out,
+                                               int32_t id_bits, unsigned long long *false_count, void *stream) {
+  QR_CHECK_ARG(n >= 0 && P == 128 && b == 32 && id_bits > 0 && id_bits <= 26,
+               "qrlsh_score_pairs_rev_checked: serves P = 128, b = 32, id_bits in [1,26] (n=%lld P=%d b=%d id_bits=%d)",
+               (long long)n, P, b, id_bits);
+  if (n == 0) return QRLSH_OK;
+  QR_CHECK_ARG(sig && norm2 && pairs && milli_out && rev_out && false_count, "qrlsh_score_pairs_rev_checked: null pointer");
+  QR_CHECK_ARG(((uintptr_t)sig & 15) == 0, "qrlsh_score_pairs_rev_checked: rows must be 16-byte aligned");
+  const int64_t rb = ceil_div64(ceil_div64(n, SCORE_LPP), 256 / SCORE_LPP);
+  QR_CHECK_ARG(rb <= 2147483647ll, "qrlsh_score_pairs_rev_checked: too many pairs for one launch");
+  QR_LAUNCH("score_pairs", (score_runs_kernel<1, true>), dim3((unsigned)rb), dim3(256), 0, static_cast<hipStream_t>(stream),
+            static_cast<const uint16_t *>(sig), norm2, pairs, n, milli_out, (double *)nullptr, rev_out, id_bits,
+            (uint32_t *)nullptr, (const uint16_t *)nullptr, (const int64_t *)nullptr, 0xFFFFFFFFu, 1, false_count);
+  QR_LAUNCH_CHECK("qrlsh_score_pairs_rev_checked");
+  return QRLSH_OK;
+}
+
+constexpr int DROP_IPT = 16, DROP_TILE = 256 * DROP_IPT, DROP_GRID = 2048;
+__device__ static inline void drop_range(int64_t n, int64_t &t0, int64_t &t1) {
+  const int64_t ntiles = (n + DROP_TILE - 1) / DROP_TILE, per = (ntiles + gridDim.x - 1) / gridDim.x;
+  t0 = min((int64_t)blockIdx.x * per, ntiles);
+  t1 = min(t0 + per, ntiles);
+}
+__global__ __launch_bounds__(256) void drop_count_kernel(const int32_t *__restrict__ milli, int64_t n,
+                                                         const unsigned long long *__restrict__ false_count,
+                                                         uint32_t *__restrict__ bcnt) {
+  __shared__ uint32_t wsum[4];
+  if (*false_count == 0) return;
+  int64_t t0, t1;
+  drop_range(n, t0, t1);
+  uint32_t c = 0;
+  for (int64_t tile = t0; tile < t1; ++tile)
+#pragma unroll
+    for (int k = 0; k < DROP_IPT; ++k) {
+      const int64_t i = tile * DROP_TILE + k * 256 + threadIdx.x;
+      c += i < n && milli[i] < 0;
+    }
+  for (int d = 32; d > 0; d >>= 1) c += __shfl_xor(c, d, WAVE);
+  if ((threadIdx.x & (WAVE - 1)) == 0) wsum[threadIdx.x >> 6] = c;
+  __syncthreads();
+  if (threadIdx.x == 0) bcnt[blockIdx.x] = wsum[0] + wsum[1] + wsum[2] + wsum[3];
+}
+__global__ __launch_bounds__(256) void drop_scatter_kernel(const uint64_t *__restrict__ pairs,
+                                                           const int32_t *__restrict__ milli, int64_t n,
+                                                           const unsigned long long *__restrict__ false_count,
+                                                           const uint32_t *__restrict__ bcnt, uint64_t *__restrict__ tpairs,
+                                                           int32_t *__restrict__ tmilli) {
+  __shared__ uint32_t part[DROP_IPT * 4];
+  __shared__ uint32_t wsum[4];
+  if (*false_count == 0) return;
+  const int tid = threadIdx.x, lane = tid & (WAVE - 1), w = tid >> 6;
+  int64_t t0, t1;
+  drop_range(n, t0, t1);
+  uint32_t before = 0;
+  for (uint32_t g = tid; g < blockIdx.x; g += 256) before += bcnt[g];
+  for (int d = 32; d > 0; d >>= 1) before += __shfl_xor(before, d, WAVE);
+  if (lane == 0) wsum[w] = before;
+  __syncthreads();
+  int64_t out = t0 * DROP_TILE - (int64_t)(wsum[0] + wsum[1] + wsum[2] + wsum[3]);
+  for (int64_t tile = t0; tile < t1; ++tile) {
+    bool keep[DROP_IPT];
+    uint32_t below[DROP_IPT];
+#pragma unroll
+    for (int k = 0; k < DROP_IPT; ++k) {
+      const int64_t i = tile * DROP_TILE + k * 256 + tid;
+      keep[k] = i < n && milli[i] >= 0;
+      const uint64_t m = __ballot(keep[k]);
+      below[k] = __popcll(m & ((1ull << lane) - 1ull));
+      if (lane == 0) part[k * 4 + w] = (uint32_t)__popcll(m);
+    }
+    __syncthreads();
+    if (w == 0) {
+      const uint32_t v = part[lane];
+      uint32_t inc = v;
+      for (int d = 1; d < WAVE; d <<= 1) {
+        const uint32_t o = __shfl_up(inc, d, WAVE);
+        if (lane >= d) inc += o;
+      }
+      part[lane] = inc - v;
+      if (lane == WAVE - 1) wsum[0] = inc;
+    }
+    __syncthreads();
+#pragma unroll
+    for (int k = 0; k < DROP_IPT; ++k)
+      if (keep[k]) {
+        const int64_t i = tile * DROP_TILE + k * 256 + tid, o = out + part[k * 4 + w] + below[k];
+        tpairs[o] = pairs[i];
+        tmilli[o] = milli[i];
+      }
+    out += wsum[0];
+    __syncthreads();
+  }
+}
+__global__ __launch_bounds__(256) void drop_copy_kernel(uint64_t *__restrict__ pairs, int32_t *__restrict__ milli, int64_t n,
+                                                        const unsigned long long *__restrict__ false_count,
+                                                        const uint64_t *__restrict__ tpairs,
+                                                        const int32_t *__restrict__ tmilli) {
+  const unsigned long long f = *false_count;
+  if (f == 0) return;
+  const int64_t kept = n - (int64_t)f;
+  for (int64_t i = (int64_t)blockIdx.x * 256 + threadIdx.x; i < n; i += (int64_t)gridDim.x * 256) {
+    pairs[i] = i < kept ? tpairs[i] : ~0ull;
+    milli[i] = i < kept ? tmilli[i] : -1;
+  }
+}
+
+QRLSH_EXPORT size_t qrlsh_drop_marked_workspace_bytes(int64_t n) {
+  if (n <= 0) return 64;
+  return ((size_t)n * 12 + 15) / 16 * 16 + (size_t)DROP_GRID * sizeof(uint32_t);
+}
+QRLSH_EXPORT int qrlsh_drop_marked_pairs(uint64_t *pairs, int32_t *milli, int64_t n,
+                                         const unsigned long long *false_count, void *workspace, size_t workspace_bytes,
+                                         void *stream) {
+  QR_CHECK_ARG(n >= 0 && n < (1ll << 40), "qrlsh_drop_marked_pairs: bad size n=%lld", (long long)n);
+  if (n == 0) return QRLSH_OK;
+  QR_CHECK_ARG(pairs && milli && false_count && workspace, "qrlsh_drop_marked_pairs: null pointer");
+  if (workspace_bytes < qrlsh_drop_marked_workspace_bytes(n)) {
+    qrlsh_set_error("qrlsh_drop_marked_pairs: workspace %zu < %zu bytes", workspace_bytes,
+                    qrlsh_drop_marked_workspace_bytes(n));
+    return QRLSH_EWORKSPACE;
+  }
+  hipStream_t st = static_cast<hipStream_t>(stream);
+  uint64_t *tp = static_cast<uint64_t *>(workspace);
+  int32_t *tm = reinterpret_cast<int32_t *>(tp + n);
+  uint32_t *bcnt = reinterpret_cast<uint32_t *>(static_cast<char *>(workspace) + ((size_t)n * 12 + 15) / 16 * 16);
+  const int64_t ntiles = ceil_div64(n, DROP_TILE);
+  const dim3 grid((unsigned)(ntiles < DROP_GRID ? ntiles : DROP_GRID)), blk(256);
+  QR_LAUNCH("drop_marked", drop_count_kernel, grid, blk, 0, st, (const int32_t *)milli, n, false_count, bcnt);
+  QR_LAUNCH("drop_marked", drop_scatter_kernel, grid, blk, 0, st, (const uint64_t *)pairs, (const int32_t *)milli, n,
+            false_count, (const uint32_t *)bcnt, tp, tm);
+  QR_LAUNCH("drop_marked", drop_copy_kernel, dim3(DROP_GRID), blk, 0, st, pairs, milli, n, false_count,
+            (const uint64_t *)tp, (const int32_t *)tm);
+  QR_LAUNCH_CHECK("qrlsh_drop_marked_pairs");
+  return QRLSH_OK;
+}
+
 QRLSH_EXPORT int qrlsh_score_pairs_split(const void *sig, const int64_t *norm2, int64_t split_rows, const void *sig_b,
                                          const int64_t *norm2_b, int32_t sig_dtype, int32_t P, const uint64_t *pairs,
                                          int64_t n, int32_t *milli_out, void *stream) {
diff --git a/query-recommendation-system_amd/csrc/sort.hip b/query-recommendation-system_amd/csrc/sort.hip
--- a/query-recommendation-system_amd/csrc/sort.hip
+++ b/query-recommendation-system_amd/csrc/sort.hip
@@ -483,19 +483,22 @@
 constexpr int PS_IPT = QR_PS_IPT;
 constexpr int PS_TILE = SORT_THREADS * PS_IPT;
 constexpr int PS_WGS = PS_IPT <= 16 ? 3 : 2;
-template <bool LEVEL2>
-__global__ __launch_bounds__(SORT_THREADS, PS_WGS) void part_scatter_atomic_kernel(
+constexpr int PS_WGS_PACKED = PS_IPT <= 16 ? 4 : 2;
+template <bool LEVEL2, bool PACKED = false>
+__global__ __launch_bounds__(SORT_THREADS, PACKED ? PS_WGS_PACKED : PS_WGS) void part_scatter_atomic_kernel(
     const uint64_t *__restrict__ keys_in, const uint32_t *__restrict__ vals_in, uint64_t *__restrict__ keys_out,
     uint32_t *__restrict__ vals_out, int64_t n_in, int ntiles, int shift, uint32_t dmask,
     uint32_t *__restrict__ cursors, uint32_t cap, uint32_t *__restrict__ overflow, uint64_t ek,
     const uint32_t *__restrict__ in_counts, uint32_t in_cap, int64_t chunk_len, int64_t chunk_stride,
-    int64_t band_stride, PartPool pool) {
+    int64_t band_stride, PartPool pool, uint64_t hmask = 0) {
   __shared__ uint32_t cnt[RADIX];
   __shared__ uint32_t lsum[SORT_THREADS / WAVE];
   __shared__ uint32_t gdelta[RADIX];
   __shared__ uint8_t gok[RADIX];
+  constexpr bool DIG = PACKED && !LEVEL2;
   __shared__ uint64_t skey[PS_TILE];
-  __shared__ uint32_t sval[PS_TILE];
+  __shared__ uint32_t sval[PACKED ? 1 : PS_TILE];
+  __shared__ uint8_t sdig[DIG ? PS_TILE : 1];
   const int tile = LEVEL2 ? (int)blockIdx.x : xcd_tile(blockIdx.x, ntiles), batch = blockIdx.y;
   const int lane = threadIdx.x & (WAVE - 1), w = threadIdx.x >> 6;
   const int64_t n = LEVEL2 ? (int64_t)min(in_counts[batch], in_cap) : n_in;
@@ -515,7 +518,7 @@
     const int64_t idx = wbase + (int64_t)k * WAVE + lane;
     const size_t at = chunked ? boff + (size_t)(idx / chunk_len) * chunk_stride + (size_t)(idx % chunk_len) : boff + idx;
     key[k] = idx < n ? keys_in[at] : ek;
-    val[k] = LEVEL2 ? (idx < n ? vals_in[boff + idx] : 0u) : (uint32_t)idx;
+    val[k] = LEVEL2 ? (PACKED || idx >= n ? 0u : vals_in[boff + idx]) : (uint32_t)idx;
   }
 #pragma unroll
   for (int k = 0; k < PS_IPT; ++k) {
@@ -549,8 +552,13 @@
   for (int k = 0; k < PS_IPT; ++k) {
     if (dr[k] != 0xFFFFFFFFu) {
       const uint32_t lp = cnt[dr[k] >> 16] + (dr[k] & 0xFFFFu);
-      skey[lp] = key[k];
-      sval[lp] = val[k];
+      if (DIG) {
+        skey[lp] = (key[k] << (64 - shift) & hmask) | val[k];
+        sdig[lp] = (uint8_t)(dr[k] >> 16);
+      } else {
+        skey[lp] = key[k];
+        if (!PACKED) sval[lp] = val[k];
+      }
     }
   }
   {
@@ -587,16 +595,16 @@
     const uint32_t p = k * SORT_THREADS + threadIdx.x;
     if (p < nstaged) {
       const uint64_t x = skey[p];
-      const uint32_t d = (uint32_t)(x >> shift) & dmask;
+      const uint32_t d = DIG ? (uint32_t)sdig[p] : (uint32_t)(x >> shift) & dmask;
       const uint32_t where = gok[d];
       if (where == 1u) {
         const size_t dst = obase + (uint32_t)(gdelta[d] + p);
         keys_out[dst] = x;
-        vals_out[dst] = sval[p];
+        if (!PACKED) vals_out[dst] = sval[p];
       } else if (where == 2u) {
         const uint32_t dst = gdelta[d] + p;
         pool.keys[dst] = x;
-        pool.vals[dst] = sval[p];
+        if (!PACKED) pool.vals[dst] = sval[p];
       }
     }
   }
@@ -1116,11 +1124,24 @@
 }
 
 constexpr int FIN_PK_THREADS = 512, FIN_PK_CAP = 4096, FIN_PK_MAX = 4095;
+template <bool PACKED>
+__device__ static inline void load_record(const uint64_t *k, const uint32_t *id, size_t i, int ib, uint64_t &key,
+                                          uint32_t &rid) {
+  if (PACKED) {
+    const uint64_t w = k[i];
+    key = w >> ib;
+    rid = (uint32_t)w & ((1u << ib) - 1u);
+  } else {
+    key = k[i];
+    rid = id[i];
+  }
+}
+template <bool PACKED = false>
 __global__ __launch_bounds__(FIN_PK_THREADS, 8) void bucket_finish_packed_kernel(
     const uint64_t *__restrict__ keys, const uint32_t *__restrict__ ids, int nparts, uint64_t *__restrict__ blk,
     uint32_t *__restrict__ overflow, uint64_t *__restrict__ out, uint64_t capacity, const uint32_t *__restrict__ counts,
     uint32_t cap, uint64_t *__restrict__ biglist, unsigned long long *__restrict__ nbig, uint32_t big_max,
-    uint32_t big_base) {
+    uint32_t big_base, int ib = 0) {
   constexpr int THREADS = FIN_PK_THREADS, CAP = FIN_PK_CAP, IPT = CAP / THREADS;
   constexpr unsigned long long KMASK = (1ull << 52) - 1ull, ONE = 1ull << 52;
   __shared__ unsigned long long gbase;
@@ -1145,14 +1166,15 @@
   if (m == 0) return;
   const size_t first = bslot * cap;
   const uint64_t *k = keys + first;
-  const uint32_t *id = ids + first;
+  const uint32_t *id = PACKED ? nullptr : ids + first;
   uint64_t kreg[IPT];
   uint32_t ireg[IPT];
 #pragma unroll
   for (int j = 0; j < IPT; ++j) {
     const uint32_t i = tid + j * THREADS;
-    kreg[j] = i < m ? k[i] : 0ull;
-    ireg[j] = i < m ? id[i] : 0u;
+    kreg[j] = 0ull;
+    ireg[j] = 0u;
+    if (i < m) load_record<PACKED>(k, id, i, ib, kreg[j], ireg[j]);
   }
 #pragma unroll
   for (int j = 0; j < IPT; ++j) tab[tid + j * THREADS] = 0ull;
@@ -1262,6 +1284,7 @@
   uint32_t m, pool;
 };
 
+template <bool PACKED = false>
 __global__ __launch_bounds__(256) void bucket_big_gather_kernel(const uint64_t *__restrict__ biglist,
                                                                 const unsigned long long *__restrict__ nbig, uint32_t big_max,
                                                                 BigDesc *__restrict__ desc, const uint64_t *__restrict__ part_keys,
@@ -1303,7 +1326,7 @@
     }
     for (uint32_t i = tid; i < f; i += blockDim.x) {
       pool.keys[base + i] = part_keys[(size_t)slot * cap + i];
-      pool.vals[base + i] = part_ids[(size_t)slot * cap + i];
+      if (!PACKED) pool.vals[base + i] = part_ids[(size_t)slot * cap + i];
     }
     uint32_t at = f;
     unsigned long long nr = *pool.nruns;
@@ -1321,7 +1344,7 @@
         if (at + run.y <= m)
           for (uint32_t i = tid; i < run.y; i += blockDim.x) {
             pool.keys[base + at + i] = pool.keys[(size_t)run.z + i];
-            pool.vals[base + at + i] = pool.vals[(size_t)run.z + i];
+            if (!PACKED) pool.vals[base + at + i] = pool.vals[(size_t)run.z + i];
           }
         at += run.y;
       }
@@ -1333,10 +1356,11 @@
   }
 }
 
+template <bool PACKED = false>
 __global__ __launch_bounds__(FIN_THREADS) void bucket_finish_big_kernel(
     const uint64_t *__restrict__ keys, const uint32_t *__restrict__ ids, const uint64_t *pool_keys, const uint32_t *pool_ids,
     uint64_t ek, const BigDesc *__restrict__ desc, const unsigned long long *__restrict__ nbig, uint32_t big_max,
-    uint64_t *__restrict__ blk, uint64_t *__restrict__ out, uint64_t capacity) {
+    uint64_t *__restrict__ blk, uint64_t *__restrict__ out, uint64_t capacity, int ib = 0) {
   __shared__ unsigned long long gbase;
   __shared__ __attribute__((aligned(16))) unsigned long long tab[FIN_CAP];
   __shared__ uint32_t cnt[FIN_CAP + 1];
@@ -1381,7 +1405,7 @@
     const BigDesc de = desc[e];
     const uint32_t m = de.m;
     const uint64_t *k = (de.pool ? pool_keys : keys) + de.where;
-    const uint32_t *id = (de.pool ? pool_ids : ids) + de.where;
+    const uint32_t *id = PACKED ? nullptr : (de.pool ? pool_ids : ids) + de.where;
     const uint32_t nblk = (m + FIN_CAP - 1) / FIN_CAP;
     if (bi >= nblk) continue;
     {
@@ -1392,8 +1416,9 @@
 #pragma unroll
       for (int j = 0; j < FIN_IPT; ++j) {
         const uint32_t i = tid + j * FIN_THREADS;
-        kreg[j] = i < mb ? k[lo + i] : ek;
-        ireg[j] = i < mb ? id[lo + i] : 0u;
+        kreg[j] = ek;
+        ireg[j] = 0u;
+        if (i < mb) load_record<PACKED>(k, id, lo + i, ib, kreg[j], ireg[j]);
         tab[i] = ek;
         cnt[i] = 0;
       }
@@ -1481,8 +1506,8 @@
 #pragma unroll
         for (int j = 0; j < FIN_IPT; ++j) {
           const uint32_t i = tid + j * FIN_THREADS;
-          const uint64_t x = k[lo2 + i];
-          ireg[j] = id[lo2 + i];
+          uint64_t x;
+          load_record<PACKED>(k, id, lo2 + i, ib, x, ireg[j]);
           uint32_t slot = fin_home(x), found = 0xFFFFFFFFu;
           const bool my_slice = (uint32_t)(tid & (FIN_BIG_SLICES - 1)) == sl;
           for (int step = 0; my_slice && step < FIN_CAP; ++step) {
@@ -1525,6 +1550,22 @@
   const char *e = getenv("QRLSH_FIN_PACKED");
   return !(e && e[0] == '0') ? 1 : 0;
 }();
+
+static int g_packed_records = [] {
+  const char *e = getenv("QRLSH_PACKED_RECORDS");
+  return !(e && e[0] == '0') ? 1 : 0;
+}();
+static int g_packed_hash_bits = 0;
+QRLSH_EXPORT int qrlsh_set_packed_records(int on) {
+  const int old = g_packed_records;
+  if (on >= 0) g_packed_records = on != 0;
+  return old;
+}
+QRLSH_EXPORT int qrlsh_set_packed_hash_bits(int bits) {
+  const int old = g_packed_hash_bits;
+  g_packed_hash_bits = bits > 0 ? bits : 0;
+  return old;
+}
 
 static uint32_t g_big_limit = (uint32_t)FIN_BIG_BLOCKS * FIN_CAP;
 QRLSH_EXPORT int64_t qrlsh_set_big_part_limit(int64_t records) {
@@ -1709,6 +1750,138 @@
   return regions > plain ? regions : plain;
 }
 
+template <bool PACKED>
+static int bucket_emit_regions(const uint64_t *keys, int64_t key_chunk, int64_t key_chunk_stride, int64_t key_band_stride,
+                               uint64_t *part_keys, uint32_t *part_ids, uint64_t *tmp_keys, uint32_t *tmp_ids, int64_t nq,
+                               int32_t b, int32_t r, int32_t part_bits, const BucketWs &w, int ib, uint64_t *pairs_out,
+                               uint64_t capacity, uint64_t *total_overflow_out, hipStream_t st) {
+  const int nparts = 1 << part_bits;
+  const uint64_t ekx = PACKED ? ~0ull : qr_mix64(qr_empty_key(r));
+#define QR_PART_SCATTER(LEVEL2_, ...) QR_LAUNCH("part_scatter", (part_scatter_atomic_kernel<LEVEL2_, PACKED>), __VA_ARGS__)
+  const int T = part_bits;
+  const bool two = T > 8;
+  const int c1 = two ? coarse_bits(T) : 8;
+  const uint32_t cap1 = two ? coarse_region(nq, c1) : part_region(nq), cap2 = two ? fine_region(nq, T) : cap1;
+  const uint32_t lowmask = (1u << (T - c1)) - 1u;
+  uint32_t *cur1 = two ? w.ghist : w.starts, *cur2 = w.starts;
+  if (hipMemsetAsync(cur1, 0, ((size_t)b << c1) * sizeof(uint32_t), st) != hipSuccess ||
+      (two && hipMemsetAsync(cur2, 0, ((size_t)b << T) * sizeof(uint32_t), st) != hipSuccess)) {
+    qrlsh_set_error("qrlsh_bucket_pairs_emit: hipMemsetAsync failed");
+    return QRLSH_EHIP;
+  }
+  uint32_t *ovf = reinterpret_cast<uint32_t *>(total_overflow_out + 1);
+  const size_t reg_words = region_words(nq, b, T);
+  PartPool pool;
+  pool.keys = part_keys + reg_words;
+  pool.vals = PACKED ? nullptr : part_ids + reg_words;
+  pool.cursor = w.poolctl;
+  pool.nruns = w.poolctl + 1;
+  pool.cap = (uint32_t)pool_records(nq, b);
+  pool.runs = w.runs;
+  pool.runs_max = POOL_RUNS;
+  pool.fill = w.fill;
+  pool.slot_base = 0;
+  PartPool no_pool = pool;
+  no_pool.keys = nullptr;
+  no_pool.vals = nullptr;
+  if (hipMemsetAsync(w.fill, 0xFF, ((size_t)b << T) * sizeof(uint32_t), st) != hipSuccess ||
+      hipMemsetAsync(w.poolctl, 0, 16, st) != hipSuccess) {
+    qrlsh_set_error("qrlsh_bucket_pairs_emit: hipMemsetAsync failed");
+    return QRLSH_EHIP;
+  }
+  constexpr int MAX_GROUPS = EMIT_MAX_GROUPS;
+  unsigned long long *nbig0 = reinterpret_cast<unsigned long long *>(w.blk);
+  uint64_t *biglist0 = w.blk + MAX_GROUPS;
+  const uint64_t slots = (uint64_t)b << T;
+  if (hipMemsetAsync(nbig0, 0, MAX_GROUPS * sizeof(unsigned long long), st) != hipSuccess) {
+    qrlsh_set_error("qrlsh_bucket_pairs_emit: hipMemsetAsync failed");
+    return QRLSH_EHIP;
+  }
+  const bool small_parts = two && small_form(nq, T);
+  uint64_t hmask = 0;
+  if (PACKED) {
+    int kb = g_packed_hash_bits > 0 && g_packed_hash_bits < 64 - ib ? g_packed_hash_bits : 64 - ib;
+    if (kb < T - c1) kb = T - c1;
+    hmask = ~0ull << (64 - kb);
+  }
+  const int ntiles = (int)ceil_div64(nq, PS_TILE);
+  const int64_t band_words = key_band_stride ? key_band_stride : nq;
+  static int groups_env = -1;
+  if (groups_env < 0) {
+    const char *e = getenv("QRLSH_EMIT_GROUPS");
+    groups_env = e ? atoi(e) : 2;
+    if (groups_env < 1) groups_env = 1;
+  }
+  int GROUPS = (int64_t)b * nq >= (64ll << 20) ? groups_env : 1;
+  if (GROUPS > MAX_GROUPS) GROUPS = MAX_GROUPS;
+  const int per = (b + GROUPS - 1) / GROUPS;
+  const int ngroups = (b + per - 1) / per;
+  const uint64_t list_room = (slots - MAX_GROUPS) / (uint64_t)ngroups;
+  const uint32_t big_max = (uint32_t)(list_room < FIN_BIG_LIST ? list_room : FIN_BIG_LIST);
+  if (ngroups > 1 && hipMemsetAsync(w.runs, 0, (size_t)POOL_RUNS * sizeof(uint4), st) != hipSuccess) {
+    qrlsh_set_error("qrlsh_bucket_pairs_emit: hipMemsetAsync failed");
+    return QRLSH_EHIP;
+  }
+  hipStream_t aux = nullptr;
+  int gi = 0;
+  for (int g0 = 0; g0 < b; g0 += per, ++gi) {
+    const int nb = (b - g0 < per) ? b - g0 : per;
+    hipStream_t s = (aux && (gi & 1)) ? aux : st;
+    uint64_t *biglist = biglist0 + (size_t)gi * big_max;
+    unsigned long long *nbig = nbig0 + gi;
+    uint64_t *k1 = two ? tmp_keys : part_keys;
+    uint32_t *v1 = two ? tmp_ids : part_ids;
+    pool.slot_base = (uint32_t)((size_t)g0 << T);
+    BigDesc *desc = w.desc + (size_t)gi * FIN_BIG_LIST;
+    QR_PART_SCATTER(false, dim3(ntiles, nb), dim3(SORT_THREADS), 0, s, keys + (size_t)g0 * band_words,
+                    (const uint32_t *)nullptr, k1 + ((size_t)g0 << c1) * cap1, v1 + ((size_t)g0 << c1) * cap1, nq,
+                    ntiles, 64 - c1, (1u << c1) - 1u, cur1 + ((size_t)g0 << c1), cap1, ovf, qr_empty_key(r),
+                    (const uint32_t *)nullptr, 0u, key_chunk, key_chunk_stride, key_band_stride, two ? no_pool : pool,
+                    hmask);
+    if (two)
+      QR_PART_SCATTER(true, dim3((unsigned)ceil_div64(cap1, PS_TILE), nb << c1), dim3(SORT_THREADS), 0, s,
+                      (const uint64_t *)tmp_keys + ((size_t)g0 << c1) * cap1,
+                      (const uint32_t *)tmp_ids + ((size_t)g0 << c1) * cap1, part_keys + ((size_t)g0 << T) * cap2,
+                      part_ids + ((size_t)g0 << T) * cap2, (int64_t)0, 0, PACKED ? 64 - (T - c1) : 64 - T, lowmask,
+                      cur2 + ((size_t)g0 << T),
+                      cap2, ovf, qr_empty_key(r), (const uint32_t *)cur1 + ((size_t)g0 << c1), cap1, (int64_t)0,
+                      (int64_t)0, (int64_t)0, pool);
+    if (gi == 0 && b > per) aux = qr_aux_fork(st);
+    if (PACKED)
+      QR_LAUNCH("bucket_emit", bucket_finish_packed_kernel<true>, dim3(nparts, nb), dim3(FIN_PK_THREADS), 0, s,
+                (const uint64_t *)part_keys + ((size_t)g0 << T) * cap2, (const uint32_t *)nullptr, nparts,
+                total_overflow_out, ovf, pairs_out, capacity, (const uint32_t *)cur2 + ((size_t)g0 << T), cap2, biglist,
+                nbig, big_max, (uint32_t)((size_t)g0 << T), ib);
+    else if (small_parts && T >= 12 && g_fin_packed)
+      QR_LAUNCH("bucket_emit", bucket_finish_packed_kernel<false>, dim3(nparts, nb), dim3(FIN_PK_THREADS), 0, s,
+                (const uint64_t *)part_keys + ((size_t)g0 << T) * cap2, (const uint32_t *)part_ids + ((size_t)g0 << T) * cap2,
+                nparts, total_overflow_out, ovf, pairs_out, capacity, (const uint32_t *)cur2 + ((size_t)g0 << T), cap2, biglist,
+                nbig, big_max, (uint32_t)((size_t)g0 << T));
+    else if (small_parts)
+      QR_LAUNCH("bucket_emit", (bucket_finish_kernel<FIN_EMIT, FIN_SMALL_THREADS, FIN_SMALL_CAP>), dim3(nparts, nb),
+                dim3(FIN_SMALL_THREADS), 0, s, (const uint64_t *)part_keys + ((size_t)g0 << T) * cap2,
+                (const uint32_t *)part_ids + ((size_t)g0 << T) * cap2, nq, (const uint32_t *)nullptr, nparts, ekx,
+                total_overflow_out, ovf, pairs_out, capacity, (const uint32_t *)cur2 + ((size_t)g0 << T), cap2, biglist, nbig,
+                big_max, (uint32_t)((size_t)g0 << T));
+    else
+      QR_LAUNCH("bucket_emit", (bucket_finish_kernel<FIN_EMIT>), dim3(nparts, nb), dim3(FIN_THREADS), 0, s,
+                (const uint64_t *)part_keys + ((size_t)g0 << T) * cap2, (const uint32_t *)part_ids + ((size_t)g0 << T) * cap2,
+                nq, (const uint32_t *)nullptr, nparts, ekx, total_overflow_out, ovf, pairs_out, capacity,
+                (const uint32_t *)cur2 + ((size_t)g0 << T), cap2, biglist, nbig, big_max, (uint32_t)((size_t)g0 << T));
+    QR_LAUNCH("bucket_emit_big", bucket_big_gather_kernel<PACKED>, dim3(64), dim3(256), 0, s, (const uint64_t *)biglist,
+              (const unsigned long long *)nbig, big_max, desc, (const uint64_t *)part_keys, (const uint32_t *)part_ids,
+              (const uint32_t *)cur2, cap2, pool, g_big_limit, ovf);
+    QR_LAUNCH("bucket_emit_big", bucket_finish_big_kernel<PACKED>, dim3(FIN_BIG_GRID), dim3(FIN_THREADS), 0, s,
+              (const uint64_t *)part_keys, (const uint32_t *)part_ids, (const uint64_t *)pool.keys,
+              (const uint32_t *)pool.vals, ekx, (const BigDesc *)desc, (const unsigned long long *)nbig, big_max,
+              total_overflow_out, pairs_out, capacity, ib);
+  }
+  if (aux && qr_aux_join(st) != QRLSH_OK) return QRLSH_EHIP;
+  QR_LAUNCH_CHECK("qrlsh_bucket_pairs_emit");
+  return QRLSH_OK;
+#undef QR_PART_SCATTER
+}
+
 QRLSH_EXPORT int qrlsh_bucket_pairs_emit(const uint64_t *keys, uint64_t *part_keys, uint32_t *part_ids,
                                          uint64_t *tmp_keys, uint32_t *tmp_ids, int64_t nq, int32_t b, int32_t r,
                                          int32_t part_bits, void *workspace, size_t workspace_bytes,
@@ -1734,119 +1907,9 @@
                (unsigned long long)capacity);
   const int nparts = 1 << part_bits;
   const BucketWs w = bucket_ws(workspace, nq, b, part_bits);
-  const uint64_t ekx = qr_mix64(qr_empty_key(r));
-#define QR_PART_SCATTER(LEVEL2_, ...) QR_LAUNCH("part_scatter", (part_scatter_atomic_kernel<LEVEL2_>), __VA_ARGS__)
-  if (one_kernel_partition(nq, part_bits)) {
-    const int T = part_bits;
-    const bool two = T > 8;
-    const int c1 = two ? coarse_bits(T) : 8;
-    const uint32_t cap1 = two ? coarse_region(nq, c1) : part_region(nq), cap2 = two ? fine_region(nq, T) : cap1;
-    const uint32_t lowmask = (1u << (T - c1)) - 1u;
-    uint32_t *cur1 = two ? w.ghist : w.starts, *cur2 = w.starts;
-    if (hipMemsetAsync(cur1, 0, ((size_t)b << c1) * sizeof(uint32_t), st) != hipSuccess ||
-        (two && hipMemsetAsync(cur2, 0, ((size_t)b << T) * sizeof(uint32_t), st) != hipSuccess)) {
-      qrlsh_set_error("qrlsh_bucket_pairs_emit: hipMemsetAsync failed");
-      return QRLSH_EHIP;
-    }
-    uint32_t *ovf = reinterpret_cast<uint32_t *>(total_overflow_out + 1);
-    const size_t reg_words = region_words(nq, b, T);
-    PartPool pool;
-    pool.keys = part_keys + reg_words;
-    pool.vals = part_ids + reg_words;
-    pool.cursor = w.poolctl;
-    pool.nruns = w.poolctl + 1;
-    pool.cap = (uint32_t)pool_records(nq, b);
-    pool.runs = w.runs;
-    pool.runs_max = POOL_RUNS;
-    pool.fill = w.fill;
-    pool.slot_base = 0;
-    PartPool no_pool = pool;
-    no_pool.keys = nullptr;
-    no_pool.vals = nullptr;
-    if (hipMemsetAsync(w.fill, 0xFF, ((size_t)b << T) * sizeof(uint32_t), st) != hipSuccess ||
-        hipMemsetAsync(w.poolctl, 0, 16, st) != hipSuccess) {
-      qrlsh_set_error("qrlsh_bucket_pairs_emit: hipMemsetAsync failed");
-      return QRLSH_EHIP;
-    }
-    constexpr int MAX_GROUPS = EMIT_MAX_GROUPS;
-    unsigned long long *nbig0 = reinterpret_cast<unsigned long long *>(w.blk);
-    uint64_t *biglist0 = w.blk + MAX_GROUPS;
-    const uint64_t slots = (uint64_t)b << T;
-    if (hipMemsetAsync(nbig0, 0, MAX_GROUPS * sizeof(unsigned long long), st) != hipSuccess) {
-      qrlsh_set_error("qrlsh_bucket_pairs_emit: hipMemsetAsync failed");
-      return QRLSH_EHIP;
-    }
-    const bool small_parts = two && small_form(nq, T);
-    const int ntiles = (int)ceil_div64(nq, PS_TILE);
-    const int64_t band_words = key_band_stride ? key_band_stride : nq;
-    static int groups_env = -1;
-    if (groups_env < 0) {
-      const char *e = getenv("QRLSH_EMIT_GROUPS");
-      groups_env = e ? atoi(e) : 2;
-      if (groups_env < 1) groups_env = 1;
-    }
-    int GROUPS = (int64_t)b * nq >= (64ll << 20) ? groups_env : 1;
-    if (GROUPS > MAX_GROUPS) GROUPS = MAX_GROUPS;
-    const int per = (b + GROUPS - 1) / GROUPS;
-    const int ngroups = (b + per - 1) / per;
-    const uint64_t list_room = (slots - MAX_GROUPS) / (uint64_t)ngroups;
-    const uint32_t big_max = (uint32_t)(list_room < FIN_BIG_LIST ? list_room : FIN_BIG_LIST);
-    if (ngroups > 1 && hipMemsetAsync(w.runs, 0, (size_t)POOL_RUNS * sizeof(uint4), st) != hipSuccess) {
-      qrlsh_set_error("qrlsh_bucket_pairs_emit: hipMemsetAsync failed");
-      return QRLSH_EHIP;
-    }
-    hipStream_t aux = nullptr;
-    int gi = 0;
-    for (int g0 = 0; g0 < b; g0 += per, ++gi) {
-      const int nb = (b - g0 < per) ? b - g0 : per;
-      hipStream_t s = (aux && (gi & 1)) ? aux : st;
-      uint64_t *biglist = biglist0 + (size_t)gi * big_max;
-      unsigned long long *nbig = nbig0 + gi;
-      uint64_t *k1 = two ? tmp_keys : part_keys;
-      uint32_t *v1 = two ? tmp_ids : part_ids;
-      pool.slot_base = (uint32_t)((size_t)g0 << T);
-      BigDesc *desc = w.desc + (size_t)gi * FIN_BIG_LIST;
-      QR_PART_SCATTER(false, dim3(ntiles, nb), dim3(SORT_THREADS), 0, s, keys + (size_t)g0 * band_words,
-                      (const uint32_t *)nullptr, k1 + ((size_t)g0 << c1) * cap1, v1 + ((size_t)g0 << c1) * cap1, nq,
-                      ntiles, 64 - c1, (1u << c1) - 1u, cur1 + ((size_t)g0 << c1), cap1, ovf, qr_empty_key(r),
-                      (const uint32_t *)nullptr, 0u, key_chunk, key_chunk_stride, key_band_stride, two ? no_pool : pool);
-      if (two)
-        QR_PART_SCATTER(true, dim3((unsigned)ceil_div64(cap1, PS_TILE), nb << c1), dim3(SORT_THREADS), 0, s,
-                        (const uint64_t *)tmp_keys + ((size_t)g0 << c1) * cap1,
-                        (const uint32_t *)tmp_ids + ((size_t)g0 << c1) * cap1, part_keys + ((size_t)g0 << T) * cap2,
-                        part_ids + ((size_t)g0 << T) * cap2, (int64_t)0, 0, 64 - T, lowmask, cur2 + ((size_t)g0 << T),
-                        cap2, ovf, qr_empty_key(r), (const uint32_t *)cur1 + ((size_t)g0 << c1), cap1, (int64_t)0,
-                        (int64_t)0, (int64_t)0, pool);
-      if (gi == 0 && b > per) aux = qr_aux_fork(st);
-      if (small_parts && T >= 12 && g_fin_packed)
-        QR_LAUNCH("bucket_emit", bucket_finish_packed_kernel, dim3(nparts, nb), dim3(FIN_PK_THREADS), 0, s,
-                  (const uint64_t *)part_keys + ((size_t)g0 << T) * cap2, (const uint32_t *)part_ids + ((size_t)g0 << T) * cap2,
-                  nparts, total_overflow_out, ovf, pairs_out, capacity, (const uint32_t *)cur2 + ((size_t)g0 << T), cap2, biglist,
-                  nbig, big_max, (uint32_t)((size_t)g0 << T));
-      else if (small_parts)
-        QR_LAUNCH("bucket_emit", (bucket_finish_kernel<FIN_EMIT, FIN_SMALL_THREADS, FIN_SMALL_CAP>), dim3(nparts, nb),
-                  dim3(FIN_SMALL_THREADS), 0, s, (const uint64_t *)part_keys + ((size_t)g0 << T) * cap2,
-                  (const uint32_t *)part_ids + ((size_t)g0 << T) * cap2, nq, (const uint32_t *)nullptr, nparts, ekx,
-                  total_overflow_out, ovf, pairs_out, capacity, (const uint32_t *)cur2 + ((size_t)g0 << T), cap2, biglist, nbig,
-                  big_max, (uint32_t)((size_t)g0 << T));
-      else
-        QR_LAUNCH("bucket_emit", (bucket_finish_kernel<FIN_EMIT>), dim3(nparts, nb), dim3(FIN_THREADS), 0, s,
-                  (const uint64_t *)part_keys + ((size_t)g0 << T) * cap2, (const uint32_t *)part_ids + ((size_t)g0 << T) * cap2,
-                  nq, (const uint32_t *)nullptr, nparts, ekx, total_overflow_out, ovf, pairs_out, capacity,
-                  (const uint32_t *)cur2 + ((size_t)g0 << T), cap2, biglist, nbig, big_max, (uint32_t)((size_t)g0 << T));
-      QR_LAUNCH("bucket_emit_big", bucket_big_gather_kernel, dim3(64), dim3(256), 0, s, (const uint64_t *)biglist,
-                (const unsigned long long *)nbig, big_max, desc, (const uint64_t *)part_keys, (const uint32_t *)part_ids,
-                (const uint32_t *)cur2, cap2, pool, g_big_limit, ovf);
-      QR_LAUNCH("bucket_emit_big", bucket_finish_big_kernel, dim3(FIN_BIG_GRID), dim3(FIN_THREADS), 0, s,
-                (const uint64_t *)part_keys, (const uint32_t *)part_ids, (const uint64_t *)pool.keys,
-                (const uint32_t *)pool.vals, ekx, (const BigDesc *)desc, (const unsigned long long *)nbig, big_max,
-                total_overflow_out, pairs_out, capacity);
-    }
-    if (aux && qr_aux_join(st) != QRLSH_OK) return QRLSH_EHIP;
-    QR_LAUNCH_CHECK("qrlsh_bucket_pairs_emit");
-    return QRLSH_OK;
-  }
-#undef QR_PART_SCATTER
+  if (one_kernel_partition(nq, part_bits))
+    return bucket_emit_regions<false>(keys, key_chunk, key_chunk_stride, key_band_stride, part_keys, part_ids, tmp_keys,
+                                      tmp_ids, nq, b, r, part_bits, w, 0, pairs_out, capacity, total_overflow_out, st);
   QR_CHECK_ARG(key_chunk == 0, "qrlsh_bucket_pairs_emit_chunked: chunked keys need nq < 2^32");
   bucket_partition(keys, part_keys, part_ids, tmp_keys, tmp_ids, nq, b, r, part_bits, w, st);
   QR_LAUNCH("bucket_emit", (bucket_finish_kernel<FIN_EMIT>), dim3(nparts, b), dim3(FIN_THREADS), 0, st,
@@ -1855,6 +1918,25 @@
             capacity);
   QR_LAUNCH_CHECK("qrlsh_bucket_pairs_emit");
   return QRLSH_OK;
+}
+
+QRLSH_EXPORT int qrlsh_bucket_pairs_emit_packed(const uint64_t *keys, uint64_t *part_words, uint64_t *tmp_words, int64_t nq,
+                                                int32_t b, int32_t r, int32_t part_bits, int32_t id_bits, void *workspace,
+                                                size_t workspace_bytes, uint64_t *pairs_out, uint64_t capacity,
+                                                uint64_t *total_overflow_out, void *stream) {
+  hipStream_t st = static_cast<hipStream_t>(stream);
+  QR_CHECK_ARG(part_bits >= 12 && part_bits <= 16 && id_bits >= 1 && id_bits <= 24 && nq <= (1ll << id_bits),
+               "qrlsh_bucket_pairs_emit_packed: part_bits=%d must be in [12,16], id_bits=%d in [1,24], nq=%lld <= 2^id_bits",
+               part_bits, id_bits, (long long)nq);
+  uint32_t *dummy = reinterpret_cast<uint32_t *>(part_words);
+  const int rc = bucket_check("qrlsh_bucket_pairs_emit_packed", keys, part_words, dummy, tmp_words, dummy, nq, b, r,
+                              part_bits, workspace, workspace_bytes, total_overflow_out, st);
+  if (rc != QRLSH_OK || nq == 0) return rc;
+  QR_CHECK_ARG(pairs_out || capacity == 0, "qrlsh_bucket_pairs_emit_packed: null output with capacity %llu",
+               (unsigned long long)capacity);
+  const BucketWs w = bucket_ws(workspace, nq, b, part_bits);
+  return bucket_emit_regions<true>(keys, 0, 0, 0, part_words, nullptr, tmp_words, nullptr, nq, b, r, part_bits, w,
+                                   id_bits, pairs_out, capacity, total_overflow_out, st);
 }
 
 QRLSH_EXPORT int qrlsh_bucket_pairs_fill(const uint64_t *part_keys, const uint32_t *part_ids, int64_t nq, int32_t b,
diff --git a/query-recommendation-system_amd/qrlsh/_lib.py b/query-recommendation-system_amd/qrlsh/_lib.py
--- a/query-recommendation-system_amd/qrlsh/_lib.py
+++ b/query-recommendation-system_amd/qrlsh/_lib.py
@@ -50,6 +50,12 @@
     "qrlsh_bucket_part_words": (_sz, [_i64, _i32, _i32]),
     "qrlsh_set_big_part_limit": (_i64, [_i64]),
     "qrlsh_set_score_runs": (_i32, [_i32]),
+    "qrlsh_bucket_pairs_emit_packed": (ctypes.c_int, [_vp, _vp, _vp, _i64, _i32, _i32, _i32, _i32, _vp, _sz, _vp, _u64, _vp, _vp]),
+    "qrlsh_set_packed_records": (_i32, [_i32]),
+    "qrlsh_set_packed_hash_bits": (_i32, [_i32]),
+    "qrlsh_score_pairs_rev_checked": (ctypes.c_int, [_vp, _vp, _i32, _i32, _vp, _i64, _vp, _vp, _i32, _vp, _vp]),
+    "qrlsh_drop_marked_workspace_bytes": (_sz, [_i64]),
+    "qrlsh_drop_marked_pairs": (ctypes.c_int, [_vp, _vp, _i64, _vp, _vp, _sz, _vp]),
     "qrlsh_bucket_tmp_words": (_sz, [_i64, _i32, _i32]),
     "qrlsh_bucket_pairs_emit": (ctypes.c_int, [_vp, _vp, _vp, _vp, _vp, _i64, _i32, _i32, _i32, _vp, _sz, _vp, _u64, _vp, _vp]),
     "qrlsh_compact_workspace_bytes": (_sz, [_i64]),
diff --git a/query-recommendation-system_amd/qrlsh/ops.py b/query-recommendation-system_amd/qrlsh/ops.py
--- a/query-recommendation-system_amd/qrlsh/ops.py
+++ b/query-recommendation-system_amd/qrlsh/ops.py
@@ -415,7 +415,7 @@
 _EMIT_HINT = {}
 
 
-def emit_pairs_fast(keys, r, part_bits=None, one_pass=True, capacity=None, chunks=None):
+def emit_pairs_fast(keys, r, part_bits=None, one_pass=True, capacity=None, chunks=None, id_bits=None):
     lib = _lib.load()
     if chunks is not None:
         world, b, nql = chunks[:3]
@@ -433,12 +433,15 @@
     T = part_bits if part_bits is not None else part_bits_for(nq)
     if nq > 6144 * (1 << T):
         return None
+    packed = id_bits is not None
+    if packed and (T < 12 or not one_pass or chunks is not None):
+        raise ValueError("8-byte records need part_bits >= 12, the one-pass form and plain keys")
     words = lib.qrlsh_bucket_part_words(nq, b, T) if one_pass else b * nq
     pk = torch.empty((words,), dtype=torch.int64, device=dev)
-    pid = torch.empty((words,), dtype=torch.int32, device=dev)
+    pid = None if packed else torch.empty((words,), dtype=torch.int32, device=dev)
     twords = (lib.qrlsh_bucket_tmp_words(nq, b, T) if one_pass else b * nq) if T > 8 else 0
     tk = torch.empty((twords,), dtype=torch.int64, device=dev) if T > 8 else None
-    tid = torch.empty((twords,), dtype=torch.int32, device=dev) if T > 8 else None
+    tid = torch.empty((twords,), dtype=torch.int32, device=dev) if T > 8 and not packed else None
     ws = _ws(lib.qrlsh_bucket_workspace_bytes(nq, b, T), dev)
     tot = torch.zeros(2, dtype=torch.int64, device=dev)
     if one_pass:
@@ -447,9 +450,14 @@
             capacity = _EMIT_HINT[shape] * 5 // 4 + 1024 if shape in _EMIT_HINT else 24 * nq + 1024
         while True:
             pairs = torch.empty((capacity,), dtype=torch.int64, device=dev)
-            _lib.check(lib.qrlsh_bucket_pairs_emit_chunked(_ptr(keys), layout[0], layout[1], layout[2], _ptr(pk),
-                                                           _ptr(pid), _ptr(tk), _ptr(tid), nq, b, r, T, _ptr(ws),
-                                                           ws.numel(), _ptr(pairs), capacity, _ptr(tot), _stream()))
+            if packed:
+                _lib.check(lib.qrlsh_bucket_pairs_emit_packed(_ptr(keys), _ptr(pk), _ptr(tk), nq, b, r, T, int(id_bits),
+                                                              _ptr(ws), ws.numel(), _ptr(pairs), capacity, _ptr(tot),
+                                                              _stream()))
+            else:
+                _lib.check(lib.qrlsh_bucket_pairs_emit_chunked(_ptr(keys), layout[0], layout[1], layout[2], _ptr(pk),
+                                                               _ptr(pid), _ptr(tk), _ptr(tid), nq, b, r, T, _ptr(ws),
+                                                               ws.numel(), _ptr(pairs), capacity, _ptr(tot), _stream()))
             n, overflow = tot.tolist()
             if overflow:
                 return None
@@ -470,11 +478,12 @@
     return pairs
 
 
-def emit_pairs_any(keys, r, stats=None):
-    emitted = emit_pairs_fast(keys, r)
+def emit_pairs_any(keys, r, stats=None, part_bits=None, id_bits=None):
+    emitted = emit_pairs_fast(keys, r, part_bits=part_bits, id_bits=id_bits)
     if stats is not None:
         stats["bucket_path"] = "partition+lds" if emitted is not None else "general-sort"
-        stats["part_bits"] = part_bits_for(keys.shape[1])
+        stats["part_bits"] = part_bits if part_bits is not None else part_bits_for(keys.shape[1])
+        stats["record_bytes"] = 8 if id_bits is not None and emitted is not None else 12
     if emitted is None:
         sk, sid = bucket_sort(keys)
         emitted = emit_pairs(sk, sid, r)
@@ -504,11 +513,11 @@
     return pairs if bad == 0 else pairs[flags.bool()]
 
 
-def candidate_pairs(keys, r, stats=None, sig=None):
+def candidate_pairs(keys, r, stats=None, sig=None, part_bits=None, packed_id_bits=None):
     b, nq = keys.shape
     if r > 4 and sig is None:
         raise ValueError("band width r=%d > 4 needs the signatures for exact verification" % r)
-    emitted = emit_pairs_any(keys, r, stats)
+    emitted = emit_pairs_any(keys, r, stats, part_bits=part_bits, id_bits=packed_id_bits)
     if stats is not None:
         stats["emitted_pairs"] = int(emitted.numel())
     if emitted.numel() == 0:
@@ -686,10 +695,53 @@
     return milli, ((rev, rdst) if wide else rev)
 
 
+def packed_records_enabled():
+    return _lib.load().qrlsh_set_packed_records(-1) != 0
+
+
+def set_packed_records(on):
+    return _lib.load().qrlsh_set_packed_records(1 if on else 0) != 0
+
+
+def set_packed_hash_bits(bits):
+    return _lib.load().qrlsh_set_packed_hash_bits(int(bits))
+
+
+def packed_route(nq, b, r, sig, part_bits=None):
+    T = part_bits if part_bits is not None else part_bits_for(nq)
+    ib = id_bits_for(nq)
+    if not (T >= 12 and ib <= 24 and nq < (1 << ib) and r == 4 and b == 32 and sig.dtype == torch.int16
+            and sig.shape[1] == 128 and packed_records_enabled()):
+        return None
+    return ib
+
+
+def score_pairs_rev_checked(sig, norm2, pairs, id_bits, b, false_count):
+    lib = _lib.load()
+    _need(sig, torch.int16, "sig", 2)
+    _need(norm2, torch.int64, "norm2", 1)
+    _need(pairs, torch.int64, "pairs", 1)
+    n, dev = pairs.numel(), sig.device
+    milli = torch.empty((n,), dtype=torch.int32, device=dev)
+    rev = torch.empty((n,), dtype=torch.int64, device=dev)
+    _lib.check(lib.qrlsh_score_pairs_rev_checked(_ptr(sig), _ptr(norm2), sig.shape[1], int(b), _ptr(pairs), n, _ptr(milli),
+                                                 _ptr(rev), int(id_bits), _ptr(false_count), _stream()))
+    return milli, rev
+
+
+def drop_marked(pairs, milli, false_count):
+    lib = _lib.load()
+    n = pairs.numel()
+    if n == 0:
+        return
+    ws = _ws(lib.qrlsh_drop_marked_workspace_bytes(n), pairs.device)
+    _lib.check(lib.qrlsh_drop_marked_pairs(_ptr(pairs), _ptr(milli), n, _ptr(false_count), _ptr(ws), ws.numel(), _stream()))
+
+
 SELECT_MAX_K = 256
 
 
-def topk_select(pairs, milli, rev, K, id_bits, nq):
+def topk_select(pairs, milli, rev, K, id_bits, nq, total=None):
     lib = _lib.load()
     rdst = None
     if isinstance(rev, tuple):
@@ -698,7 +750,7 @@
     n = rev.numel()
     if n == 0:
         z = torch.empty((0,), dtype=torch.int32, device=dev)
-        return z, z.clone(), z.clone()
+        return (z, z.clone(), z.clone(), int(total[1].item())) if total is not None else (z, z.clone(), z.clone())
     if K > SELECT_MAX_K:
         raise ValueError("topk_select handles K <= %d; use topk_edges (the sort form) beyond" % SELECT_MAX_K)
     if rdst is None:
@@ -707,16 +759,19 @@
     else:
         rs, rd = sort_u64(rev, rdst, 11, 11 + id_bits)
     ws = _ws(lib.qrlsh_topk_select_workspace_bytes(nq), dev)
-    total = torch.zeros(1, dtype=torch.int64, device=dev)
+    extra = total is not None
+    if total is None:
+        total = torch.zeros(1, dtype=torch.int64, device=dev)
     _lib.check(lib.qrlsh_topk_select_count(_ptr(pairs), n, _ptr(rs), _ptr(rd), int(nq), K, int(id_bits), _ptr(ws), ws.numel(),
                                            _ptr(total), _stream()))
-    m = int(total.item())
+    read = total.tolist()
+    m = int(read[0])
     src = torch.empty((m,), dtype=torch.int32, device=dev)
     dst = torch.empty((m,), dtype=torch.int32, device=dev)
     val = torch.empty((m,), dtype=torch.int32, device=dev)
     _lib.check(lib.qrlsh_topk_select_fill(_ptr(pairs), _ptr(milli), n, _ptr(rs), _ptr(rd), int(nq), K, int(id_bits), _ptr(ws),
                                           _ptr(src), _ptr(dst), _ptr(val), _stream()))
-    return src, dst, val
+    return (src, dst, val, int(read[1])) if extra else (src, dst, val)
 
 
 def remap_pairs(pairs, q0, nql, need):
diff --git a/query-recommendation-system_amd/qrlsh/pipeline.py b/query-recommendation-system_amd/qrlsh/pipeline.py
--- a/query-recommendation-system_amd/qrlsh/pipeline.py
+++ b/query-recommendation-system_amd/qrlsh/pipeline.py
@@ -39,7 +39,7 @@
 
 
 def query_similarities(offsets, rows, table, b, K, timings=None, compact=None, wide_ids=None, topk="select",
-                       validate=True):
+                       validate=True, part_bits=None):
     nq = offsets.numel() - 1
     P = table.P
     if P % b != 0:
@@ -59,13 +59,32 @@
         compact = ops.can_compact(table)
     sig, norm2, keys = ops.minhash(offsets, rows, table, b=b, want_norm=True, compact=compact, validate=validate)
     t0 = tick("signatures", t0)
-    pairs = ops.candidate_pairs(keys, r, stats, sig=sig)
+    pib = (ops.packed_route(nq, b, r, sig, part_bits) if topk == "select" and K <= ops.SELECT_MAX_K and not wide_ids
+           else None)
+    pairs = ops.candidate_pairs(keys, r, stats, sig=sig, part_bits=part_bits, packed_id_bits=pib)
     del keys
     t0 = tick("candidates", t0)
     ib = ops.id_bits_for(nq)
+    stats.setdefault("record_bytes", 12)
+    stats["false_pairs_removed"] = 0
     if topk == "select" and (K > ops.SELECT_MAX_K or pairs.numel() >= (1 << 31)):
         topk = "sort"
-    if topk == "select":
+    packed = stats["record_bytes"] == 8
+    if packed and topk != "select":
+        n0 = pairs.numel()
+        pairs = ops.drop_unverified(sig, b, pairs)
+        stats["false_pairs_removed"] = n0 - pairs.numel()
+        packed = False
+    if topk == "select" and packed:
+        total = torch.zeros(2, dtype=torch.int64, device=pairs.device)
+        milli, rev = ops.score_pairs_rev_checked(sig, norm2, pairs, ib, b, total[1:])
+        ops.drop_marked(pairs, milli, total[1:])
+        t0 = tick("scoring", t0)
+        src, dst, val, f = ops.topk_select(pairs, milli, rev, K, ib, nq, total=total)
+        stats["false_pairs_removed"] = f
+        stats["emitted_pairs"] -= f
+        pairs, milli = pairs[:pairs.numel() - f], milli[:milli.numel() - f]
+    elif topk == "select":
         milli, rev = ops.score_pairs_rev(sig, norm2, pairs, ib, wide=wide_ids)
         t0 = tick("scoring", t0)
         src, dst, val = ops.topk_select(pairs, milli, rev, K, ib, nq)
```

Result: faster. 613.5 million, median of 6 (+1.6%).
